# youdie006/CLAP2Diffusion

Hardware: AMD Instinct MI355X
Metric: 512x512 images/sec @ 50 DDIM steps, batch=8, 1/2/4/8 MI355X (higher is better)
Workload: dtype fp16; 1 GPU; c3: batch=8/GPU, 50 DDIM steps, 512x512, CFG 7.5, log-mel+HTSAT+projectors+CLIP+UNet+VAE, all-gather of images; global_batch=8, ddim_steps=50, resolution=512, parallelism=dp1

## Files before the change

clap2diffusion_amd/csrc/common.h:

```cpp
#pragma once
#include <hip/hip_runtime.h>
#include <stdint.h>
#include <stddef.h>
#include <type_traits>
#include <mutex>
#include "../../include/c2d.h"

typedef _Float16 f16;
typedef _Float16 f16x8 __attribute__((ext_vector_type(8)));
typedef _Float16 f16x4 __attribute__((ext_vector_type(4)));
typedef _Float16 f16x2 __attribute__((ext_vector_type(2)));
typedef float f32x4 __attribute__((ext_vector_type(4)));
typedef float f32x2 __attribute__((ext_vector_type(2)));
typedef float f32x16 __attribute__((ext_vector_type(16)));
typedef short s16x4 __attribute__((ext_vector_type(4)));
typedef uint32_t u32x4 __attribute__((ext_vector_type(4)));
typedef uint32_t u32x2 __attribute__((ext_vector_type(2)));

#define LDS_AS __attribute__((address_space(3)))



#ifdef C2D_ENABLE_ABLATION
#define C2D_ABL(x, bit) ((x) & (bit))
#else
#define C2D_ABL(x, bit) 0
#endif

namespace c2d {

template <int B, int E, class F>
__device__ __forceinline__ void static_for(F&& f) {
    if constexpr (B < E) {
        f(std::integral_constant<int, B>{});
        static_for<B + 1, E>(f);
    }
}

extern thread_local int g_last_hip_error;

#ifndef C2D_TUNE_GEMM_MODE
#define C2D_TUNE_GEMM_MODE 0
#endif
#ifndef C2D_TUNE_GEMM_KORDER
#define C2D_TUNE_GEMM_KORDER 1
#endif
#ifndef C2D_TUNE_GEMM_LDSEPI
#define C2D_TUNE_GEMM_LDSEPI 1
#endif
#ifndef C2D_TUNE_SPLITK_F16
#define C2D_TUNE_SPLITK_F16 0
#endif
#ifndef C2D_TUNE_TAIL_SPLIT
#define C2D_TUNE_TAIL_SPLIT 1
#endif
#ifndef C2D_TUNE_PANEL_REGB
#define C2D_TUNE_PANEL_REGB 0
#endif
#ifndef C2D_TUNE_PANEL_STAGGER
#define C2D_TUNE_PANEL_STAGGER 2
#endif
#ifndef C2D_TUNE_PANEL_CARRY
#define C2D_TUNE_PANEL_CARRY 1
#endif
#ifndef C2D_TUNE_PANEL_PRIO
#define C2D_TUNE_PANEL_PRIO 1
#endif
#ifndef C2D_TUNE_ATTN_NEGC
#define C2D_TUNE_ATTN_NEGC 1
#endif
#ifndef C2D_TUNE_ATTN_RES
#define C2D_TUNE_ATTN_RES 1
#endif
#ifndef C2D_TUNE_ATTN_W8
#define C2D_TUNE_ATTN_W8 1
#endif
#ifndef C2D_TUNE_ATTN_PP
#define C2D_TUNE_ATTN_PP 0
#endif
#ifndef C2D_TUNE_GN_BLOCKS
#define C2D_TUNE_GN_BLOCKS 512
#endif
#ifndef C2D_TUNE_GN_APPLY_BLOCKS
#define C2D_TUNE_GN_APPLY_BLOCKS 2048
#endif
#ifndef C2D_TUNE_GN_FUSED_HW
#define C2D_TUNE_GN_FUSED_HW 256
#endif
#ifndef C2D_TUNE_GN_FOLD
#define C2D_TUNE_GN_FOLD 1
#endif
#ifndef C2D_TUNE_GN_FOLD_CAP
#define C2D_TUNE_GN_FOLD_CAP 32
#endif
#ifndef C2D_TUNE_GN_FOLD_APPLY_BLOCKS
#define C2D_TUNE_GN_FOLD_APPLY_BLOCKS 1024
#endif
struct Tuning {
    int gemm_mode, gemm_korder, gemm_lds_epi, splitk_f16, tail_split, panel_regb, panel_stagger;
    int attn_negc, attn_res, attn_w8, attn_pp;
    int gn_blocks, gn_apply_blocks, gn_fused_hw, gn_fold, gn_fold_cap, gn_fold_apply_blocks;
};
constexpr Tuning kTuning = {
    C2D_TUNE_GEMM_MODE, C2D_TUNE_GEMM_KORDER, C2D_TUNE_GEMM_LDSEPI, C2D_TUNE_SPLITK_F16, C2D_TUNE_TAIL_SPLIT,
    C2D_TUNE_PANEL_REGB, C2D_TUNE_PANEL_STAGGER,
    C2D_TUNE_ATTN_NEGC, C2D_TUNE_ATTN_RES, C2D_TUNE_ATTN_W8, C2D_TUNE_ATTN_PP,
    C2D_TUNE_GN_BLOCKS < 64 ? 512 : C2D_TUNE_GN_BLOCKS, C2D_TUNE_GN_APPLY_BLOCKS < 64 ? 2048 : C2D_TUNE_GN_APPLY_BLOCKS,
    C2D_TUNE_GN_FUSED_HW, C2D_TUNE_GN_FOLD, C2D_TUNE_GN_FOLD_CAP < 1 ? 32 : C2D_TUNE_GN_FOLD_CAP,
    C2D_TUNE_GN_FOLD_APPLY_BLOCKS < 64 ? 1024 : C2D_TUNE_GN_FOLD_APPLY_BLOCKS,
};
constexpr const Tuning& tuning() { return kTuning; }
int ablation_gemm();
int ablation_attn();
int plan_override_tile();
int plan_override_split();
constexpr int kMaxDevices = 64;
int current_device();

template <auto K>
inline void ensure_lds(int bytes) {
    static std::once_flag once[kMaxDevices];
    std::call_once(once[current_device()], [bytes] {
        (void)hipFuncSetAttribute((const void*)K, hipFuncAttributeMaxDynamicSharedMemorySize, bytes);
    });
}

inline int check_launch() {
    hipError_t e = hipGetLastError();
    if (e != hipSuccess) {
        g_last_hip_error = (int)e;
        return C2D_E_HIP;
    }
    return C2D_OK;
}

inline bool aligned16(const void* p) { return ((uintptr_t)p & 15) == 0; }

__device__ __forceinline__ float silu_f(float x) { return x / (1.0f + __expf(-x)); }
__device__ __forceinline__ float sigmoid_lin(float x, float k) { return x / (1.0f + __expf(-k * x)); }
__device__ __forceinline__ float erf_as(float x) {
    const float z = fabsf(x);
    const float t = __builtin_amdgcn_rcpf(fmaf(0.3275911f, z, 1.0f));
    float p = fmaf(1.061405429f, t, -1.453152027f);
    p = fmaf(p, t, 1.421413741f);
    p = fmaf(p, t, -0.284496736f);
    p = fmaf(p, t, 0.254829592f);
    const float e = 1.0f - p * t * __expf(-z * z);
    return copysignf(e, x);
}
__device__ __forceinline__ float gelu_f(float x) { return 0.5f * x * (1.0f + erf_as(x * 0.70710678118654752f)); }

__device__ __forceinline__ float gelu_sig(float x) {
    const float xc = __builtin_amdgcn_fmed3f(x, -8.0f, 8.0f);
    const float x2 = xc * xc;
    const float z = xc * fmaf(fmaf(-0.0009763994f, x2, 0.10652431f), x2, 2.3013635f);
    return x * __builtin_amdgcn_rcpf(1.0f + __builtin_amdgcn_exp2f(-z));
}
__device__ __forceinline__ f32x2 geglu2(f32x2 h, f32x2 g) {
    const f32x2 xc = {__builtin_amdgcn_fmed3f(g.x, -8.0f, 8.0f), __builtin_amdgcn_fmed3f(g.y, -8.0f, 8.0f)};
    const f32x2 x2 = xc * xc;
    f32x2 q = __builtin_elementwise_fma(x2, (f32x2){0.0009763994f, 0.0009763994f},
                                        (f32x2){-0.10652431f, -0.10652431f});
    q = __builtin_elementwise_fma(q, x2, (f32x2){-2.3013635f, -2.3013635f});
    const f32x2 nz = xc * q;
    f32x2 e = {__builtin_amdgcn_exp2f(nz.x), __builtin_amdgcn_exp2f(nz.y)};
    e = e + (f32x2){1.0f, 1.0f};
    const f32x2 hg = h * g;
    return hg * (f32x2){__builtin_amdgcn_rcpf(e.x), __builtin_amdgcn_rcpf(e.y)};
}


__device__ __forceinline__ int xcd_remap(int bid, int nwg) {
    const int q = nwg >> 3, r = nwg & 7;
    const int xcd = bid & 7, local = bid >> 3;
    return (xcd < r ? xcd * (q + 1) : r * (q + 1) + (xcd - r) * q) + local;
}

__device__ __forceinline__ const char* uniform_ptr(const void* p) {
    const uint64_t v = (uint64_t)p;
    const uint32_t lo = __builtin_amdgcn_readfirstlane((uint32_t)v);
    const uint32_t hi = __builtin_amdgcn_readfirstlane((uint32_t)(v >> 32));
    return (const char*)(((uint64_t)hi << 32) | lo);
}

__device__ __forceinline__ __amdgpu_buffer_rsrc_t make_rsrc(const void* base, unsigned bytes) {
    return __builtin_amdgcn_make_buffer_rsrc(const_cast<void*>(base), 0, (int)bytes, 0x00020000);
}

__device__ __forceinline__ float wave_sum(float v) {
#pragma unroll
    for (int o = 32; o > 0; o >>= 1) v += __shfl_xor(v, o);
    return v;
}
__device__ __forceinline__ float wave_max(float v) {
#pragma unroll
    for (int o = 32; o > 0; o >>= 1) v = fmaxf(v, __shfl_xor(v, o));
    return v;
}

}
```

clap2diffusion_amd/csrc/epilogue.h:

```cpp
#pragma once

namespace c2d {

template <int W, bool GG, int ROWS, int COLS, int RES, int TEMB, int NT = 64, int RG = 0, bool WB = false>
struct EpiPass {
    typedef _Float16 hv __attribute__((ext_vector_type(W)));
    static constexpr int CPR = GG ? COLS / (2 * W) : COLS / W;
    static constexpr int CPT = 16 / W;
    static constexpr int NCH = ROWS * CPR;
    static constexpr int NIT = (NCH + NT - 1) / NT;
    static_assert(COLS % (GG ? 32 : 8) == 0, "epilogue image width");
    hv r[RES ? NIT : 1], t[TEMB ? NIT : 1];
    __device__ __forceinline__ static bool has_res(const IgemmParams& p) { return RES > 0 || (RES < 0 && p.resid); }
    __device__ __forceinline__ static bool has_temb(const IgemmParams& p) { return TEMB > 0 || (TEMB < 0 && p.temb); }

    __device__ __forceinline__ static void geo(const IgemmParams& p, int m0, int jp0, int lane, int it, int& row,
                                               int& sc, int& m, int& j, bool& ok) {
        int c = lane + NT * it;
        ok = c < NCH;
        c = ok ? c : NCH - 1;
        row = c / CPR;
        const int cc = c - row * CPR;
        if constexpr (GG) {
            const int t = cc / CPT, q = cc - t * CPT;
            sc = t * 32 + q * W;
            j = ((jp0 + t * 32) >> 1) + q * W;
        } else {
            sc = cc * W;
            j = jp0 + sc;
        }
        m = m0 + (RG ? (row >> 5) * RG + (row & 31) : row);
        ok = ok && m < p.M && j < (GG ? (p.cout >> 1) : p.cout);
        if (!ok) { m = m0 < p.M ? m0 : 0; j = 0; }
    }

    __device__ __forceinline__ void prefetch(const IgemmParams& p, int m0, int jp0, int lane) {
        if constexpr (RES != 0 || TEMB != 0) {
            const int hw = p.oh * p.ow;
            const int n_all = (RG == 0 && (hw % ROWS) == 0) ? m0 / hw : -1;
#pragma unroll
            for (int it = 0; it < NIT; ++it) {
                int row, sc, m, j;
                bool ok;
                geo(p, m0, jp0, lane, it, row, sc, m, j, ok);
                if (TEMB != 0 && has_temb(p))
                    t[it] = *reinterpret_cast<const hv*>(p.temb + (size_t)(ok ? (n_all >= 0 ? n_all : m / hw) : 0) *
                                                                      p.temb_ld + j);
                if (RES != 0 && has_res(p)) r[it] = *reinterpret_cast<const hv*>(p.resid + (size_t)m * p.resid_ld + j);
            }
        }
    }

    __device__ __forceinline__ static void body(const IgemmParams& p, const float* img, int pitchf, int row, int sc,
                                                int m, int j, bool ok, const hv& rr, const hv& tt) {
        const float* src = img + row * pitchf + sc;
        float v[W];
#pragma unroll
        for (int q = 0; q < W; q += 4) {
            const float4 x = *reinterpret_cast<const float4*>(src + q);
            v[q] = x.x; v[q + 1] = x.y; v[q + 2] = x.z; v[q + 3] = x.w;
        }
        if constexpr (GG) {
#pragma unroll
            for (int q = 0; q < W; q += 4) {
                const float4 y = *reinterpret_cast<const float4*>(src + 16 + q);
                v[q] *= gelu_sig(y.x); v[q + 1] *= gelu_sig(y.y); v[q + 2] *= gelu_sig(y.z); v[q + 3] *= gelu_sig(y.w);
            }
        } else if (p.act == C2D_ACT_GELU) {
#pragma unroll
            for (int q = 0; q < W; ++q) v[q] = gelu_f(v[q]);
        } else if (p.act == C2D_ACT_RELU) {
#pragma unroll
            for (int q = 0; q < W; ++q) v[q] = fmaxf(v[q], 0.f);
        } else if (p.act == C2D_ACT_SILU) {
#pragma unroll
            for (int q = 0; q < W; ++q) v[q] = silu_f(v[q]);
        } else if (p.act == C2D_ACT_QUICK_GELU) {
#pragma unroll
            for (int q = 0; q < W; ++q) v[q] = sigmoid_lin(v[q], 1.702f);
        }
        if (TEMB != 0 && has_temb(p)) {
#pragma unroll
            for (int q = 0; q < W; ++q) v[q] += (float)tt[q];
        }
        if (RES != 0 && has_res(p)) {
#pragma unroll
            for (int q = 0; q < W; ++q) v[q] += (float)rr[q];
        }
        hv o;
#pragma unroll
        for (int q = 0; q < W; ++q) o[q] = (f16)v[q];
        if (ok) *reinterpret_cast<hv*>(p.out + (size_t)m * p.out_ld + j) = o;
        if constexpr (WB) {
            float* dst = const_cast<float*>(src);
#pragma unroll
            for (int q = 0; q < W; q += 4)
                *reinterpret_cast<float4*>(dst + q) = make_float4((float)o[q], (float)o[q + 1], (float)o[q + 2], (float)o[q + 3]);
        }
    }

    __device__ __forceinline__ void finish(const IgemmParams& p, const float* img, int pitchf, int m0, int jp0,
                                           int lane) const {
#pragma unroll
        for (int it = 0; it < NIT; ++it) {
            int row, sc, m, j;
            bool ok;
            geo(p, m0, jp0, lane, it, row, sc, m, j, ok);
            body(p, img, pitchf, row, sc, m, j, ok, r[RES ? it : 0], t[TEMB ? it : 0]);
        }
    }

    __device__ __forceinline__ static void compact(const IgemmParams& p, const float* img, int pitchf, int m0,
                                                   int jp0, int lane) {
        const int hw = p.oh * p.ow;
        const int n_all = (RG == 0 && (hw % ROWS) == 0) ? m0 / hw : -1;
#pragma unroll 2
        for (int it = 0; it < NIT; ++it) {
            int row, sc, m, j;
            bool ok;
            geo(p, m0, jp0, lane, it, row, sc, m, j, ok);
            hv rr, tt;
            if (TEMB != 0 && has_temb(p))
                tt = *reinterpret_cast<const hv*>(p.temb + (size_t)(ok ? (n_all >= 0 ? n_all : m / hw) : 0) * p.temb_ld + j);
            if (RES != 0 && has_res(p)) rr = *reinterpret_cast<const hv*>(p.resid + (size_t)m * p.resid_ld + j);
            body(p, img, pitchf, row, sc, m, j, ok, rr, tt);
        }
    }
};

template <bool COMPACT, int NT, int RG, int W, bool GG, int ROWS, int COLS, int RES, int TEMB, class WriteImg>
__device__ __forceinline__ void epi_pass_t(const IgemmParams& p, const float* img, int pitchf, int m0, int jp0,
                                           int lane, WriteImg&& write_img) {
    typedef EpiPass<W, GG, ROWS, COLS, RES, TEMB, NT, RG> EP;
    auto sync = [&]() __attribute__((always_inline)) {
        if constexpr (NT == 64) {
            __builtin_amdgcn_s_waitcnt(15 | (7 << 4) | (0 << 8) | (3 << 14));
            __builtin_amdgcn_wave_barrier();
        } else {
            __builtin_amdgcn_s_waitcnt(15 | (7 << 4) | (0 << 8) | (3 << 14));
            asm volatile("" ::: "memory");
            __builtin_amdgcn_s_barrier();
            asm volatile("" ::: "memory");
        }
    };
    if constexpr (COMPACT) {
        write_img();
        sync();
        EP::compact(p, img, pitchf, m0, jp0, lane);
    } else {
        EP ep;
        ep.prefetch(p, m0, jp0, lane);
        write_img();
        sync();
        ep.finish(p, img, pitchf, m0, jp0, lane);
    }
    sync();
}

template <int NT, int RG, int ROWS, int COLS, class WriteImg, class After>
__device__ __forceinline__ void epi_pass_wb(const IgemmParams& p, const float* img, int pitchf, int m0, int jp0,
                                            int lane, WriteImg&& write_img, After&& after) {
    typedef EpiPass<8, false, ROWS, COLS, -1, -1, NT, RG, true> EP;
    auto sync = [&]() __attribute__((always_inline)) {
        __builtin_amdgcn_s_waitcnt(15 | (7 << 4) | (0 << 8) | (3 << 14));
        asm volatile("" ::: "memory");
        __builtin_amdgcn_s_barrier();
        asm volatile("" ::: "memory");
    };
    write_img();
    sync();
    EP::compact(p, img, pitchf, m0, jp0, lane);
    sync();
    after();
    sync();
}

template <int NPASS, int ROWS, int BN, int BM, int RG, class WriteImg>
__device__ __forceinline__ void epi_gn_moments(const IgemmParams& p, float* img, int pitchb, int m0, int n0, int tid,
                                               WriteImg&& write_img) {
    float sh = 0.f, s1 = 0.f, s2 = 0.f;
    static_for<0, NPASS>([&](auto pass) __attribute__((always_inline)) {
        constexpr int b0 = 2 * decltype(pass)::value;
        epi_pass_wb<512, RG, ROWS, BN>(p, img, pitchb, m0 + b0 * 16, n0, tid,
                                       [&]() __attribute__((always_inline)) { write_img(pass); },
                                       [&]() __attribute__((always_inline)) {
            if (tid < BN) {
                if constexpr (b0 == 0) sh = img[tid];
#pragma unroll 8
                for (int r = 0; r < ROWS; ++r) {
                    const float d = img[r * pitchb + tid] - sh;
                    s1 += d;
                    s2 = fmaf(d, d, s2);
                }
            }
        });
    });
    float2* chm = reinterpret_cast<float2*>(img);
    if (tid < BN) chm[tid] = make_float2(sh + s1 * (1.0f / BM), s2 - s1 * s1 * (1.0f / BM));
    __syncthreads();
    const int cpg = p.gn_cpg, ng = BN / cpg;
    if (tid < ng) {
        float mg = 0.f;
        for (int i = 0; i < cpg; ++i) mg += chm[tid * cpg + i].x;
        mg /= (float)cpg;
        float q = 0.f;
        for (int i = 0; i < cpg; ++i) {
            const float2 e = chm[tid * cpg + i];
            const float d = e.x - mg;
            q += e.y + (float)BM * d * d;
        }
        const int hw = p.oh * p.ow, nimg = m0 / hw, tpi = hw / BM, groups = p.cout / cpg;
        const size_t slot = ((size_t)nimg * tpi + (m0 - nimg * hw) / BM) * groups + n0 / cpg + tid;
        reinterpret_cast<float2*>(p.gn_mom)[slot] = make_float2(mg, q);
    }
}

template <int ROWS, int COLS, bool COMPACT, int NT = 64, int RG = 0, class WriteImg>
__device__ __forceinline__ void epi_pass(const IgemmParams& p, const float* img, int pitchf, int m0, int jp0,
                                         int lane, WriteImg&& w) {
    const bool gg = p.act == C2D_ACT_GEGLU;
    const int out_cols = gg ? (p.cout >> 1) : p.cout;
    const uintptr_t al = (uintptr_t)p.out | (uintptr_t)p.resid | (uintptr_t)p.temb;
    const bool wide = ((out_cols | p.out_ld | (p.resid ? p.resid_ld : 0) | (p.temb ? p.temb_ld : 0)) & 7) == 0 &&
                      (al & 15) == 0;
    if constexpr (COMPACT) {
        if constexpr (COLS % 32 == 0) {
            if (gg) {
                if (wide) epi_pass_t<true, NT, RG, 8, true, ROWS, COLS, -1, 0>(p, img, pitchf, m0, jp0, lane, w);
                else epi_pass_t<true, NT, RG, 4, true, ROWS, COLS, -1, 0>(p, img, pitchf, m0, jp0, lane, w);
                return;
            }
        }
        if (wide) epi_pass_t<true, NT, RG, 8, false, ROWS, COLS, -1, -1>(p, img, pitchf, m0, jp0, lane, w);
        else epi_pass_t<true, NT, RG, 4, false, ROWS, COLS, -1, -1>(p, img, pitchf, m0, jp0, lane, w);
        return;
    }
    if constexpr (COLS % 32 == 0) {
        if (gg) {
            if (wide && !p.resid) epi_pass_t<COMPACT, NT, RG, 8, true, ROWS, COLS, 0, 0>(p, img, pitchf, m0, jp0, lane, w);
            else epi_pass_t<COMPACT, NT, RG, 4, true, ROWS, COLS, -1, 0>(p, img, pitchf, m0, jp0, lane, w);
            return;
        }
    }
    if (!wide) epi_pass_t<COMPACT, NT, RG, 4, false, ROWS, COLS, -1, -1>(p, img, pitchf, m0, jp0, lane, w);
    else if (p.resid) {
        if (p.temb) epi_pass_t<COMPACT, NT, RG, 8, false, ROWS, COLS, 1, 1>(p, img, pitchf, m0, jp0, lane, w);
        else epi_pass_t<COMPACT, NT, RG, 8, false, ROWS, COLS, 1, 0>(p, img, pitchf, m0, jp0, lane, w);
    } else {
        if (p.temb) epi_pass_t<COMPACT, NT, RG, 8, false, ROWS, COLS, 0, 1>(p, img, pitchf, m0, jp0, lane, w);
        else epi_pass_t<COMPACT, NT, RG, 8, false, ROWS, COLS, 0, 0>(p, img, pitchf, m0, jp0, lane, w);
    }
}

__device__ __forceinline__ f32x4 bias4(const IgemmParams& p, int j) {
    if (!p.bias || j >= p.cout) return (f32x4){0.f, 0.f, 0.f, 0.f};
    return *reinterpret_cast<const f32x4*>(p.bias + j);
}

template <int W, bool GG, int ROWS, int COLS>
__device__ __forceinline__ void epi_rows_plain_t(const IgemmParams& p, const float* img, int pitchf, int m0, int jp0,
                                           int lane) {
    typedef _Float16 hv __attribute__((ext_vector_type(W)));
    constexpr int CPR = GG ? COLS / (2 * W) : COLS / W;
    constexpr int CPT = 16 / W;
    static_assert(COLS % (GG ? 32 : 8) == 0, "epilogue image width");
    const int hw = p.oh * p.ow;
    const int out_cols = GG ? (p.cout >> 1) : p.cout;
    const int n_all = (hw % ROWS) == 0 ? m0 / hw : -1;
#pragma unroll 2
    for (int c = lane; c < ROWS * CPR; c += 64) {
        const int row = c / CPR, cc = c - row * CPR;
        const int m = m0 + row;
        int sc, jp, j;
        if constexpr (GG) {
            const int t = cc / CPT, q = cc - t * CPT;
            sc = t * 32 + q * W;
            jp = jp0 + sc;
            j = ((jp0 + t * 32) >> 1) + q * W;
        } else {
            sc = cc * W;
            jp = jp0 + sc;
            j = jp;
        }
        if (m >= p.M || j >= out_cols) continue;
        const float* src = img + row * pitchf + sc;
        float v[W];
#pragma unroll
        for (int r = 0; r < W; r += 4) {
            const float4 x = *reinterpret_cast<const float4*>(src + r);
            v[r] = x.x; v[r + 1] = x.y; v[r + 2] = x.z; v[r + 3] = x.w;
        }
        if (p.bias) {
#pragma unroll
            for (int r = 0; r < W; r += 4) {
                const float4 bb = *reinterpret_cast<const float4*>(p.bias + jp + r);
                v[r] += bb.x; v[r + 1] += bb.y; v[r + 2] += bb.z; v[r + 3] += bb.w;
            }
        }
        if constexpr (GG) {
            float g[W];
#pragma unroll
            for (int r = 0; r < W; r += 4) {
                const float4 x = *reinterpret_cast<const float4*>(src + 16 + r);
                g[r] = x.x; g[r + 1] = x.y; g[r + 2] = x.z; g[r + 3] = x.w;
                if (p.bias) {
                    const float4 bb = *reinterpret_cast<const float4*>(p.bias + jp + 16 + r);
                    g[r] += bb.x; g[r + 1] += bb.y; g[r + 2] += bb.z; g[r + 3] += bb.w;
                }
            }
#pragma unroll
            for (int r = 0; r < W; ++r) v[r] *= gelu_sig(g[r]);
        } else if (p.act == C2D_ACT_GELU) {
#pragma unroll
            for (int r = 0; r < W; ++r) v[r] = gelu_f(v[r]);
        } else if (p.act == C2D_ACT_RELU) {
#pragma unroll
            for (int r = 0; r < W; ++r) v[r] = fmaxf(v[r], 0.f);
        } else if (p.act == C2D_ACT_SILU) {
#pragma unroll
            for (int r = 0; r < W; ++r) v[r] = silu_f(v[r]);
        } else if (p.act == C2D_ACT_QUICK_GELU) {
#pragma unroll
            for (int r = 0; r < W; ++r) v[r] = sigmoid_lin(v[r], 1.702f);
        }
        if (p.temb) {
            const hv tt = *reinterpret_cast<const hv*>(p.temb + (size_t)(n_all >= 0 ? n_all : m / hw) * p.temb_ld + j);
#pragma unroll
            for (int r = 0; r < W; ++r) v[r] += (float)tt[r];
        }
        if (p.resid) {
            const hv rr = *reinterpret_cast<const hv*>(p.resid + (size_t)m * p.resid_ld + j);
#pragma unroll
            for (int r = 0; r < W; ++r) v[r] += (float)rr[r];
        }
        hv o;
#pragma unroll
        for (int r = 0; r < W; ++r) o[r] = (f16)v[r];
        *reinterpret_cast<hv*>(p.out + (size_t)m * p.out_ld + j) = o;
    }
}

template <int ROWS, int COLS>
__device__ __forceinline__ void epi_rows_plain(const IgemmParams& p, const float* img, int pitchf, int m0, int jp0,
                                         int lane) {
    const bool gg = p.act == C2D_ACT_GEGLU;
    const int out_cols = gg ? (p.cout >> 1) : p.cout;
    const uintptr_t al = (uintptr_t)p.out | (uintptr_t)p.resid | (uintptr_t)p.temb;
    const bool wide = ((out_cols | p.out_ld | (p.resid ? p.resid_ld : 0) | (p.temb ? p.temb_ld : 0)) & 7) == 0 &&
                      (al & 15) == 0;
    if constexpr (COLS % 32 == 0) {
        if (gg) {
            if (wide) epi_rows_plain_t<8, true, ROWS, COLS>(p, img, pitchf, m0, jp0, lane);
            else epi_rows_plain_t<4, true, ROWS, COLS>(p, img, pitchf, m0, jp0, lane);
            return;
        }
    }
    if (wide) epi_rows_plain_t<8, false, ROWS, COLS>(p, img, pitchf, m0, jp0, lane);
    else epi_rows_plain_t<4, false, ROWS, COLS>(p, img, pitchf, m0, jp0, lane);
}

}
```

clap2diffusion_amd/csrc/igemm.hip:

```cpp
#include "common.h"
#include <stdlib.h>
#include <type_traits>

#ifndef C2D_PP16_DEFAULT
#define C2D_PP16_DEFAULT 1
#endif

#ifndef C2D_IGEMM_PART
#define C2D_IGEMM_PART -1
#endif
#define C2D_PART(k) (C2D_IGEMM_PART < 0 || C2D_IGEMM_PART == (k))

namespace c2d {

enum AMode { AM_1X1 = 0, AM_3X3_FAST = 1, AM_3X3_GEN = 2 };

struct IgemmParams {
    const f16* src0; const f16* src1; int c0, c1, cin;
    int n, h, w, oh, ow, stride, up, pad;
    int vh, vw;
    const f16* wt; int cout, kpad, ktot;
    int pro, pro_silu;
    const float* pro_a; const float* pro_b; const float* gamma; const float* beta;
    const float* bias; int act;
    const f16* temb; int temb_ld;
    const f16* resid; int resid_ld;
    f16* out; int out_ld;
    int M;
    int gx, gy;
    int ksplit;
    int nkt;
    float* ws;
    int slab16;
    int abl;
    int lds_epi;
    int cmajor;
    float pro_eps;
    float* gn_mom;
    int gn_cpg;
};

__device__ __forceinline__ void store_partial(const IgemmParams& p, int slice, int m, int j, const f32x4& v) {
    const size_t off = ((size_t)slice * p.M + m) * p.cout + j;
    if (p.slab16) {
        const f16x4 h = {(f16)v[0], (f16)v[1], (f16)v[2], (f16)v[3]};
        *reinterpret_cast<f16x4*>(reinterpret_cast<f16*>(p.ws) + off) = h;
    } else {
        *reinterpret_cast<f32x4*>(p.ws + off) = v;
    }
}

}
#include "epilogue.h"
namespace c2d {

__device__ __forceinline__ int lds_off(int row, int c) { return row * 128 + ((c ^ ((row >> 1) & 7)) << 4); }

template <int BM>
struct RowInfo {
    int n[BM / 32], iy[BM / 32], ix[BM / 32];
    bool ok[BM / 32];
};

__device__ __forceinline__ f16x8 zero8() {
    f16x8 z;
#pragma unroll
    for (int i = 0; i < 8; ++i) z[i] = (f16)0.f;
    return z;
}

template <int AMODE>
__device__ __forceinline__ f16x8 load_a_chunk(const IgemmParams& p, int n, int iy0, int ix0, bool rok,
                                              int k, int tap_fast, int cbase_fast, int cc, int& cout_c,
                                              bool& valid) {
    int c, ky, kx;
    if (AMODE == AM_1X1) {
        c = k; ky = 0; kx = 0;
        valid = rok && (c < p.cin);
    } else if (AMODE == AM_3X3_FAST) {
        c = cbase_fast + cc * 8;
        ky = tap_fast / 3; kx = tap_fast - ky * 3;
        valid = rok;
    } else {
        int tap = k / p.cin;
        c = k - tap * p.cin;
        ky = tap / 3; kx = tap - ky * 3;
        valid = rok && (tap < 9);
    }
    int iy = iy0 + ky, ix = ix0 + kx;
    valid = valid && iy >= 0 && iy < p.vh && ix >= 0 && ix < p.vw;
    cout_c = c;
    if (!valid) return zero8();
    if (p.up) { iy >>= 1; ix >>= 1; }
    size_t pix = ((size_t)n * p.h + iy) * p.w + ix;
    const f16* ptr = (c < p.c0) ? (p.src0 + pix * p.c0 + c) : (p.src1 + pix * p.c1 + (c - p.c0));
    return *reinterpret_cast<const f16x8*>(ptr);
}

__device__ __forceinline__ f16x8 apply_pro(const IgemmParams& p, f16x8 v, int n, int m, int c) {
    if (p.pro == C2D_PRO_GN) {
        const float4* sc = reinterpret_cast<const float4*>(p.pro_a + (size_t)n * p.cin + c);
        const float4* sh = reinterpret_cast<const float4*>(p.pro_b + (size_t)n * p.cin + c);
        float4 s0 = sc[0], s1 = sc[1], h0 = sh[0], h1 = sh[1];
        float s[8] = {s0.x, s0.y, s0.z, s0.w, s1.x, s1.y, s1.z, s1.w};
        float hh[8] = {h0.x, h0.y, h0.z, h0.w, h1.x, h1.y, h1.z, h1.w};
#pragma unroll
        for (int i = 0; i < 8; ++i) {
            float y = (float)v[i] * s[i] + hh[i];
            if (p.pro_silu) y = silu_f(y);
            v[i] = (f16)y;
        }
    } else if (p.pro == C2D_PRO_LN) {
        float2 st = *reinterpret_cast<const float2*>(p.pro_a + (size_t)m * 2);
        const float4* g = reinterpret_cast<const float4*>(p.gamma + c);
        const float4* b = reinterpret_cast<const float4*>(p.beta + c);
        float4 g0 = g[0], g1 = g[1], b0 = b[0], b1 = b[1];
        float gg[8] = {g0.x, g0.y, g0.z, g0.w, g1.x, g1.y, g1.z, g1.w};
        float bb[8] = {b0.x, b0.y, b0.z, b0.w, b1.x, b1.y, b1.z, b1.w};
#pragma unroll
        for (int i = 0; i < 8; ++i) v[i] = (f16)(((float)v[i] - st.x) * st.y * gg[i] + bb[i]);
    } else if (p.pro == C2D_PRO_SILU) {
#pragma unroll
        for (int i = 0; i < 8; ++i) v[i] = (f16)silu_f((float)v[i]);
    }
    return v;
}

template <int TM, int TN>
__device__ __forceinline__ void epilogue_tiles(const IgemmParams& p, f32x4 (&acc)[TN][TM], int mrow0, int ncol0,
                                               int lane) {
    const int hw = p.oh * p.ow;
    const int lr = lane & 15, lc = 4 * (lane >> 4);
    int mrow[TM], nimg[TM];
    bool mok[TM];
#pragma unroll
    for (int b = 0; b < TM; ++b) {
        const int m = mrow0 + b * 16 + lr;
        mok[b] = m < p.M;
        mrow[b] = mok[b] ? m : p.M - 1;
        nimg[b] = mrow[b] / hw;
    }
    if (p.act != C2D_ACT_GEGLU) {
        int col[TN];
        bool cok[TN];
        float4 bv[TN];
#pragma unroll
        for (int a = 0; a < TN; ++a) {
            const int j = ncol0 + a * 16 + lc;
            cok[a] = j < p.cout;
            col[a] = cok[a] ? j : 0;
            bv[a] = p.bias ? *reinterpret_cast<const float4*>(p.bias + col[a]) : make_float4(0.f, 0.f, 0.f, 0.f);
        }
        f16x4 rv[TM][TN], tv[TM][TN];
        if (p.resid) {
#pragma unroll
            for (int b = 0; b < TM; ++b)
#pragma unroll
                for (int a = 0; a < TN; ++a)
                    rv[b][a] = *reinterpret_cast<const f16x4*>(p.resid + (size_t)mrow[b] * p.resid_ld + col[a]);
        }
        if (p.temb) {
#pragma unroll
            for (int b = 0; b < TM; ++b)
#pragma unroll
                for (int a = 0; a < TN; ++a)
                    tv[b][a] = *reinterpret_cast<const f16x4*>(p.temb + (size_t)nimg[b] * p.temb_ld + col[a]);
        }
#pragma unroll
        for (int b = 0; b < TM; ++b) {
#pragma unroll
            for (int a = 0; a < TN; ++a) {
                float v[4] = {acc[a][b][0] + bv[a].x, acc[a][b][1] + bv[a].y, acc[a][b][2] + bv[a].z,
                              acc[a][b][3] + bv[a].w};
#pragma unroll
                for (int r = 0; r < 4; ++r) {
                    if (p.act == C2D_ACT_GELU) v[r] = gelu_f(v[r]);
                    else if (p.act == C2D_ACT_RELU) v[r] = fmaxf(v[r], 0.f);
                    else if (p.act == C2D_ACT_SILU) v[r] = silu_f(v[r]);
                    else if (p.act == C2D_ACT_QUICK_GELU) v[r] = sigmoid_lin(v[r], 1.702f);
                    if (p.temb) v[r] += (float)tv[b][a][r];
                    if (p.resid) v[r] += (float)rv[b][a][r];
                }
                f16x4 o;
#pragma unroll
                for (int r = 0; r < 4; ++r) o[r] = (f16)v[r];
                if (mok[b] && cok[a]) *reinterpret_cast<f16x4*>(p.out + (size_t)mrow[b] * p.out_ld + col[a]) = o;
            }
        }
    } else {
        constexpr int TP = TN / 2;
        int jo[TP], jh[TP];
        bool cok[TP];
        float4 bh[TP], bg[TP];
#pragma unroll
        for (int q = 0; q < TP; ++q) {
            const int jp = ncol0 + 2 * q * 16;
            cok[q] = jp < p.cout;
            const int jpc = cok[q] ? jp : 0;
            jo[q] = (jpc >> 1) + lc;
            jh[q] = jpc + lc;
            bh[q] = p.bias ? *reinterpret_cast<const float4*>(p.bias + jh[q]) : make_float4(0.f, 0.f, 0.f, 0.f);
            bg[q] = p.bias ? *reinterpret_cast<const float4*>(p.bias + jh[q] + 16) : make_float4(0.f, 0.f, 0.f, 0.f);
        }
        f16x4 rv[TM][TP];
        if (p.resid) {
#pragma unroll
            for (int b = 0; b < TM; ++b)
#pragma unroll
                for (int q = 0; q < TP; ++q)
                    rv[b][q] = *reinterpret_cast<const f16x4*>(p.resid + (size_t)mrow[b] * p.resid_ld + jo[q]);
        }
#pragma unroll
        for (int b = 0; b < TM; ++b) {
#pragma unroll
            for (int q = 0; q < TP; ++q) {
                const f32x4 h4 = acc[2 * q][b], g4 = acc[2 * q + 1][b];
                const float hb[4] = {bh[q].x, bh[q].y, bh[q].z, bh[q].w}, gb[4] = {bg[q].x, bg[q].y, bg[q].z, bg[q].w};
                f16x4 o;
#pragma unroll
                for (int r = 0; r < 4; ++r) {
                    float v = (h4[r] + hb[r]) * gelu_sig(g4[r] + gb[r]);
                    if (p.resid) v += (float)rv[b][q][r];
                    o[r] = (f16)v;
                }
                if (mok[b] && cok[q]) *reinterpret_cast<f16x4*>(p.out + (size_t)mrow[b] * p.out_ld + jo[q]) = o;
            }
        }
    }
}

template <int BM, int BN>
__device__ __forceinline__ void epilogue(const IgemmParams& p, f32x4 (&acc)[BN / 32][BM / 32], int m0, int n0, int wm,
                                         int wn, int lane) {
    epilogue_tiles<BM / 32, BN / 32>(p, acc, m0 + wm * (BM / 2), n0 + wn * (BN / 2), lane);
}

__device__ __forceinline__ void epilogue_w64(const IgemmParams& p, f32x4 (&acc)[4][4], int mw0, int nw0, int lane) {
    epilogue_tiles<4, 4>(p, acc, mw0, nw0, lane);
}

template <int BM, int BN, int AMODE>
__global__ void __launch_bounds__(256) igemm_kernel(IgemmParams p) {
    constexpr int TM = BM / 32;
    constexpr int TN = BN / 32;
    constexpr int ACH = BM / 32;
    constexpr int BCH = BN / 32;
    constexpr int A_BYTES = BM * 128, B_BYTES = BN * 128;
    extern __shared__ __attribute__((aligned(16))) char smem[];

    const int tid = threadIdx.x, lane = tid & 63, wave = tid >> 6;
    const int wm = wave >> 1, wn = wave & 1;
    const int tile = xcd_remap(blockIdx.x, p.gx * p.gy);
    const int mt = tile / p.gx, nt = tile - mt * p.gx;
    const int m0 = mt * BM, n0 = nt * BN;

    const int cc = tid & 7;
    const int hw = p.oh * p.ow;
    int a_n[ACH], a_iy[ACH], a_ix[ACH], a_m[ACH];
    bool a_ok[ACH];
#pragma unroll
    for (int i = 0; i < ACH; ++i) {
        int m = m0 + (tid >> 3) + 32 * i;
        a_m[i] = m;
        a_ok[i] = m < p.M;
        int mm = a_ok[i] ? m : 0;
        int nn = mm / hw, r = mm - nn * hw;
        int oy = r / p.ow, ox = r - oy * p.ow;
        a_n[i] = nn;
        a_iy[i] = oy * p.stride - p.pad;
        a_ix[i] = ox * p.stride - p.pad;
    }
    const f16* b_ptr[BCH];
    bool b_ok[BCH];
#pragma unroll
    for (int i = 0; i < BCH; ++i) {
        int j = n0 + (tid >> 3) + 32 * i;
        b_ok[i] = j < p.cout;
        b_ptr[i] = p.wt + (size_t)(b_ok[i] ? j : 0) * p.kpad + cc * 8;
    }

    f32x4 acc[TN][TM];
#pragma unroll
    for (int a = 0; a < TN; ++a)
#pragma unroll
        for (int b = 0; b < TM; ++b) acc[a][b] = (f32x4){0.f, 0.f, 0.f, 0.f};

    f16x8 ra[ACH], rb[BCH];
    int rc[ACH];
    bool rv[ACH];
    const int nk = p.kpad / 64;

    auto gload = [&](int kt) {
        const int k0 = kt * 64;
        int tap = 0, cbase = 0;
        if (AMODE == AM_3X3_FAST) { tap = k0 / p.cin; cbase = k0 - tap * p.cin; }
#pragma unroll
        for (int i = 0; i < ACH; ++i)
            ra[i] = load_a_chunk<AMODE>(p, a_n[i], a_iy[i], a_ix[i], a_ok[i], k0 + cc * 8, tap, cbase, cc, rc[i], rv[i]);
#pragma unroll
        for (int i = 0; i < BCH; ++i)
            rb[i] = b_ok[i] ? *reinterpret_cast<const f16x8*>(b_ptr[i] + k0) : zero8();
    };
    auto swrite = [&](int buf) {
        char* As = smem + buf * (A_BYTES + B_BYTES);
        char* Bs = As + A_BYTES;
#pragma unroll
        for (int i = 0; i < ACH; ++i) {
            f16x8 v = ra[i];
            if (p.pro != C2D_PRO_NONE && rv[i]) v = apply_pro(p, v, a_n[i], a_m[i], rc[i]);
            int row = (tid >> 3) + 32 * i;
            *reinterpret_cast<f16x8*>(As + lds_off(row, cc)) = v;
        }
#pragma unroll
        for (int i = 0; i < BCH; ++i) {
            int row = (tid >> 3) + 32 * i;
            *reinterpret_cast<f16x8*>(Bs + lds_off(row, cc)) = rb[i];
        }
    };

    gload(0);
    swrite(0);
    __syncthreads();

    for (int kt = 0; kt < nk; ++kt) {
        const int buf = kt & 1;
        if (kt + 1 < nk) gload(kt + 1);
        const char* As = smem + buf * (A_BYTES + B_BYTES);
        const char* Bs = As + A_BYTES;
#pragma unroll
        for (int kk = 0; kk < 2; ++kk) {
            const int ch = kk * 4 + (lane >> 4);
            f16x8 fa[TM], fb[TN];
#pragma unroll
            for (int t = 0; t < TM; ++t) {
                int row = wm * (BM / 2) + t * 16 + (lane & 15);
                fa[t] = *reinterpret_cast<const f16x8*>(As + lds_off(row, ch));
            }
#pragma unroll
            for (int t = 0; t < TN; ++t) {
                int row = wn * (BN / 2) + t * 16 + (lane & 15);
                fb[t] = *reinterpret_cast<const f16x8*>(Bs + lds_off(row, ch));
            }
#pragma unroll
            for (int a = 0; a < TN; ++a)
#pragma unroll
                for (int b = 0; b < TM; ++b)
                    acc[a][b] = __builtin_amdgcn_mfma_f32_16x16x32_f16(fb[a], fa[b], acc[a][b], 0, 0, 0);
        }
        if (kt + 1 < nk) swrite(buf ^ 1);
        __syncthreads();
    }

    epilogue<BM, BN>(p, acc, m0, n0, wm, wn, lane);
}


typedef __attribute__((address_space(3))) void* lptr_t;
constexpr unsigned kOOB = 0x80000000u;

__device__ __forceinline__ void wait_vmcnt_le(int n) {
#define C2D_WAITVM(N) __builtin_amdgcn_s_waitcnt(((N) & 15) | (7 << 4) | (15 << 8) | (((N) >> 4) << 14))
    switch (n) {
        case 4: C2D_WAITVM(4); break;
        case 6: C2D_WAITVM(6); break;
        case 8: C2D_WAITVM(8); break;
        case 12: C2D_WAITVM(12); break;
        case 16: C2D_WAITVM(16); break;
        default: C2D_WAITVM(0); break;
    }
#undef C2D_WAITVM
}


__device__ __forceinline__ void dma_piece(__amdgpu_buffer_rsrc_t r, char* lds, unsigned off) {
    __builtin_amdgcn_raw_ptr_buffer_load_lds(r, (lptr_t)lds, 16, off, 0, 0, 0);
}

template <int TM, int TN>
__device__ __forceinline__ void epilogue_chunked(const IgemmParams& p, f32x4 (&acc)[TN][TM], int mrow0, int ncol0,
                                                 int lane) {
    constexpr int MC = TM < 4 ? TM : 4;
#pragma unroll
    for (int b0 = 0; b0 < TM; b0 += MC) {
        f32x4 sub[TN][MC];
#pragma unroll
        for (int a = 0; a < TN; ++a)
#pragma unroll
            for (int b = 0; b < MC; ++b) sub[a][b] = acc[a][b0 + b];
        epilogue_tiles<MC, TN>(p, sub, mrow0 + b0 * 16, ncol0, lane);
    }
}

template <int WM, int WN, int TM, int TN, int STAGES, int KS, int KG = 1>
__global__ void __launch_bounds__(64 * WM * WN * KG) igemm_dma_kernel(IgemmParams p) {
    constexpr int NW = WM * WN;
    constexpr int BM = WM * TM * 16, BN = WN * TN * 16;
    constexpr int AI = BM / (8 * NW), BI = BN / (8 * NW);
    constexpr int PER = AI + BI;
    constexpr int A_BYTES = BM * 128, B_BYTES = BN * 128, STAGE = A_BYTES + B_BYTES;
    static_assert(AI * 8 * NW == BM && BI * 8 * NW == BN, "tile / wave mismatch");
    extern __shared__ __attribute__((aligned(16))) char smem_all[];

    const int tid = threadIdx.x, lane = tid & 63;
    const int wave_all = __builtin_amdgcn_readfirstlane(tid >> 6);
    const int kg = wave_all / NW, wave = wave_all - kg * NW;
    char* const smem = smem_all + (KG > 1 ? kg * STAGES * STAGE : 0);
    const int wm = wave / WN, wn = wave - (wave / WN) * WN;
    const int bid = xcd_remap(blockIdx.x, p.gx * p.gy * p.ksplit);
    const int tile = bid / p.ksplit, slice = bid - tile * p.ksplit;
    const int mt = tile / p.gx, nt = tile - mt * p.gx;
    const int m0 = mt * BM, n0 = nt * BN;
    const int lrow = lane >> 3, slot = lane & 7;
    const int hw = p.oh * p.ow;
    const bool two = p.c1 > 0;
    const int pshift = KS == 3 ? p.w + 1 : 0;

    unsigned a_off0[AI], a_off1[AI], a_mask[AI];
    int a_ch[AI];
#pragma unroll
    for (int i = 0; i < AI; ++i) {
        const int row = (wave * AI + i) * 8 + lrow;
        const int m = m0 + row;
        const int mm = m < p.M ? m : 0;
        const int nn = mm / hw, r = mm - nn * hw;
        const int oy = r / p.ow, ox = r - oy * p.ow;
        const int iy0 = oy * p.stride - p.pad, ix0 = ox * p.stride - p.pad;
        unsigned mask = 0;
        if (m < p.M) {
#pragma unroll
            for (int ky = 0; ky < KS; ++ky)
#pragma unroll
                for (int kx = 0; kx < KS; ++kx)
                    if (iy0 + ky >= 0 && iy0 + ky < p.h && ix0 + kx >= 0 && ix0 + kx < p.w) mask |= 1u << (ky * KS + kx);
        }
        const int pix0 = (nn * p.h + iy0) * p.w + ix0 + pshift;
        a_ch[i] = (slot ^ ((row >> 1) & 7)) * 8;
        a_off0[i] = (unsigned)(2 * (pix0 * p.c0 + a_ch[i]));
        a_off1[i] = (unsigned)(2 * (pix0 * p.c1 + a_ch[i]));
        a_mask[i] = mask;
    }
    unsigned b_off[BI];
#pragma unroll
    for (int i = 0; i < BI; ++i) {
        const int row = (wave * BI + i) * 8 + lrow;
        const int j = n0 + row;
        b_off[i] = (j < p.cout) ? (unsigned)(2 * (j * p.kpad + (slot ^ ((row >> 1) & 7)) * 8)) : kOOB;
    }
    const size_t npix = (size_t)p.n * p.h * p.w;
    const unsigned bytes0 = (unsigned)(npix * p.c0 * 2), bytes1 = (unsigned)(npix * p.c1 * 2);
    const unsigned wbytes = (unsigned)((size_t)p.cout * p.kpad * 2);
    const bool ctail = (p.cin & 63) != 0;

    const int nk_all = p.kpad / 64;
    const int kb0 = slice * p.nkt, ke0 = min(nk_all, kb0 + p.nkt);
    const int kper = (ke0 - kb0 + KG - 1) / KG;
    const int kb = min(ke0, kb0 + kg * kper), ke = min(ke0, kb + kper);
    const char* u_src0 = uniform_ptr(p.src0);
    const char* u_src1 = uniform_ptr(p.src1);
    const char* u_wt = uniform_ptr(p.wt);
    int tap = 0, cbase = kb * 64;
    if (KS == 3) {
        if (p.cmajor) { tap = kb % 9; cbase = (kb / 9) * 64; }
        else { tap = cbase / p.cin; cbase -= tap * p.cin; }
    }
    auto issue = [&](int kt, int buf) {
        (void)kt;
        const int k0 = tap * p.cin + cbase;
        const int ky = tap / 3, kx = tap - (tap / 3) * 3;
        const bool use1 = two && cbase >= p.c0;
        const int cs = use1 ? p.c1 : p.c0;
        const unsigned sterm = 2u * (unsigned)((KS == 3 ? (ky * p.w + kx) * cs : 0) + (use1 ? cbase - p.c0 : cbase));
        const char* sb = use1 ? u_src1 : u_src0;
        const unsigned bias = 2u * (unsigned)(pshift * cs);
        const unsigned sbytes = use1 ? bytes1 : bytes0;
        const __amdgpu_buffer_rsrc_t ra = make_rsrc(sb + sterm - bias, sbytes + bias - sterm);
        const __amdgpu_buffer_rsrc_t rb = make_rsrc(u_wt + 2 * k0, wbytes - 2 * k0);
        const int lim = p.cin - cbase;
        char* base = smem + buf * STAGE;
#pragma unroll
        for (int i = 0; i < AI; ++i) {
            unsigned ok = (a_mask[i] >> tap) & 1u;
            if (ctail) ok &= (unsigned)(a_ch[i] < lim);
            const unsigned off = (use1 ? a_off1[i] : a_off0[i]) | ((ok - 1u) & kOOB);
            dma_piece(ra, base + (wave * AI + i) * 1024, off);
        }
#pragma unroll
        for (int i = 0; i < BI; ++i)
            dma_piece(rb, base + A_BYTES + (wave * BI + i) * 1024, b_off[i]);
        if (KS == 3 && p.cmajor) {
            if (++tap == 9) { tap = 0; cbase += 64; }
        } else {
            cbase += 64;
            if (KS == 3 && cbase >= p.cin) { cbase = 0; ++tap; }
        }
    };

    int fa0[2], fb0[2];
#pragma unroll
    for (int kk = 0; kk < 2; ++kk) {
        const int l = lds_off(lane & 15, kk * 4 + (lane >> 4));
        fa0[kk] = wm * TM * 2048 + l;
        fb0[kk] = A_BYTES + wn * TN * 2048 + l;
    }

    f32x4 acc[TN][TM];
#pragma unroll
    for (int a = 0; a < TN; ++a)
#pragma unroll
        for (int b = 0; b < TM; ++b) acc[a][b] = (f32x4){0.f, 0.f, 0.f, 0.f};

#pragma unroll
    for (int s0 = 0; s0 < STAGES - 1; ++s0)
        if (kb + s0 < ke) issue(kb + s0, s0);
    int rd = 0, wr = STAGES - 1;
    const int kend = KG > 1 ? kb + kper : ke;
    for (int kt = kb; kt < kend; ++kt) {
        if (kt + STAGES - 2 < ke) wait_vmcnt_le(PER * (STAGES - 2));
        else wait_vmcnt_le(0);
        asm volatile("" ::: "memory");
        __builtin_amdgcn_s_barrier();
        asm volatile("" ::: "memory");
        if (kt + STAGES - 1 < ke && !(C2D_ABL(p.abl, 1))) issue(kt + STAGES - 1, wr);
        const char* S = smem + rd * STAGE;
        if (KG > 1 && kt >= ke) continue;
#pragma unroll
        for (int kk = 0; kk < 2; ++kk) {
            f16x8 fa[TM], fb[TN];
#pragma unroll
            for (int t = 0; t < TN; ++t) fb[t] = *reinterpret_cast<const f16x8*>(S + fb0[kk] + t * 2048);
#pragma unroll
            for (int t = 0; t < TM; ++t) fa[t] = *reinterpret_cast<const f16x8*>(S + fa0[kk] + t * 2048);
            if (C2D_ABL(p.abl, 2)) {
#pragma unroll
                for (int t = 0; t < TN; ++t) asm volatile("" :: "v"(fb[t]));
#pragma unroll
                for (int t = 0; t < TM; ++t) asm volatile("" :: "v"(fa[t]));
                continue;
            }
            __builtin_amdgcn_s_setprio(1);
#pragma unroll
            for (int b = 0; b < TM; ++b)
#pragma unroll
                for (int a = 0; a < TN; ++a)
                    acc[a][b] = __builtin_amdgcn_mfma_f32_16x16x32_f16(fb[a], fa[b], acc[a][b], 0, 0, 0);
            __builtin_amdgcn_s_setprio(0);
        }
        rd = (rd + 1 == STAGES) ? 0 : rd + 1;
        wr = (wr + 1 == STAGES) ? 0 : wr + 1;
    }
    if constexpr (KG > 1) {
        constexpr int EPI = NW * 16 * (TM < 2 ? TM : 2) * (TN * 16 + 4) * 4;
        constexpr int RED = (EPI + 1023) / 1024 * 1024;
        f32x4* red = reinterpret_cast<f32x4*>(smem_all + RED);
        __syncthreads();
        if (kg > 0) {
#pragma unroll
            for (int a = 0; a < TN; ++a)
#pragma unroll
                for (int b = 0; b < TM; ++b)
                    red[((((kg - 1) * NW + wave) * TN + a) * TM + b) * 64 + lane] = acc[a][b];
        }
        __syncthreads();
        if (kg > 0) return;
#pragma unroll
        for (int g = 1; g < KG; ++g)
#pragma unroll
            for (int a = 0; a < TN; ++a)
#pragma unroll
                for (int b = 0; b < TM; ++b) acc[a][b] += red[((((g - 1) * NW + wave) * TN + a) * TM + b) * 64 + lane];
    }
    if (p.ksplit > 1) {
        const int mw0 = m0 + wm * TM * 16, nw0 = n0 + wn * TN * 16;
#pragma unroll
        for (int b = 0; b < TM; ++b) {
            const int m = mw0 + b * 16 + (lane & 15);
#pragma unroll
            for (int a = 0; a < TN; ++a) {
                const int j = nw0 + a * 16 + 4 * (lane >> 4);
                if (m < p.M && j < p.cout) store_partial(p, slice, m, j, acc[a][b]);
            }
        }
        return;
    }
    __syncthreads();
    {
        constexpr int PITCHF = TN * 16 + 4;
        constexpr int RB = TM < 2 ? TM : 2;
        float* img = reinterpret_cast<float*>(smem) + wave * 16 * RB * PITCHF;
        const int mw0 = m0 + wm * TM * 16, nw0 = n0 + wn * TN * 16;
        static_for<0, TM / RB>([&](auto pass) __attribute__((always_inline)) {
            constexpr int b0 = RB * decltype(pass)::value;
            epi_pass<RB * 16, TN * 16, false>(p, img, PITCHF, mw0 + b0 * 16, nw0, lane, [&]() __attribute__((always_inline)) {
                f32x4 bv[TN];
#pragma unroll
                for (int a = 0; a < TN; ++a) bv[a] = bias4(p, nw0 + a * 16 + 4 * (lane >> 4));
#pragma unroll
                for (int bb = 0; bb < RB; ++bb)
#pragma unroll
                    for (int a = 0; a < TN; ++a)
                        *reinterpret_cast<f32x4*>(img + (bb * 16 + (lane & 15)) * PITCHF + a * 16 + 4 * (lane >> 4)) =
                            acc[a][b0 + bb] + bv[a];
            });
        });
    }
}

#if C2D_PART(0)
template <bool S16>
__device__ __forceinline__ f32x4 slab_quad(const float* ws, size_t off) {
    if constexpr (S16) {
        const f16x4 h = *reinterpret_cast<const f16x4*>(reinterpret_cast<const f16*>(ws) + off);
        return (f32x4){(float)h[0], (float)h[1], (float)h[2], (float)h[3]};
    } else {
        return *reinterpret_cast<const f32x4*>(ws + off);
    }
}

template <int KS, bool S16>
__global__ void __launch_bounds__(256) splitk_reduce_kernel(IgemmParams p) {
    const int cq = p.cout >> 2;
    const size_t i = (size_t)blockIdx.x * blockDim.x + threadIdx.x;
    if (i >= (size_t)p.M * cq) return;
    const int hw = p.oh * p.ow;
    const size_t slab = (size_t)p.M * p.cout;
    const int m = (int)(i / cq);
    const int j = (int)(i - (size_t)m * cq) * 4;
    const size_t src = (size_t)m * p.cout + j;
    float4 bv = {0.f, 0.f, 0.f, 0.f};
    f16x4 tv = {0, 0, 0, 0}, rv = {0, 0, 0, 0};
    if (p.bias) bv = *reinterpret_cast<const float4*>(p.bias + j);
    if (p.temb) tv = *reinterpret_cast<const f16x4*>(p.temb + (size_t)(m / hw) * p.temb_ld + j);
    if (p.resid) rv = *reinterpret_cast<const f16x4*>(p.resid + (size_t)m * p.resid_ld + j);
    f32x4 acc;
    if constexpr (KS > 0) {
        f32x4 v[KS];
#pragma unroll
        for (int sl = 0; sl < KS; ++sl) v[sl] = slab_quad<S16>(p.ws, src + sl * slab);
        acc = v[0];
#pragma unroll
        for (int sl = 1; sl < KS; ++sl) acc += v[sl];
    } else {
        acc = slab_quad<S16>(p.ws, src);
        int sl = 1;
        for (; sl + 4 <= p.ksplit; sl += 4) {
            const f32x4 a = slab_quad<S16>(p.ws, src + sl * slab);
            const f32x4 b = slab_quad<S16>(p.ws, src + (sl + 1) * slab);
            const f32x4 c = slab_quad<S16>(p.ws, src + (sl + 2) * slab);
            const f32x4 d = slab_quad<S16>(p.ws, src + (sl + 3) * slab);
            acc += a; acc += b; acc += c; acc += d;
        }
        for (; sl < p.ksplit; ++sl) acc += slab_quad<S16>(p.ws, src + sl * slab);
    }
    float v[4] = {acc[0] + bv.x, acc[1] + bv.y, acc[2] + bv.z, acc[3] + bv.w};
    f16x4 o;
#pragma unroll
    for (int r = 0; r < 4; ++r) {
        if (p.act == C2D_ACT_GELU) v[r] = gelu_f(v[r]);
        else if (p.act == C2D_ACT_RELU) v[r] = fmaxf(v[r], 0.f);
        else if (p.act == C2D_ACT_SILU) v[r] = silu_f(v[r]);
        else if (p.act == C2D_ACT_QUICK_GELU) v[r] = sigmoid_lin(v[r], 1.702f);
        if (p.temb) v[r] += (float)tv[r];
        if (p.resid) v[r] += (float)rv[r];
        o[r] = (f16)v[r];
    }
    *reinterpret_cast<f16x4*>(p.out + (size_t)m * p.out_ld + j) = o;
}

constexpr int kGnRb = 16;
template <int KS, bool S16>
__global__ void __launch_bounds__(640) splitk_reduce_gn_kernel(IgemmParams p) {
    __shared__ float2 cm[8][320];
    const int t = threadIdx.x, q = t % 80, rs = t / 80;
    const int m0 = blockIdx.x * kGnRb, j = blockIdx.y * 320 + 4 * q;
    const int hw = p.oh * p.ow;
    const size_t slab = (size_t)p.M * p.cout;
    float4 bv = {0.f, 0.f, 0.f, 0.f};
    f16x4 tv = {0, 0, 0, 0}, rv[2] = {{0, 0, 0, 0}, {0, 0, 0, 0}};
    if (p.bias) bv = *reinterpret_cast<const float4*>(p.bias + j);
    if (p.temb) tv = *reinterpret_cast<const f16x4*>(p.temb + (size_t)(m0 / hw) * p.temb_ld + j);
    f32x4 v[2][KS];
#pragma unroll
    for (int i = 0; i < 2; ++i) {
        const int m = m0 + rs + 8 * i;
        if (p.resid) rv[i] = *reinterpret_cast<const f16x4*>(p.resid + (size_t)m * p.resid_ld + j);
#pragma unroll
        for (int sl = 0; sl < KS; ++sl) v[i][sl] = slab_quad<S16>(p.ws, (size_t)m * p.cout + j + sl * slab);
    }
    float y[2][4];
    const float b4[4] = {bv.x, bv.y, bv.z, bv.w};
#pragma unroll
    for (int i = 0; i < 2; ++i) {
        f32x4 acc = v[i][0];
#pragma unroll
        for (int sl = 1; sl < KS; ++sl) acc += v[i][sl];
        f16x4 o;
#pragma unroll
        for (int r = 0; r < 4; ++r) {
            float x = acc[r] + b4[r];
            if (p.temb) x += (float)tv[r];
            if (p.resid) x += (float)rv[i][r];
            o[r] = (f16)x;
            y[i][r] = (float)o[r];
        }
        *reinterpret_cast<f16x4*>(p.out + (size_t)(m0 + rs + 8 * i) * p.out_ld + j) = o;
    }
#pragma unroll
    for (int r = 0; r < 4; ++r) {
        const float d = y[0][r] - y[1][r];
        cm[rs][4 * q + r] = make_float2(0.5f * (y[0][r] + y[1][r]), 0.5f * d * d);
    }
    __syncthreads();
    float2 col = {0.f, 0.f};
    if (t < 320) {
        float mu = 0.f;
#pragma unroll
        for (int k = 0; k < 8; ++k) mu += cm[k][t].x;
        mu *= 0.125f;
        float m2 = 0.f;
#pragma unroll
        for (int k = 0; k < 8; ++k) {
            const float d = cm[k][t].x - mu;
            m2 += cm[k][t].y + 2.0f * d * d;
        }
        col = make_float2(mu, m2);
    }
    __syncthreads();
    if (t < 320) cm[0][t] = col;
    __syncthreads();
    const int cpg = p.gn_cpg, ng = 320 / cpg;
    if (t < ng) {
        float mg = 0.f;
        for (int i = 0; i < cpg; ++i) mg += cm[0][t * cpg + i].x;
        mg /= (float)cpg;
        float m2 = 0.f;
        for (int i = 0; i < cpg; ++i) {
            const float d = cm[0][t * cpg + i].x - mg;
            m2 += cm[0][t * cpg + i].y + (float)kGnRb * d * d;
        }
        const int nimg = m0 / hw, groups = p.cout / cpg;
        const size_t slot = ((size_t)nimg * (hw / kGnRb) + (m0 - nimg * hw) / kGnRb) * groups + blockIdx.y * ng + t;
        reinterpret_cast<float2*>(p.gn_mom)[slot] = make_float2(mg, m2);
    }
}

void run_splitk_reduce(const IgemmParams& p, hipStream_t s) {
    if (p.gn_mom) {
        const dim3 grid((unsigned)(p.M / kGnRb), (unsigned)(p.cout / 320)), blk(640);
#define C2D_SKG(KS)                                                                                    \
    if (p.slab16) hipLaunchKernelGGL((splitk_reduce_gn_kernel<KS, true>), grid, blk, 0, s, p);        \
    else hipLaunchKernelGGL((splitk_reduce_gn_kernel<KS, false>), grid, blk, 0, s, p)
        switch (p.ksplit) {
            case 2: C2D_SKG(2); break;
            case 3: C2D_SKG(3); break;
            case 4: C2D_SKG(4); break;
            case 5: C2D_SKG(5); break;
            case 6: C2D_SKG(6); break;
            case 8: C2D_SKG(8); break;
            case 10: C2D_SKG(10); break;
            case 12: C2D_SKG(12); break;
            case 15: C2D_SKG(15); break;
            default: C2D_SKG(16); break;
        }
#undef C2D_SKG
        return;
    }
    const size_t total = (size_t)p.M * (p.cout >> 2);
    const dim3 grid((unsigned)((total + 255) / 256)), blk(256);
#define C2D_SKR(KS)                                                                   \
    if (p.slab16) hipLaunchKernelGGL((splitk_reduce_kernel<KS, true>), grid, blk, 0, s, p); \
    else hipLaunchKernelGGL((splitk_reduce_kernel<KS, false>), grid, blk, 0, s, p)
    switch (p.ksplit) {
        case 2: C2D_SKR(2); break;
        case 3: C2D_SKR(3); break;
        case 4: C2D_SKR(4); break;
        case 6: C2D_SKR(6); break;
        case 8: C2D_SKR(8); break;
        case 12: C2D_SKR(12); break;
        case 16: C2D_SKR(16); break;
        default: C2D_SKR(0); break;
    }
#undef C2D_SKR
}
#else
void run_splitk_reduce(const IgemmParams& p, hipStream_t s);
#endif

}
#include "igemm_m32.h"
#include "igemm_pp16.h"
#include "igemm_pps.h"
#include "igemm_pp16r.h"
#include "igemm_panel.h"
namespace c2d {

template <int WM, int WN, int TM, int TN, int STAGES, int KS, int KG = 1>
static void launch_dma(const IgemmParams& p, hipStream_t s) {
    constexpr int ring = KG * STAGES * (WM * TM + WN * TN) * 16 * 128;
    constexpr int epi0 = WM * WN * 16 * (TM < 2 ? TM : 2) * (TN * 16 + 4) * 4;
    constexpr int epi = KG > 1 ? (epi0 + 1023) / 1024 * 1024 + (KG - 1) * WM * WN * TM * TN * 1024 : epi0;
    constexpr int smem = ring > epi ? ring : epi;
    static_assert(smem <= 160 * 1024, "LDS ring / epilogue image too large");
    auto k = igemm_dma_kernel<WM, WN, TM, TN, STAGES, KS, KG>;
    ensure_lds<igemm_dma_kernel<WM, WN, TM, TN, STAGES, KS, KG>>(smem);
    hipLaunchKernelGGL(k, dim3(p.gx * p.gy * p.ksplit), dim3(64 * WM * WN * KG), smem, s, p);
    if (p.ksplit > 1) run_splitk_reduce(p, s);
}

template <int BM, int BN, int AMODE>
static void launch(const IgemmParams& p, hipStream_t s) {
    const int smem = 2 * (BM + BN) * 128;
    dim3 grid(p.gx * p.gy);
    hipLaunchKernelGGL((igemm_kernel<BM, BN, AMODE>), grid, dim3(256), smem, s, p);
}

}

using namespace c2d;

static int gemm_mode() { return tuning().gemm_mode; }

static int gemm_tile() { return plan_override_tile(); }

template <int WM, int WN, int TM, int TN, int ST, int KG = 1>
static void run_dma(IgemmParams& p, int ksize, int cout, hipStream_t s) {
    constexpr int BM = WM * TM * 16, BN = WN * TN * 16;
    p.gx = (cout + BN - 1) / BN;
    p.gy = (p.M + BM - 1) / BM;
    if (ksize == 1) launch_dma<WM, WN, TM, TN, ST, 1, KG>(p, s);
    else launch_dma<WM, WN, TM, TN, ST, 3, KG>(p, s);
}

#define C2D_TILE_FN(ID) void run_tile_##ID(IgemmParams& p, int ksize, int cout, hipStream_t s)
namespace c2d {
C2D_TILE_FN(25); C2D_TILE_FN(40); C2D_TILE_FN(41); C2D_TILE_FN(28); C2D_TILE_FN(29);
C2D_TILE_FN(7); C2D_TILE_FN(1); C2D_TILE_FN(2); C2D_TILE_FN(3); C2D_TILE_FN(50); C2D_TILE_FN(8); C2D_TILE_FN(9);
C2D_TILE_FN(42); C2D_TILE_FN(43); C2D_TILE_FN(44); C2D_TILE_FN(70); C2D_TILE_FN(80); C2D_TILE_FN(81);
#if C2D_PART(1)
C2D_TILE_FN(40) { run_pp16<5>(p, ksize, cout, s); }
C2D_TILE_FN(41) { run_pp16<4>(p, ksize, cout, s); }
C2D_TILE_FN(50) { (void)ksize; (void)cout; run_pps(p, s); }
C2D_TILE_FN(42) { (void)ksize; (void)cout; run_pp16r<5>(p, 42, s); }
C2D_TILE_FN(43) { (void)ksize; (void)cout; run_pp16r<5>(p, 43, s); }
C2D_TILE_FN(44) { (void)ksize; (void)cout; run_pp16r<5>(p, 44, s); }
#endif
#if C2D_PART(2)
C2D_TILE_FN(25) { run_m32<4, 2, 2, 5, 64, 2, 3, 0, true>(p, ksize, cout, s); }
C2D_TILE_FN(28) { run_m32<4, 2, 2, 4, 64, 2, 3>(p, ksize, cout, s); }
C2D_TILE_FN(29) { run_m32<4, 2, 2, 2, 64, 3, 3>(p, ksize, cout, s); }
#endif
#if C2D_PART(3)
C2D_TILE_FN(7) { run_dma<2, 4, 4, 5, 2>(p, ksize, cout, s); }
C2D_TILE_FN(1) { run_dma<4, 2, 4, 4, 3>(p, ksize, cout, s); }
C2D_TILE_FN(2) { run_dma<2, 2, 4, 4, 3>(p, ksize, cout, s); }
C2D_TILE_FN(3) { run_dma<2, 2, 2, 2, 3>(p, ksize, cout, s); }
C2D_TILE_FN(8) { run_dma<2, 2, 4, 5, 2>(p, ksize, cout, s); }
C2D_TILE_FN(9) { run_dma<2, 2, 2, 5, 2>(p, ksize, cout, s); }
C2D_TILE_FN(80) { run_dma<2, 2, 4, 5, 2, 2>(p, ksize, cout, s); }
C2D_TILE_FN(81) { run_dma<2, 2, 2, 5, 2, 2>(p, ksize, cout, s); }
#endif
#if C2D_PART(4)
C2D_TILE_FN(70) { (void)ksize; (void)cout; run_panel(p, s); }
#endif
}
#undef C2D_TILE_FN

#if C2D_PART(0)
struct DmaTile { int id, bm, bn, occ; float rate; bool geglu; };
static const DmaTile kDmaTiles[] = {
    {25, 256, 320, 1, 0.0f, true},
    {40, 256, 320, 1, 0.0f, false},
    {41, 256, 256, 1, 0.0f, true},
    {28, 256, 256, 1, 0.0f, true},
    {29, 256, 128, 1, 0.0f, true},
    {7, 128, 320, 1, 3.1f, false},
    {1, 256, 128, 1, 2.9f, true},
    {2, 128, 128, 1, 2.2f, true},
    {3, 64, 64, 3, 1.9f, true},
    {8, 128, 160, 2, 0.0f, false},
    {9, 64, 160, 2, 0.0f, false},
    {80, 128, 160, 1, 0.0f, false},
    {81, 64, 160, 1, 0.0f, false},
    {42, 256, 320, 1, 0.0f, false},
    {43, 128, 320, 1, 0.0f, false},
    {44, 128, 320, 1, 0.0f, false},
};
struct DmaPlan { int id, split, nkt; };

static DmaPlan plan_dma(long M, int cout, int nk, bool geglu, int force_id, int force_split) {
    DmaPlan best = {3, 1, nk};
    double best_t = 1e300;
    const int splits[] = {1, 2, 3, 4, 6, 8, 12, 16};
    for (const DmaTile& t : kDmaTiles) {
        if (geglu && !t.geglu) continue;
        if (force_id && t.id != force_id) continue;
        if (!force_id && t.rate <= 0.f) continue;
        const long tiles = ((M + t.bm - 1) / t.bm) * ((cout + t.bn - 1) / t.bn);
        for (int sp : splits) {
            if (force_split && sp != force_split) continue;
            if (!force_split && sp > 8) continue;
            if (sp > 1 && (geglu || nk < 8 * sp || tiles >= 256)) continue;
            const int nkt = (nk + sp - 1) / sp;
            const int eff = (nk + nkt - 1) / nkt;
            const long blocks = tiles * eff;
            const long slots = 256L * t.occ;
            const double blk_us = 2.0 * t.bm * t.bn * 64.0 * (nkt + 3) * t.occ / ((t.rate > 0.f ? t.rate : 3.0f) * 1e6);
            double est = (double)((blocks + slots - 1) / slots) * blk_us;
            if (eff > 1) est += (double)M * cout * 4.0 * (eff + 1) / 4e6 + 2.0;
            if (est < best_t) { best_t = est; best = {t.id, eff, nkt}; }
        }
    }
    return best;
}

static int gemm_abl() { return ablation_gemm(); }

static int gemm_korder() { return tuning().gemm_korder; }

static int gemm_lds_epi() { return tuning().gemm_lds_epi; }

static bool epi_direct_ok(const c2d_conv_desc* d) {
    const int out_cols = d->act == C2D_ACT_GEGLU ? d->cout / 2 : d->cout;
    const uintptr_t a8 = (uintptr_t)d->out | (uintptr_t)d->resid | (uintptr_t)d->temb;
    return (out_cols % 4) == 0 && (d->out_ld % 4) == 0 && (!d->resid || (d->resid_ld % 4) == 0) &&
           (!d->temb || (d->temb_ld % 4) == 0) && (a8 & 7) == 0 && ((uintptr_t)d->bias & 15) == 0;
}

static int gemm_split() { return plan_override_split(); }

static bool pps_eligible(const c2d_conv_desc* d) {
    const long M = (long)d->n * d->oh * d->ow;
    return d->ksize == 1 && !d->resid && !d->temb && (d->act == C2D_ACT_NONE || d->act == C2D_ACT_GEGLU) &&
           pps_nk_ok(d->kpad / 64) && (d->out_ld % 4) == 0 && ((uintptr_t)d->out & 7) == 0 &&
           ((uintptr_t)d->bias & 15) == 0 && (size_t)M * d->out_ld * 2 < (1u << 31);
}

struct PlanHint { int ksize; long M; int kpad, cout; bool geglu; int id, split; };
static const PlanHint kPlanHints[] = {
    {1, 8192, 1280, 320, false, 9, 1},
    {1, 2048, 640, 1920, false, 9, 1},
    {1, 512, 1280, 1280, false, 3, 1},
    {1, 2048, 640, 5120, true, 50, 1},
    {3, 8192, 2880, 320, false, 7, 4},
    {3, 8192, 5760, 320, false, 40, 6},
    {3, 8192, 8640, 320, false, 40, 8},
    {3, 2048, 5760, 640, false, 7, 8},
    {3, 2048, 17280, 640, false, 40, 16},
    {3, 512, 11520, 1280, false, 7, 12},
    {3, 512, 17280, 1280, false, 41, 16},
    {3, 512, 23040, 1280, false, 41, 16},
    {3, 128, 11520, 1280, false, 81, 12},
    {3, 128, 23040, 1280, false, 81, 12},
    {1, 2048, 3200, 640, false, 81, 2},
    {1, 128, 6400, 1280, false, 3, 12},
    {1, 73728, 320, 320, false, 7, 1},
    {1, 73728, 1280, 320, false, 7, 1},
    {1, 18432, 640, 640, false, 41, 1},
    {1, 18432, 2560, 640, false, 41, 1},
    {1, 4608, 5120, 1280, false, 40, 3},
    {1, 4608, 1280, 10240, true, 41, 1},
    {1, 1152, 1280, 1280, false, 3, 1},
    {3, 18432, 5760, 640, false, 41, 1},
    {3, 1152, 11520, 1280, false, 41, 8},
    {3, 1152, 23040, 1280, false, 41, 8},
    {1, 1152, 6400, 1280, false, 80, 3},
    {1, 73728, 1600, 320, false, 7, 1},
    {1, 18432, 3200, 640, false, 41, 1},
#ifndef C2D_NO_PANEL_HINTS
    {1, 65536, 320, 2560, true, 70, 1},
    {1, 16384, 640, 5120, true, 70, 1},
    {1, 65536, 320, 960, false, 70, 1},
    {1, 73728, 320, 2560, true, 70, 1},
    {1, 8192, 320, 2560, true, 70, 1},
    {1, 8192, 320, 960, false, 70, 1},
#endif
    {1, 4096, 1280, 1280, false, 80, 1},
    {1, 1024, 1280, 1280, false, 3, 1},
    {3, 1024, 11520, 1280, false, 41, 12},
    {3, 1024, 23040, 1280, false, 41, 12},
    {1, 4096, 6400, 1280, false, 80, 1},
    {1, 2097152, 256, 128, false, 1, 1},
    {1, 524288, 512, 256, false, 1, 1},
};

static bool plan_hint(int ksize, long M, int kpad, int cout, bool geglu, DmaPlan& pl) {
    for (const PlanHint& h : kPlanHints)
        if (h.ksize == ksize && h.M == M && h.kpad == kpad && h.cout == cout && h.geglu == geglu) {
            const int nk = kpad / 64;
            const int nkt = (nk + h.split - 1) / h.split;
            pl = {h.id, (nk + nkt - 1) / nkt, nkt};
            return true;
        }
    return false;
}

struct RrHint { long M; int kpad, cout, id, split; };
static const RrHint kRrHints[] = {
    {8192, 5760, 320, 42, 5},
    {8192, 8640, 320, 42, 8},
    {2048, 2880, 640, 43, 5},
    {2048, 5760, 640, 43, 5},
    {2048, 8640, 640, 43, 8},
    {2048, 11520, 640, 43, 5},
    {2048, 17280, 640, 43, 8},
    {512, 5760, 1280, 44, 10},
    {512, 11520, 1280, 44, 10},
    {512, 17280, 1280, 44, 15},
    {512, 23040, 1280, 44, 10},
};

static bool rr_compatible(int id, int rr_id) { return id == rr_id; }

static bool rr_hint(long M, int kpad, int cout, int rr_id, int& id, int& split) {
    for (const RrHint& h : kRrHints)
        if (h.M == M && h.kpad == kpad && h.cout == cout && rr_compatible(h.id, rr_id)) {
            id = h.id;
            split = h.split;
            return true;
        }
    return false;
}

static DmaPlan rr_plan(int id, int nk, int split) {
    const int ncb = nk / 9;
    const int sp = split < 1 ? 1 : (split > ncb ? ncb : split);
    const int cbs = (ncb + sp - 1) / sp;
    return {id, (ncb + cbs - 1) / cbs, 9 * cbs};
}

static DmaPlan plan_for(long M, int cout, int kpad, int act, bool pps_ok, int ksize, int rr_id = 0,
                        bool panel_ok = false) {
    const bool geglu = act == C2D_ACT_GEGLU;
    const int nk = kpad / 64;
    int id = gemm_tile();
    if (id == 70) {
        if (panel_ok && gemm_split() <= 1) return {70, 1, nk};
        id = 0;
    }
    if (id == 42 || id == 43 || id == 44) {
        if (rr_id && rr_compatible(id, rr_id)) return rr_plan(id, nk, gemm_split());
        id = 0;
    }
    if (!id && rr_id && !gemm_split()) {
        int hid = 0, sp = 0;
        if (rr_hint(M, kpad, cout, rr_id, hid, sp)) return rr_plan(hid, nk, sp);
    }
    if (!id && rr_id && !gemm_split() && cout % 320 == 0) {
        const long tiles = (M / (rr_id == 42 ? 256 : 128)) * (cout / 320);
        const int ncb = nk / 9;
        if (tiles >= 192 && (rr_id != 43 || ncb < 30)) return rr_plan(rr_id, nk, 1);
        if (rr_id == 44 && tiles >= 96 && ncb >= 4 && ncb <= 10) return rr_plan(rr_id, nk, 2);
    }
    if (!id && !gemm_split()) {
        DmaPlan pl;
        if (plan_hint(ksize, M, kpad, cout, geglu, pl) && (pl.id != 50 || pps_ok) && (pl.id != 70 || panel_ok)) return pl;
    }
    if (id == 7 && geglu) id = 0;
    if (id == 50) {
        if (pps_ok) return {50, 1, nk};
        id = 0;
    }
    if (!id && pps_ok && geglu && (nk == 5 || nk == 10) && ((M + 191) / 192) * ((cout + 255) / 256) >= 512)
        return {50, 1, nk};
    if (id) {
        DmaPlan pl = plan_dma(M, cout, nk, geglu, id, gemm_split());
        if (pl.id) return pl;
    }
    if (cout <= 64 && !geglu) {
        DmaPlan pl = plan_dma(M, cout, nk, geglu, 29, 0);
        if (pl.id == 29) return pl;
    }
    if (!geglu && cout % 320 != 0) {
        const long mt = (M + 255) / 256;
        if (C2D_PP16_DEFAULT && cout % 256 == 0 && mt * (cout / 256) >= 192) return {41, 1, nk};
        if (cout % 256 != 0 && cout % 128 == 0 && mt * (cout / 128) >= 192) return {29, 1, nk};
    }
    const int t256x320 = (geglu || !C2D_PP16_DEFAULT) ? 25 : 40;
    const long t24 = ((M + 255) / 256) * ((cout + 319) / 320);
    if (t24 >= 192) {
        if (!geglu && C2D_PP16_DEFAULT) {
            const long mt = (M + 255) / 256;
            const long r40 = (t24 + 255) / 256, r41 = (mt * ((cout + 255) / 256) + 255) / 256;
            if (r41 * 256 < r40 * 320) return {41, 1, nk};
        }
        return {t256x320, 1, nk};
    }
    if (nk >= 90 && t24 >= 64) {
        DmaPlan pl = plan_dma(M, cout, nk, geglu, 25, 0);
        if (pl.id == 25) pl.id = t256x320;
        return pl;
    }
    const long t7 = geglu ? ((M + 255) / 256) * ((cout + 127) / 128) : ((M + 127) / 128) * ((cout + 319) / 320);
    if (t7 >= 256) return {geglu ? 1 : 7, 1, nk};
    return plan_dma(M, cout, nk, geglu, 0, 0);
}

static void dispatch_dma(IgemmParams& p, const DmaPlan& pl, int ksize, int cout, hipStream_t s) {
    p.ksplit = pl.split;
    p.nkt = pl.nkt;
    switch (pl.id) {
        case 42: return run_tile_42(p, ksize, cout, s);
        case 43: return run_tile_43(p, ksize, cout, s);
        case 44: return run_tile_44(p, ksize, cout, s);
        case 25: return run_tile_25(p, ksize, cout, s);
        case 40: return run_tile_40(p, ksize, cout, s);
        case 41: return run_tile_41(p, ksize, cout, s);
        case 28: return run_tile_28(p, ksize, cout, s);
        case 29: return run_tile_29(p, ksize, cout, s);
        case 50: return run_tile_50(p, ksize, cout, s);
        case 7: return run_tile_7(p, ksize, cout, s);
        case 1: return run_tile_1(p, ksize, cout, s);
        case 2: return run_tile_2(p, ksize, cout, s);
        case 8: return run_tile_8(p, ksize, cout, s);
        case 9: return run_tile_9(p, ksize, cout, s);
        case 80: return run_tile_80(p, ksize, cout, s);
        case 81: return run_tile_81(p, ksize, cout, s);
        case 70: return run_tile_70(p, ksize, cout, s);
        default: return run_tile_3(p, ksize, cout, s);
    }
}

static bool dma_eligible(const c2d_conv_desc* d) {
    const int cin = d->c0 + d->c1;
    const int amode = (d->ksize == 1) ? AM_1X1 : ((cin % 64) == 0 ? AM_3X3_FAST : AM_3X3_GEN);
    const int pd = d->src_pad ? 2 : 0;
    const size_t src_bytes = (size_t)d->n * (d->h + pd) * (d->w + pd) * (size_t)(d->c0 > d->c1 ? d->c0 : d->c1) * 2;
    return (d->pro == C2D_PRO_NONE || d->pro == C2D_PRO_LNFOLD) && amode != AM_3X3_GEN && !d->up && gemm_mode() != 2 &&
           (d->c1 == 0 || (d->c0 & 63) == 0) && src_bytes < (1u << 31) &&
           (size_t)d->cout * d->kpad * 2 < (1u << 31);
}

static bool panel_eligible(const c2d_conv_desc* d) {
    return d->ksize == 1 && d->c1 == 0 && (d->c0 == 320 || d->c0 == 640) && d->kpad == d->c0 && (d->cout & 31) == 0 &&
           (d->pro == C2D_PRO_NONE || (d->pro == C2D_PRO_LNFOLD && !d->resid)) &&
           !d->temb && (d->act == C2D_ACT_NONE || (d->act == C2D_ACT_GEGLU && !d->resid)) &&
           epi_direct_ok(d) && dma_eligible(d) && (size_t)d->n * d->oh * d->ow * d->out_ld * 2 < (1u << 31);
}

static int rr_eligible(const c2d_conv_desc* d) {
    if (!(d->src_pad && d->pro == C2D_PRO_NONE && d->oh == d->h && d->ow == d->w && d->kpad == 9 * d->c0)) return 0;
    return pp16r_tile_for(d->ksize, d->stride, 0, d->c1, d->c0, d->ow, d->oh, d->w + 2);
}

static int tail_images(const c2d_conv_desc* d, const DmaPlan& pl) {
    if (pl.split != 1 || d->n < 2 || d->pro != C2D_PRO_NONE || d->kpad / 64 < 16) return 0;
    if (plan_override_tile() || plan_override_split() || !tuning().tail_split) return 0;
    const DmaTile* t = nullptr;
    for (const DmaTile& x : kDmaTiles)
        if (x.id == pl.id) t = &x;
    if (!t) return 0;
    const long hw = (long)d->oh * d->ow, slots = 256L * t->occ;
    const long gx = (d->cout + t->bn - 1) / t->bn;
    const long tiles = (d->n * hw + t->bm - 1) / t->bm * gx;
    const long full = tiles / slots * slots, rem = tiles - full;
    if (full == 0 || rem == 0 || rem > slots / 4) return 0;
    int n1 = d->n - 1;
    while (n1 > 0 && (n1 * hw + t->bm - 1) / t->bm * gx > full) --n1;
    return n1;
}

static c2d_conv_desc tail_desc(const c2d_conv_desc* d, int n1) {
    c2d_conv_desc t = *d;
    const size_t in_pix = (size_t)n1 * (d->src_pad ? (size_t)(d->h + 2) * (d->w + 2) : (size_t)d->h * d->w);
    const size_t out_rows = (size_t)n1 * d->oh * d->ow;
    t.n = d->n - n1;
    t.src0 = static_cast<const f16*>(d->src0) + in_pix * d->c0;
    if (d->src1) t.src1 = static_cast<const f16*>(d->src1) + in_pix * d->c1;
    if (d->temb) t.temb = static_cast<const f16*>(d->temb) + (size_t)n1 * d->temb_ld;
    if (d->resid) t.resid = static_cast<const f16*>(d->resid) + out_rows * d->resid_ld;
    t.out = static_cast<f16*>(d->out) + out_rows * d->out_ld;
    return t;
}

static size_t tail_ws_bytes(const c2d_conv_desc* d, int n1) {
    const c2d_conv_desc t = tail_desc(d, n1);
    const long Mt = (long)t.n * t.oh * t.ow;
    const DmaPlan tp = plan_for(Mt, t.cout, t.kpad, t.act, pps_eligible(&t), t.ksize, rr_eligible(&t), panel_eligible(&t));
    return tp.split > 1 ? (size_t)tp.split * Mt * t.cout * sizeof(float) : 0;
}

extern "C" size_t c2d_conv2d_igemm_workspace_size(const c2d_conv_desc* d) {
    if (!d || d->ksize < 1 || d->oh <= 0 || d->ow <= 0 || d->n <= 0 || d->cout <= 0 || d->kpad < 64) return 0;
    if (!dma_eligible(d)) return 0;
    if (d->pro == C2D_PRO_LNFOLD) return 0;
    const long M = (long)d->n * d->oh * d->ow;
    const DmaPlan pl = plan_for(M, d->cout, d->kpad, d->act, pps_eligible(d), d->ksize, rr_eligible(d), panel_eligible(d));
    if (const int n1 = tail_images(d, pl)) return tail_ws_bytes(d, n1);
    return pl.split > 1 ? (size_t)pl.split * M * d->cout * sizeof(float) : 0;
}

static bool gn_split_ok(int ks) {
    return ks == 2 || ks == 3 || ks == 4 || ks == 5 || ks == 6 || ks == 8 || ks == 10 || ks == 12 || ks == 15 || ks == 16;
}

static int gn_rows_for(const c2d_conv_desc* d) {
    if (!d || d->gn_groups <= 0 || d->cout % d->gn_groups) return 0;
    const int cpg = d->cout / d->gn_groups;
    if (320 % cpg || d->cout % 320 || d->act != C2D_ACT_NONE) return 0;
    if ((d->out_ld & 7) || (d->resid && (d->resid_ld & 7)) || (d->temb && (d->temb_ld & 7)) || d->out_ld < d->cout) return 0;
    if (((uintptr_t)d->out | (uintptr_t)d->resid | (uintptr_t)d->temb) & 15) return 0;
    if (d->ksize < 1 || d->oh <= 0 || d->ow <= 0 || d->n <= 0 || d->kpad < 64 || !dma_eligible(d)) return 0;
    const long M = (long)d->n * d->oh * d->ow;
    DmaPlan pl = plan_for(M, d->cout, d->kpad, d->act, pps_eligible(d), d->ksize, rr_eligible(d), panel_eligible(d));
    if (pl.id == 50 || pl.id == 70) return 0;
    bool split = false;
    if (pl.split > 1) {
        const size_t need = (size_t)pl.split * M * d->cout * sizeof(float);
        split = d->ws && d->ws_bytes >= need && aligned16(d->ws);
    }
    if (d->n >= 2 && tail_images(d, pl)) return 0;
    if (split) {
        if (pl.id == 42 || pl.id == 43 || pl.id == 44) {
            const int ncb = d->c0 / 64, cbs = (pl.nkt + 8) / 9 < 1 ? 1 : ((pl.nkt + 8) / 9 > ncb ? ncb : (pl.nkt + 8) / 9);
            pl.split = (ncb + cbs - 1) / cbs;
        }
        return gn_split_ok(pl.split) && ((long)d->oh * d->ow) % kGnRb == 0 ? kGnRb : 0;
    }
    if (!(d->resid || d->temb)) return 0;
    if (pl.id == 40) return ((long)d->oh * d->ow) % 256 == 0 ? 256 : 0;
    if (pl.id != 42 && pl.id != 43 && pl.id != 44) return 0;
    return pl.id == 42 ? 256 : 128;
}

extern "C" int c2d_conv2d_gn_rows(const c2d_conv_desc* d) { return gn_rows_for(d); }

extern "C" int c2d_conv2d_igemm_plan(const c2d_conv_desc* d, int* tile_id, int* ksplit) {
    if (!d || !tile_id || !ksplit) return C2D_E_ARG;
    if (d->ksize < 1 || d->oh <= 0 || d->ow <= 0 || d->n <= 0 || d->cout <= 0 || d->kpad < 64) return C2D_E_SHAPE;
    if (d->pro == C2D_PRO_LNFOLD) {
        if (!panel_eligible(d)) return C2D_E_SHAPE;
        *tile_id = 70;
        *ksplit = 1;
        return C2D_OK;
    }
    if (!dma_eligible(d)) {
        *tile_id = 0;
        *ksplit = 1;
        return C2D_OK;
    }
    const long M = (long)d->n * d->oh * d->ow;
    DmaPlan pl = plan_for(M, d->cout, d->kpad, d->act, pps_eligible(d), d->ksize, rr_eligible(d), panel_eligible(d));
    if (pl.split > 1) {
        const size_t need = (size_t)pl.split * M * d->cout * sizeof(float);
        if (!(d->ws && d->ws_bytes >= need && aligned16(d->ws))) pl.split = 1;
    }
    *tile_id = pl.id;
    *ksplit = pl.split;
    return C2D_OK;
}

static int conv_run(const c2d_conv_desc* d, hipStream_t s, const DmaPlan* fixed);

extern "C" int c2d_conv2d_igemm(const c2d_conv_desc* d, void* stream) {
    if (!d || !d->src0 || !d->weight || !d->out) return C2D_E_ARG;
    hipStream_t s = (hipStream_t)stream;
    if (d->gn_mom && gn_rows_for(d) == 0) return C2D_E_SHAPE;
    if (d->gn_mom && ((uintptr_t)d->gn_mom & 7)) return C2D_E_ALIGN;
    if (d->n >= 2 && d->ksize >= 1 && d->oh > 0 && d->ow > 0 && d->cout > 0 && d->kpad >= 64 && dma_eligible(d)) {
        const long M = (long)d->n * d->oh * d->ow;
        const DmaPlan pl = plan_for(M, d->cout, d->kpad, d->act, pps_eligible(d), d->ksize, rr_eligible(d), panel_eligible(d));
        if (const int n1 = tail_images(d, pl)) {
            c2d_conv_desc head = *d;
            head.n = n1;
            const int rc = conv_run(&head, s, &pl);
            if (rc != C2D_OK) return rc;
            const c2d_conv_desc tail = tail_desc(d, n1);
            return conv_run(&tail, s, nullptr);
        }
    }
    return conv_run(d, s, nullptr);
}

static int conv_run(const c2d_conv_desc* d, hipStream_t s, const DmaPlan* fixed) {
    if (!d || !d->src0 || !d->weight || !d->out) return C2D_E_ARG;
    if (d->ksize != 1 && d->ksize != 3) return C2D_E_SHAPE;
    if (d->c1 > 0 && !d->src1) return C2D_E_ARG;
    const int cin = d->c0 + d->c1;
    if ((d->c0 & 7) || (d->c1 & 7) || cin <= 0) return C2D_E_SHAPE;
    if (d->kpad & 63) return C2D_E_SHAPE;
    const int ktot = d->ksize * d->ksize * cin;
    if (d->kpad < ktot) return C2D_E_SHAPE;
    if ((d->cout & 3) || d->cout <= 0) return C2D_E_SHAPE;
    if (d->act == C2D_ACT_GEGLU && (d->cout & 31)) return C2D_E_SHAPE;
    if (d->act == C2D_ACT_GEGLU && d->temb) return C2D_E_ARG;
    if (d->act != C2D_ACT_NONE && d->act != C2D_ACT_GEGLU && d->temb) return C2D_E_ARG;
    if ((d->out_ld & 3) || (d->resid && (d->resid_ld & 3)) || (d->temb && (d->temb_ld & 3))) return C2D_E_ALIGN;
    if (!aligned16(d->src0) || (d->src1 && !aligned16(d->src1)) || !aligned16(d->weight)) return C2D_E_ALIGN;
    if (((uintptr_t)d->out & 7) || (d->resid && ((uintptr_t)d->resid & 7)) || (d->temb && ((uintptr_t)d->temb & 7)))
        return C2D_E_ALIGN;
    if (d->bias && ((uintptr_t)d->bias & 15)) return C2D_E_ALIGN;
    if (d->pro == C2D_PRO_GN && (!d->pro_a || !d->pro_b || (cin & 3))) return C2D_E_ARG;
    if (d->pro == C2D_PRO_LN && (!d->pro_a || !d->gamma || !d->beta)) return C2D_E_ARG;
    if (d->pro < 0 || d->pro > 4 || d->act < 0 || d->act > 5) return C2D_E_ARG;
    if (d->pro == C2D_PRO_LNFOLD && !(d->pro_eps > 0.f)) return C2D_E_ARG;
    if (d->pro == C2D_PRO_LNFOLD && !panel_eligible(d)) return C2D_E_SHAPE;
    if (d->stride != 1 && d->stride != 2) return C2D_E_SHAPE;
    if (d->ksize == 1 && (d->stride != 1 || d->up || d->oh != d->h || d->ow != d->w)) return C2D_E_SHAPE;
    if (d->up && d->stride != 1) return C2D_E_SHAPE;
    if (d->src_pad && (d->ksize != 3 || d->stride != 1 || d->up || d->c1 || d->oh != d->h || d->ow != d->w))
        return C2D_E_SHAPE;
    if (d->src_pad && d->pro != C2D_PRO_NONE) return C2D_E_ARG;

    IgemmParams p;
    p.src0 = (const f16*)d->src0; p.src1 = (const f16*)d->src1;
    p.c0 = d->c0; p.c1 = d->c1; p.cin = cin;
    p.n = d->n; p.h = d->h; p.w = d->w; p.oh = d->oh; p.ow = d->ow;
    p.stride = d->stride; p.up = d->up; p.pad = (d->ksize == 3) ? 1 : 0;
    p.vh = d->up ? 2 * d->h : d->h; p.vw = d->up ? 2 * d->w : d->w;
    if (d->src_pad) {
        p.h = d->h + 2; p.w = d->w + 2; p.vh = p.h; p.vw = p.w; p.pad = 0;
    } else if (d->ksize == 3) {
        int eh = (p.vh + 2 - 3) / d->stride + 1, ew = (p.vw + 2 - 3) / d->stride + 1;
        if (eh != d->oh || ew != d->ow) return C2D_E_SHAPE;
    }
    p.wt = (const f16*)d->weight; p.cout = d->cout; p.kpad = d->kpad; p.ktot = ktot;
    p.pro = d->pro; p.pro_silu = d->pro_silu;
    p.pro_a = d->pro_a; p.pro_b = d->pro_b; p.gamma = d->gamma; p.beta = d->beta;
    p.bias = d->bias; p.act = d->act;
    p.pro_eps = d->pro == C2D_PRO_LNFOLD ? d->pro_eps : 0.f;
    p.temb = (const f16*)d->temb; p.temb_ld = d->temb_ld;
    p.resid = (const f16*)d->resid; p.resid_ld = d->resid_ld;
    p.out = (f16*)d->out; p.out_ld = d->out_ld;
    p.M = d->n * d->oh * d->ow;
    p.gn_mom = (float*)d->gn_mom;
    p.gn_cpg = d->gn_mom ? d->cout / d->gn_groups : 0;
    if (p.M <= 0) return C2D_OK;

    const int amode = (d->ksize == 1) ? AM_1X1 : ((cin % 64) == 0 ? AM_3X3_FAST : AM_3X3_GEN);
    const bool dma = dma_eligible(d);
    p.ksplit = 1;
    p.nkt = d->kpad / 64;
    p.ws = nullptr;
    p.slab16 = tuning().splitk_f16;
    p.abl = gemm_abl();
    p.lds_epi = (gemm_lds_epi() || !epi_direct_ok(d)) ? 1 : 0;
    p.cmajor = gemm_korder();
    const long t128 = (long)((p.M + 127) / 128) * ((d->cout + 127) / 128);
    if (dma) {
        DmaPlan pl = fixed ? *fixed : plan_for(p.M, d->cout, d->kpad, d->act, pps_eligible(d), d->ksize, rr_eligible(d), panel_eligible(d));
        if (d->pro == C2D_PRO_LNFOLD) pl = {70, 1, d->kpad / 64};
        if (pl.split > 1) {
            const size_t need = (size_t)pl.split * p.M * d->cout * sizeof(float);
            if (d->ws && d->ws_bytes >= need && aligned16(d->ws)) {
                p.ws = (float*)d->ws;
            } else {
                pl.split = 1;
                pl.nkt = d->kpad / 64;
            }
        }
        dispatch_dma(p, pl, d->ksize, d->cout, s);
    } else if (t128 < 512) {
        p.gx = (d->cout + 63) / 64; p.gy = (p.M + 63) / 64;
        if (amode == AM_1X1) launch<64, 64, AM_1X1>(p, s);
        else if (amode == AM_3X3_FAST) launch<64, 64, AM_3X3_FAST>(p, s);
        else launch<64, 64, AM_3X3_GEN>(p, s);
    } else {
        p.gx = (d->cout + 127) / 128; p.gy = (p.M + 127) / 128;
        if (amode == AM_1X1) launch<128, 128, AM_1X1>(p, s);
        else if (amode == AM_3X3_FAST) launch<128, 128, AM_3X3_FAST>(p, s);
        else launch<128, 128, AM_3X3_GEN>(p, s);
    }
    return check_launch();
}

#endif
```

clap2diffusion_amd/csrc/igemm_m32.h:

```cpp
#pragma once

namespace c2d {

template <int BK, int SW = 0>
__device__ __forceinline__ int sw_of(int row) {
    if (BK == 64) return (row >> 1) & 7;
    if (SW == 1) return (0x78 >> (2 * ((row >> 2) & 3))) & 3;
    return (row >> 2) & 3;
}
template <int BK, int SW = 0>
__device__ __forceinline__ int lds_sw(int row, int c) {
    return row * (2 * BK) + ((c ^ sw_of<BK, SW>(row)) << 4);
}

template <int BM, int BN, int BK, int NW, int KS, int SW = 0, bool PRE = false>
struct M32Loader {
    static constexpr int RB = 2 * BK, RPP = 1024 / RB, CPR = BK / 8;
    static constexpr int NA = BM / RPP, NB = BN / RPP;
    static constexpr int SA = NA / NW;
    static constexpr int SB = (NB + NW - 1) / NW;
    static_assert(NA % NW == 0, "A pieces must split evenly over the waves");
    int a_pix[PRE ? 1 : SA];
    unsigned a_off0[PRE ? SA : 1], a_off1[PRE ? SA : 1];
    unsigned a_mask[SA];
    unsigned b_off[SB];
    unsigned bytes0, bytes1, wbytes;
    const char *u_src0, *u_src1, *u_wt;
    int pshift, tap, cbase, lrow, lchunk, cin_;
    bool two, ctail, cbase_major;

    static constexpr int PMIN = SA + NB / NW, PMAX = SA + SB;
    __device__ __forceinline__ static int pieces(int wave) {
        return SA + (NB / NW) + (((NB % NW) != 0 && wave < (NB % NW)) ? 1 : 0);
    }
    __device__ __forceinline__ int row_of(int wave, int i) const { return (wave + i * NW) * RPP + lrow; }
    __device__ __forceinline__ int chunk_of(int row) const { return (lchunk ^ sw_of<BK, SW>(row)) * 8; }

    __device__ __forceinline__ void init(const IgemmParams& p, int m0, int n0, int wave, int lane, int kb) {
        lrow = lane / CPR;
        lchunk = lane % CPR;
        const int hw = p.oh * p.ow;
        two = p.c1 > 0;
        pshift = KS == 3 ? p.w + 1 : 0;
#pragma unroll
        for (int i = 0; i < SA; ++i) {
            const int m = m0 + row_of(wave, i);
            const int mm = m < p.M ? m : 0;
            const int nn = mm / hw, r = mm - nn * hw;
            const int oy = r / p.ow, ox = r - oy * p.ow;
            const int iy0 = oy * p.stride - p.pad, ix0 = ox * p.stride - p.pad;
            unsigned mask = 0;
            if (m < p.M) {
#pragma unroll
                for (int ky = 0; ky < KS; ++ky)
#pragma unroll
                    for (int kx = 0; kx < KS; ++kx)
                        if (iy0 + ky >= 0 && iy0 + ky < p.h && ix0 + kx >= 0 && ix0 + kx < p.w)
                            mask |= 1u << (ky * KS + kx);
            }
            const int pix = (nn * p.h + iy0) * p.w + ix0 + pshift;
            if constexpr (PRE) {
                const int ch = chunk_of(row_of(wave, i));
                a_off0[i] = (unsigned)(2 * (pix * p.c0 + ch));
                a_off1[i] = (unsigned)(2 * (pix * p.c1 + ch));
            } else {
                a_pix[i] = pix;
            }
            a_mask[i] = mask;
        }
#pragma unroll
        for (int i = 0; i < SB; ++i) {
            const int row = row_of(wave, i);
            const int j = n0 + row;
            b_off[i] = (row < BN && j < p.cout) ? (unsigned)(2 * (j * p.kpad + chunk_of(row))) : kOOB;
        }
        const size_t npix = (size_t)p.n * p.h * p.w;
        bytes0 = (unsigned)(npix * p.c0 * 2);
        bytes1 = (unsigned)(npix * p.c1 * 2);
        wbytes = (unsigned)((size_t)p.cout * p.kpad * 2);
        ctail = (p.cin % BK) != 0;
        cin_ = p.cin;
        cbase_major = p.cmajor != 0;
        u_src0 = uniform_ptr(p.src0);
        u_src1 = uniform_ptr(p.src1);
        u_wt = uniform_ptr(p.wt);
        cbase = kb * BK;
        tap = 0;
        if (KS == 3) {
            if (p.cmajor) { tap = kb % 9; cbase = (kb / 9) * BK; }
            else { tap = cbase / p.cin; cbase -= tap * p.cin; }
        }
    }

    struct Stage {
        __amdgpu_buffer_rsrc_t ra, rb;
        int cs, lim, tap;
        bool use1;
    };
    __device__ __forceinline__ Stage prep(const IgemmParams& p) const { return prep_at(p, tap, cbase); }
    __device__ __forceinline__ Stage prep_at(const IgemmParams& p, int tap, int cbase) const {
        Stage st;
        const int k0 = tap * p.cin + cbase;
        const int ky = tap / 3, kx = tap - (tap / 3) * 3;
        const bool use1 = two && cbase >= p.c0;
        st.cs = use1 ? p.c1 : p.c0;
        const unsigned sterm = 2u * (unsigned)((KS == 3 ? (ky * p.w + kx) * st.cs : 0) + (use1 ? cbase - p.c0 : cbase));
        const char* sb = use1 ? u_src1 : u_src0;
        const unsigned bias = 2u * (unsigned)(pshift * st.cs);
        const unsigned sbytes = use1 ? bytes1 : bytes0;
        st.ra = make_rsrc(sb + sterm - bias, sbytes + bias - sterm);
        st.rb = make_rsrc(u_wt + 2 * k0, wbytes - 2 * k0);
        st.lim = p.cin - cbase;
        st.tap = tap;
        st.use1 = use1;
        return st;
    }
    __device__ __forceinline__ void piece(const Stage& st, char* lds, int wave, int i) const {
        if (i < SA) {
            const int ch = chunk_of(row_of(wave, i));
            unsigned ok = (a_mask[i] >> st.tap) & 1u;
            if (ctail) ok &= (unsigned)(ch < st.lim);
            unsigned off;
            if constexpr (PRE) off = (st.use1 ? a_off1[i] : a_off0[i]) | ((ok - 1u) & kOOB);
            else off = (unsigned)(2 * (a_pix[i] * st.cs + ch)) | ((ok - 1u) & kOOB);
            dma_piece(st.ra, lds + (wave + i * NW) * 1024, off);
        } else {
            const int j = i - SA;
            if (j == SB - 1 && (NB % NW) != 0 && wave >= (NB % NW)) return;
            dma_piece(st.rb, lds + BM * RB + (wave + j * NW) * 1024, b_off[j]);
        }
    }
    __device__ __forceinline__ void advance() {
        if (KS == 3 && cbase_major) {
            if (++tap == 9) { tap = 0; cbase += BK; }
        } else {
            cbase += BK;
            if (KS == 3 && cbase >= cin_) { cbase = 0; ++tap; }
        }
    }

    __device__ __forceinline__ void issue(const IgemmParams& p, int kt, char* lds, int wave) {
        (void)kt;
        const Stage st = prep(p);
#pragma unroll
        for (int i = 0; i < PMAX; ++i) piece(st, lds, wave, i);
        advance();
    }
};

template <int N>
__device__ __forceinline__ void wait_vm_c() {
    static_assert(N >= 0 && N < 64, "vmcnt range");
    __builtin_amdgcn_s_waitcnt((N & 15) | (7 << 4) | (15 << 8) | ((N >> 4) << 14));
}

__device__ __forceinline__ void wait_vm(int n) {
#define C2D_WVM(N) case N: __builtin_amdgcn_s_waitcnt(((N) & 15) | (7 << 4) | (15 << 8) | (((N) >> 4) << 14)); break;
    switch (n) {
        C2D_WVM(1) C2D_WVM(2) C2D_WVM(3) C2D_WVM(4) C2D_WVM(5) C2D_WVM(6) C2D_WVM(7) C2D_WVM(8) C2D_WVM(9)
        C2D_WVM(10) C2D_WVM(11) C2D_WVM(12) C2D_WVM(13) C2D_WVM(14) C2D_WVM(15) C2D_WVM(16) C2D_WVM(18)
        C2D_WVM(20) C2D_WVM(21) C2D_WVM(24) C2D_WVM(27) C2D_WVM(28) C2D_WVM(30) C2D_WVM(32) C2D_WVM(36)
        C2D_WVM(40) C2D_WVM(42) C2D_WVM(45) C2D_WVM(48) C2D_WVM(54) C2D_WVM(56) C2D_WVM(60)
        default: __builtin_amdgcn_s_waitcnt((7 << 4) | (15 << 8)); break;
    }
#undef C2D_WVM
}

template <int TM, int TN>
__device__ __forceinline__ void epilogue32_lds(const IgemmParams& p, const f32x16 (&acc)[TN][TM], int mw0, int nw0,
                                               int lane, int wave, char* lds) {
    constexpr int G = TN < 3 ? TN : 3;
    constexpr int PITCHF = G * 32 + 4;
    float* img = reinterpret_cast<float*>(lds) + wave * 32 * PITCHF;
    const int lr = lane & 31, lh = lane >> 5;
    if (!p.resid && !p.temb) {
#pragma unroll
        for (int b = 0; b < TM; ++b) {
#pragma unroll
            for (int a0 = 0; a0 < TN; a0 += G) {
#pragma unroll
                for (int a = a0; a < a0 + G && a < TN; ++a)
#pragma unroll
                    for (int g = 0; g < 4; ++g) {
                        const f32x4 v = {acc[a][b][4 * g], acc[a][b][4 * g + 1], acc[a][b][4 * g + 2], acc[a][b][4 * g + 3]};
                        *reinterpret_cast<f32x4*>(img + lr * PITCHF + (a - a0) * 32 + g * 8 + lh * 4) = v;
                    }
                __builtin_amdgcn_s_waitcnt(15 | (7 << 4) | (0 << 8) | (3 << 14));
                __builtin_amdgcn_wave_barrier();
                const int nt = (a0 + G <= TN) ? G : TN - a0;
                if (nt == 3) epi_rows_plain<32, 96>(p, img, PITCHF, mw0 + b * 32, nw0 + a0 * 32, lane);
                else if (nt == 2) epi_rows_plain<32, 64>(p, img, PITCHF, mw0 + b * 32, nw0 + a0 * 32, lane);
                else epi_rows_plain<32, 32>(p, img, PITCHF, mw0 + b * 32, nw0 + a0 * 32, lane);
                __builtin_amdgcn_s_waitcnt(15 | (7 << 4) | (0 << 8) | (3 << 14));
                __builtin_amdgcn_wave_barrier();
            }
        }
        return;
    }
    static_for<0, TM * ((TN + G - 1) / G)>([&](auto pass) __attribute__((always_inline)) {
        constexpr int b = decltype(pass)::value / ((TN + G - 1) / G);
        constexpr int a0 = (decltype(pass)::value % ((TN + G - 1) / G)) * G;
        constexpr int nt = (a0 + G <= TN) ? G : TN - a0;
        auto write_img = [&]() __attribute__((always_inline)) {
#pragma unroll
            for (int a = a0; a < a0 + nt; ++a)
#pragma unroll
                for (int g = 0; g < 4; ++g) {
                    const f32x4 bv = bias4(p, nw0 + a * 32 + g * 8 + lh * 4);
                    const f32x4 v = {acc[a][b][4 * g], acc[a][b][4 * g + 1], acc[a][b][4 * g + 2], acc[a][b][4 * g + 3]};
                    *reinterpret_cast<f32x4*>(img + lr * PITCHF + (a - a0) * 32 + g * 8 + lh * 4) = v + bv;
                }
        };
        epi_pass<32, nt * 32, true>(p, img, PITCHF, mw0 + b * 32, nw0 + a0 * 32, lane, write_img);
    });
}

template <int TM, int TN, int ACT>
__device__ __forceinline__ void epilogue32_direct(const IgemmParams& p, const f32x16 (&acc)[TN][TM], int mw0,
                                                  int nw0, int lane) {
    typedef _Float16 h4 __attribute__((ext_vector_type(4)));
    constexpr bool GG = ACT == C2D_ACT_GEGLU;
    const int lh = lane >> 5;
    const int hw = p.oh * p.ow;
    const int out_cols = GG ? (p.cout >> 1) : p.cout;
#pragma unroll
    for (int b = 0; b < TM; ++b) {
        const int m = mw0 + b * 32 + (lane & 31);
        if (m >= p.M) continue;
        const f16* trow = p.temb ? p.temb + (size_t)(m / hw) * p.temb_ld : nullptr;
        const f16* rrow = p.resid ? p.resid + (size_t)m * p.resid_ld : nullptr;
        f16* orow = p.out + (size_t)m * p.out_ld;
#pragma unroll
        for (int a = 0; a < TN; ++a) {
            const int jb = nw0 + a * 32;
#pragma unroll
            for (int g = 0; g < (GG ? 2 : 4); ++g) {
                const int jp = jb + g * 8 + 4 * lh;
                const int j = GG ? (jb >> 1) + g * 8 + 4 * lh : jp;
                if (j >= out_cols) continue;
                float v[4] = {acc[a][b][4 * g], acc[a][b][4 * g + 1], acc[a][b][4 * g + 2], acc[a][b][4 * g + 3]};
                if (p.bias) {
                    const float4 bb = *reinterpret_cast<const float4*>(p.bias + jp);
                    v[0] += bb.x; v[1] += bb.y; v[2] += bb.z; v[3] += bb.w;
                }
                if constexpr (GG) {
                    float gt[4] = {acc[a][b][4 * g + 8], acc[a][b][4 * g + 9], acc[a][b][4 * g + 10], acc[a][b][4 * g + 11]};
                    if (p.bias) {
                        const float4 bb = *reinterpret_cast<const float4*>(p.bias + jp + 16);
                        gt[0] += bb.x; gt[1] += bb.y; gt[2] += bb.z; gt[3] += bb.w;
                    }
#pragma unroll
                    for (int r = 0; r < 4; ++r) v[r] *= gelu_sig(gt[r]);
                }
                if (trow) {
                    const h4 t = *reinterpret_cast<const h4*>(trow + j);
#pragma unroll
                    for (int r = 0; r < 4; ++r) v[r] += (float)t[r];
                }
                if (rrow) {
                    const h4 t = *reinterpret_cast<const h4*>(rrow + j);
#pragma unroll
                    for (int r = 0; r < 4; ++r) v[r] += (float)t[r];
                }
                h4 o;
#pragma unroll
                for (int r = 0; r < 4; ++r) o[r] = (f16)v[r];
                *reinterpret_cast<h4*>(orow + j) = o;
            }
        }
    }
}

template <int WM, int WN, int TM, int TN, int BK, int STAGES, int KS, int DB, int WPE = 0, int EACT = -1>
__global__ void __launch_bounds__(64 * WM * WN) __attribute__((amdgpu_waves_per_eu(WPE > 0 ? WPE : 1)))
igemm_m32_kernel(IgemmParams p) {
    constexpr int NW = WM * WN;
    constexpr int BM = WM * TM * 32, BN = WN * TN * 32;
    constexpr int RB = 2 * BK, STAGE = (BM + BN) * RB, NS = BK / 16;
    typedef M32Loader<BM, BN, BK, NW, KS> Loader;
    extern __shared__ __attribute__((aligned(16))) char smem[];

    const int tid = threadIdx.x, lane = tid & 63;
    const int wave = __builtin_amdgcn_readfirstlane(tid >> 6);
    const int wm = wave / WN, wn = wave - (wave / WN) * WN;
    const int bid = xcd_remap(blockIdx.x, p.gx * p.gy * p.ksplit);
    const int tile = bid / p.ksplit, slice = bid - tile * p.ksplit;
    const int mt = tile / p.gx, nt = tile - mt * p.gx;
    const int m0 = mt * BM, n0 = nt * BN;
    const int nk_all = p.kpad / BK;
    const int kb = slice * p.nkt, ke = min(nk_all, kb + p.nkt);
// ... 199 lines not shown
```

clap2diffusion_amd/csrc/igemm_pp16.h:

```cpp
#pragma once

#ifndef C2D_PP16_PH
#define C2D_PP16_PH 0
#endif
#ifndef C2D_PP16_LGKM_ALL
#define C2D_PP16_LGKM_ALL 1
#endif

namespace c2d {

template <int TN, int KS, int PH>
__global__ void __launch_bounds__(512) igemm_pp16_kernel(IgemmParams p) {
    constexpr int BK = 64, NW = 8, TMW = 8;
    constexpr int BM = 2 * TMW * 16, BN = 4 * TN * 16;
    constexpr int RB = 2 * BK, STAGE = (BM + BN) * RB;
    typedef M32Loader<BM, BN, BK, NW, KS> Loader;
    constexpr int P = Loader::PMAX;
    static_assert(Loader::PMIN == P, "every wave deals the same pieces");
    constexpr int RT = PH == 4 ? 4 : 8;
    static_assert(PH == 2 || PH == 4, "pp16 phases per K step");
    constexpr int PPH = (P + PH - 2) / (PH - 1);
    extern __shared__ __attribute__((aligned(16))) char smem[];

    const int tid = threadIdx.x, lane = tid & 63;
    const int wave = __builtin_amdgcn_readfirstlane(tid >> 6);
    const int wr = wave >> 2, wc = wave & 3;
    const int bid = xcd_remap(blockIdx.x, p.gx * p.gy * p.ksplit);
    const int tile = bid / p.ksplit, slice = bid - tile * p.ksplit;
    const int mt = tile / p.gx, nt = tile - mt * p.gx;
    const int m0 = mt * BM, n0 = nt * BN;
    const int nk_all = p.kpad / BK;
    const int kb = slice * p.nkt, ke = min(nk_all, kb + p.nkt);

    Loader ld;
    ld.init(p, m0, n0, wave, lane, kb);
    const int fo0 = lds_sw<BK>(lane & 15, lane >> 4), fo1 = lds_sw<BK>(lane & 15, 4 + (lane >> 4));
    const int a_base = wr * TMW * 16 * RB, b_base = BM * RB + wc * TN * 16 * RB;

    f32x4 acc[TN][TMW];
#pragma unroll
    for (int a = 0; a < TN; ++a)
#pragma unroll
        for (int b = 0; b < TMW; ++b) acc[a][b] = (f32x4){0.f, 0.f, 0.f, 0.f};

#define C2D_BAR() do { asm volatile("" ::: "memory"); __builtin_amdgcn_s_barrier(); asm volatile("" ::: "memory"); } while (0)
    if (kb < ke) ld.issue(p, kb, smem + (kb & 1) * STAGE, wave);
    wait_vm_c<0>();
    C2D_BAR();
    if (wr) C2D_BAR();

    f16x8 fa[RT], fb[TN];
    for (int kt = kb; kt < ke; ++kt) {
        const char* S = smem + (kt & 1) * STAGE;
        char* Wn = smem + ((kt + 1) & 1) * STAGE;
        const bool nxt = kt + 1 < ke;
        typename Loader::Stage st = ld.prep(p);
#pragma unroll
        for (int q = 0; q < PH; ++q) {
            const int ks = PH == 4 ? q >> 1 : q, rh = PH == 4 ? q & 1 : 0;
            const int fo = ks ? fo1 : fo0;
            if (rh == 0) {
#pragma unroll
                for (int t = 0; t < TN; ++t) fb[t] = *reinterpret_cast<const f16x8*>(S + b_base + t * 16 * RB + fo);
            }
#pragma unroll
            for (int t = 0; t < RT; ++t)
                fa[t] = *reinterpret_cast<const f16x8*>(S + a_base + (rh * 4 + t) * 16 * RB + fo);
            if (q < PH - 1 && nxt && !C2D_ABL(p.abl, 1)) {
#pragma unroll
                for (int i = 0; i < PPH; ++i)
                    if (q * PPH + i < P) ld.piece(st, Wn, wave, q * PPH + i);
            }
            if (q == PH - 1 && nxt) wait_vm_c<0>();
            if (q == PH - 1 || C2D_PP16_LGKM_ALL)
                __builtin_amdgcn_s_waitcnt(15 | (7 << 4) | (0 << 8) | (3 << 14));
            C2D_BAR();
            if (C2D_ABL(p.abl, 2)) {
#pragma unroll
                for (int t = 0; t < RT; ++t) asm volatile("" :: "v"(fa[t]));
#pragma unroll
                for (int t = 0; t < TN; ++t) asm volatile("" :: "v"(fb[t]));
            } else {
                __builtin_amdgcn_s_setprio(1);
#pragma unroll
                for (int b = 0; b < RT; ++b)
#pragma unroll
                    for (int a = 0; a < TN; ++a)
                        acc[a][rh * 4 + b] = __builtin_amdgcn_mfma_f32_16x16x32_f16(fb[a], fa[b], acc[a][rh * 4 + b], 0, 0, 0);
                __builtin_amdgcn_s_setprio(0);
            }
            C2D_BAR();
        }
        if (nxt) ld.advance();
    }
    if (!wr) C2D_BAR();
#undef C2D_BAR

    const int mw0 = m0 + wr * TMW * 16, nw0 = n0 + wc * TN * 16;
    if (C2D_ABL(p.abl, 4)) {
#pragma unroll
        for (int a = 0; a < TN; ++a)
#pragma unroll
            for (int b = 0; b < TMW; ++b) asm volatile("" :: "v"(acc[a][b]));
        return;
    }
    if (p.ksplit > 1) {
#pragma unroll
        for (int b = 0; b < TMW; ++b) {
            const int m = mw0 + b * 16 + (lane & 15);
#pragma unroll
            for (int a = 0; a < TN; ++a) {
                const int j = nw0 + a * 16 + 4 * (lane >> 4);
                if (m < p.M && j < p.cout) store_partial(p, slice, m, j, acc[a][b]);
            }
        }
        return;
    }
    __syncthreads();
    if (!p.resid && !p.temb) {
        constexpr int PITCHF = TN * 16 + 4;
        float* img = reinterpret_cast<float*>(smem) + wave * 32 * PITCHF;
#pragma unroll
        for (int b0 = 0; b0 < TMW; b0 += 2) {
#pragma unroll
            for (int bb = 0; bb < 2; ++bb)
#pragma unroll
                for (int a = 0; a < TN; ++a)
                    *reinterpret_cast<f32x4*>(img + (bb * 16 + (lane & 15)) * PITCHF + a * 16 + 4 * (lane >> 4)) =
                        acc[a][b0 + bb];
            __builtin_amdgcn_s_waitcnt(15 | (7 << 4) | (0 << 8) | (3 << 14));
            __builtin_amdgcn_wave_barrier();
            epi_rows_plain<32, TN * 16>(p, img, PITCHF, mw0 + b0 * 16, nw0, lane);
            __builtin_amdgcn_s_waitcnt(15 | (7 << 4) | (0 << 8) | (3 << 14));
            __builtin_amdgcn_wave_barrier();
        }
    } else if (TN == 5 && p.gn_mom) {
        constexpr int BN = 4 * TN * 16, PITCHB = BN + 4;
        float* img = reinterpret_cast<float*>(smem);
        const int wr0 = wr * 32, wc0 = wc * TN * 16;
        epi_gn_moments<TMW / 2, 64, BN, BM, TMW * 16>(p, img, PITCHB, m0, n0, tid, [&](auto pass) __attribute__((always_inline)) {
            constexpr int b0 = 2 * decltype(pass)::value;
            f32x4 bv[TN];
#pragma unroll
            for (int a = 0; a < TN; ++a) bv[a] = bias4(p, nw0 + a * 16 + 4 * (lane >> 4));
#pragma unroll
            for (int bb = 0; bb < 2; ++bb)
#pragma unroll
                for (int a = 0; a < TN; ++a)
                    *reinterpret_cast<f32x4*>(img + (wr0 + bb * 16 + (lane & 15)) * PITCHB + wc0 + a * 16 +
                                              4 * (lane >> 4)) = acc[a][b0 + bb] + bv[a];
        });
    } else {
        constexpr int BN = 4 * TN * 16, PITCHB = BN + 4;
        float* img = reinterpret_cast<float*>(smem);
        const int wr0 = wr * 32, wc0 = wc * TN * 16;
        static_for<0, TMW / 2>([&](auto pass) __attribute__((always_inline)) {
            constexpr int b0 = 2 * decltype(pass)::value;
            epi_pass<64, BN, true, 512, TMW * 16>(p, img, PITCHB, m0 + b0 * 16, n0, tid, [&]() __attribute__((always_inline)) {
                f32x4 bv[TN];
#pragma unroll
                for (int a = 0; a < TN; ++a) bv[a] = bias4(p, nw0 + a * 16 + 4 * (lane >> 4));
#pragma unroll
                for (int bb = 0; bb < 2; ++bb)
#pragma unroll
                    for (int a = 0; a < TN; ++a)
                        *reinterpret_cast<f32x4*>(img + (wr0 + bb * 16 + (lane & 15)) * PITCHB + wc0 + a * 16 +
                                                  4 * (lane >> 4)) = acc[a][b0 + bb] + bv[a];
            });
        });
    }
}

template <int TN, int KS>
static void launch_pp16(const IgemmParams& p, hipStream_t s) {
    constexpr int PH = C2D_PP16_PH ? C2D_PP16_PH : ((KS == 1 || TN == 4) ? 2 : 4);
    constexpr int ring = 2 * (256 + 4 * TN * 16) * 128;
    constexpr int epi_wg = 64 * (4 * TN * 16 + 4) * 4, epi_wv = 8 * 32 * (TN * 16 + 4) * 4;
    constexpr int epi = epi_wg > epi_wv ? epi_wg : epi_wv;
    constexpr int smem = ring > epi ? ring : epi;
    static_assert(smem <= 160 * 1024, "LDS ring / epilogue image too large");
    auto k = igemm_pp16_kernel<TN, KS, PH>;
    ensure_lds<igemm_pp16_kernel<TN, KS, PH>>(smem);
    hipLaunchKernelGGL(k, dim3(p.gx * p.gy * p.ksplit), dim3(512), smem, s, p);
    if (p.ksplit > 1) run_splitk_reduce(p, s);
}

template <int TN>
static void run_pp16(IgemmParams& p, int ksize, int cout, hipStream_t s) {
    constexpr int BM = 256, BN = 4 * TN * 16;
    p.gx = (cout + BN - 1) / BN;
    p.gy = (p.M + BM - 1) / BM;
    if (ksize == 1) launch_pp16<TN, 1>(p, s);
    else launch_pp16<TN, 3>(p, s);
}

}
```

clap2diffusion_amd/layers.py:

```python
from __future__ import annotations

import torch
import torch.nn as nn

from . import ops


class HLinear(nn.Module):
    def __init__(self, in_features: int, out_features: int, bias: bool = True):
        super().__init__()
        self.in_features, self.out_features = in_features, out_features
        self.kpad = ops.kpad_of(in_features)
        self.register_buffer("weight", torch.zeros(out_features, self.kpad, dtype=torch.float16))
        self.register_buffer("bias", torch.zeros(out_features, dtype=torch.float32) if bias else None)

    @torch.no_grad()
    def load(self, w: torch.Tensor, b: torch.Tensor | None = None) -> None:
        wp, kp = ops.pack_linear_weight(w.float())
        assert kp == self.kpad and wp.shape[0] == self.out_features
        self.weight.copy_(wp)
        if self.bias is not None:
            self.bias.copy_(b.float() if b is not None else torch.zeros_like(self.bias))

    def forward(self, x: torch.Tensor, **kw) -> torch.Tensor:
        shp = x.shape
        x2 = x.reshape(-1, shp[-1])
        if not x2.is_contiguous():
            x2 = x2.contiguous()
        out = ops.conv(x2, self.weight, self.kpad, self.out_features, ksize=1, bias=self.bias, **kw)
        return out.view(*shp[:-1], out.shape[-1])


class HConv2d(nn.Module):

    def __init__(self, cin: int, cout: int, ksize: int, stride: int = 1, cin_pad: int | None = None):
        super().__init__()
        self.cin, self.cout, self.ksize, self.stride = cin, cout, ksize, stride
        self.cin_pad = cin_pad or cin
        self.kpad = ops.kpad_of(ksize * ksize * self.cin_pad)
        self.register_buffer("weight", torch.zeros(cout, self.kpad, dtype=torch.float16))
        self.register_buffer("bias", torch.zeros(cout, dtype=torch.float32))

    @torch.no_grad()
    def load(self, w: torch.Tensor, b: torch.Tensor | None) -> None:
        wp, kp = ops.pack_conv_weight(w.float(), cin_pad=self.cin_pad if self.cin_pad != self.cin else None)
        assert kp == self.kpad, (kp, self.kpad)
        self.weight.copy_(wp)
        if b is not None:
            self.bias.copy_(b.float())

    def forward(self, x: torch.Tensor, **kw) -> torch.Tensor:
        return ops.conv(x, self.weight, self.kpad, self.cout, ksize=self.ksize, stride=self.stride, bias=self.bias, **kw)


class HGroupNorm(nn.Module):

    def __init__(self, num_groups: int, num_channels: int, eps: float):
        super().__init__()
        self.num_groups, self.num_channels, self.eps = num_groups, num_channels, eps
        self.register_buffer("weight", torch.ones(num_channels))
        self.register_buffer("bias", torch.zeros(num_channels))

    @torch.no_grad()
    def load(self, w, b):
        self.weight.copy_(w.float())
        self.bias.copy_(b.float())

    def stats(self, x: torch.Tensor, x2: torch.Tensor | None = None):
        return ops.group_norm_stats(x, self.num_groups, self.eps, self.weight, self.bias, x2=x2)

    def apply(self, x: torch.Tensor, x2: torch.Tensor | None = None, silu: bool = False,
              pad: bool = False, mom=None) -> torch.Tensor:
        return ops.group_norm(x, self.num_groups, self.eps, self.weight, self.bias, silu, x2=x2, pad=pad, mom=mom)


class HLayerNorm(nn.Module):
    def __init__(self, c: int, eps: float = 1e-5):
        super().__init__()
        self.c, self.eps = c, eps
        self.register_buffer("weight", torch.ones(c))
        self.register_buffer("bias", torch.zeros(c))

    @torch.no_grad()
    def load(self, w, b):
        self.weight.copy_(w.float())
        self.bias.copy_(b.float())

    def forward(self, x: torch.Tensor) -> torch.Tensor:
        shp = x.shape
        return ops.layer_norm(x.reshape(-1, shp[-1]), self.weight, self.bias, self.eps).view(shp)

    def prologue(self, x2d: torch.Tensor):
        return ops.layer_norm_stats(x2d, self.eps), self.weight, self.bias


def load_tree(module: nn.Module, sd: dict, prefix: str = "") -> list[str]:
    used = []
    for name, m in module.named_modules():
        if isinstance(m, (HLinear, HConv2d, HGroupNorm, HLayerNorm)):
            key = (prefix + name) if name else prefix.rstrip(".")
            wk, bk = key + ".weight", key + ".bias"
            if wk not in sd:
                raise KeyError(f"missing weight {wk}")
            m.load(sd[wk], sd.get(bk))
            used.append(wk)
            if bk in sd:
                used.append(bk)
    return used
```

clap2diffusion_amd/ops.py:

```python
from __future__ import annotations

import ctypes
import functools
import math

import torch

from . import torch_ops
from ._lib import C2D_ACT

C2D = torch.ops.c2d

F16 = torch.float16


def _require(t: torch.Tensor, name: str) -> None:
    if not t.is_cuda:
        raise RuntimeError(f"{name} must be a device tensor (HIP path only, no CPU fallback)")


def kpad_of(k: int) -> int:
    return (k + 63) // 64 * 64


def pack_conv_weight(w: torch.Tensor, cin_pad: int | None = None) -> tuple[torch.Tensor, int]:
    cout, cin, kh, kw = w.shape
    if cin_pad and cin_pad > cin:
        w = torch.nn.functional.pad(w, (0, 0, 0, 0, 0, cin_pad - cin))
        cin = cin_pad
    k = kh * kw * cin
    wp = w.permute(0, 2, 3, 1).reshape(cout, k)
    kp = kpad_of(k)
    if kp > k:
        wp = torch.nn.functional.pad(wp, (0, kp - k))
    return wp.to(F16).contiguous(), kp


def pack_weights_device(w: torch.Tensor, cin_pad: int | None = None) -> tuple[torch.Tensor, int]:
    _require(w, "w")
    w = w.float().contiguous()
    cout, cin = w.shape[:2]
    ks = w.shape[2] if w.dim() == 4 else 1
    cp = max(cin_pad or cin, cin)
    kp = kpad_of(ks * ks * cp)
    out = torch.empty(cout, kp, device=w.device, dtype=F16)
    C2D.pack_weights(w, cout, cin, ks, cp, kp, out)
    return out, kp


def pack_linear_weight(w: torch.Tensor) -> tuple[torch.Tensor, int]:
    out_f, in_f = w.shape
    kp = kpad_of(in_f)
    wp = torch.nn.functional.pad(w, (0, kp - in_f)) if kp > in_f else w
    return wp.to(F16).contiguous(), kp


def geglu_interleave(w: torch.Tensor, b: torch.Tensor | None):
    two_i = w.shape[0]
    inner = two_i // 2
    assert inner % 16 == 0
    idx = torch.arange(two_i).view(2, inner // 16, 16).permute(1, 0, 2).reshape(-1)
    wi = w[idx]
    bi = b[idx] if b is not None else None
    return wi, bi


def conv(x: torch.Tensor, weight: torch.Tensor, kpad: int, cout: int, *, ksize: int, bias=None, stride: int = 1,
         up: bool = False, x2: torch.Tensor | None = None, gn=None, gn_silu: bool = False, ln=None,
         silu_in: bool = False, act: str | None = None, temb: torch.Tensor | None = None,
         resid: torch.Tensor | None = None, out: torch.Tensor | None = None, padded: bool = False,
         ln_fold=None, gn_moments: int = 0):
    _require(x, "x")
    if x.dim() == 2:
        h, w = 1, x.shape[0]
    else:
        _, h, w, _ = x.shape
        if padded:
            assert ksize == 3 and stride == 1 and not up and x2 is None, "padded source: 3x3, stride 1, one source"
            assert gn is None and ln is None and not silu_in, "padded source: no GN / LN / SiLU prologue"
            h, w = h - 2, w - 2
    assert x.is_contiguous() and x.dtype == F16
    if x2 is not None:
        assert x2.is_contiguous() and x2.dtype == F16 and x2.shape[:-1] == x.shape[:-1]
    if ksize == 3:
        vh, vw = (2 * h, 2 * w) if up else (h, w)
        oh, ow = (vh + 2 - 3) // stride + 1, (vw + 2 - 3) // stride + 1
    else:
        oh, ow = h, w
    out_cols = cout // 2 if act == "geglu" else cout
    if out is None:
        shape = (x.shape[0], out_cols) if x.dim() == 2 else (x.shape[0], oh, ow, out_cols)
        out = torch.empty(shape, device=x.device, dtype=F16)
    assert out.stride(-1) == 1
    if resid is not None:
        assert resid.stride(-1) == 1
    gs, gh = gn if gn is not None else (None, None)
    ls, lg, lb = ln if ln is not None else (None, None, None)
    mom, rows = None, 0
    if gn_moments and x.dim() == 4 and act is None and not up and out.is_contiguous():
        rows = gn_moment_rows(out.shape[0], oh, ow, x.shape[-1], cout, ksize, stride, bool(padded), resid is not None,
                              temb is not None, gn_moments, x2.shape[-1] if x2 is not None else 0)
        if rows:
            mom = torch.empty((out.shape[0], oh * ow // rows, gn_moments, 2), device=x.device, dtype=torch.float32)
    C2D.conv2d_igemm(x, weight, kpad, cout, ksize, stride, up, x2, gs, gh, gn_silu, ls, lg, lb, silu_in, bias,
                     C2D_ACT[act], temb, resid, out, bool(padded), float(ln_fold or 0.0), mom, int(gn_moments))
    if gn_moments:
        return out, (GnMoments(out, mom, rows, gn_moments) if mom is not None else None)
    return out


class GnMoments:

    def __init__(self, of: torch.Tensor, mom: torch.Tensor, rows: int, groups: int):
        self.of, self.mom, self.rows, self.groups = of, mom, rows, groups

    def matches(self, x: torch.Tensor, groups: int) -> bool:
        return (x is self.of and groups == self.groups and x.dim() == 4 and
                tuple(self.mom.shape[:1]) == tuple(x.shape[:1]))


@functools.lru_cache(maxsize=None)
def gn_moment_rows(n: int, oh: int, ow: int, cin: int, cout: int, ksize: int, stride: int, padded: bool, resid: bool,
                   temb: bool, groups: int, c1: int = 0) -> int:
    import ctypes
    from ._lib import ConvDesc, lib
    d = ConvDesc()
    h, w = (oh, ow) if padded or ksize == 1 or stride == 1 else (oh * stride, ow * stride)
    d.c0, d.n, d.h, d.w, d.oh, d.ow, d.ksize, d.stride, d.src_pad = cin, n, h, w, oh, ow, ksize, stride, int(padded)
    d.c1 = c1
    if c1:
        d.src1 = 256
    d.cout, d.kpad, d.out_ld = cout, kpad_of(ksize * ksize * (cin + c1)), cout
    d.out = 256
    if resid:
        d.resid, d.resid_ld = 256, cout
    if temb:
        d.temb, d.temb_ld = 256, cout
    d.ws, d.ws_bytes = 256, 1 << 40
    d.gn_groups = groups
    return int(lib().c2d_conv2d_gn_rows(ctypes.byref(d)))


@torch.no_grad()
def fold_layernorm(weight: torch.Tensor, bias: torch.Tensor | None, gamma: torch.Tensor, beta: torch.Tensor,
                   in_features: int):
    w = weight[:, :in_features].float()
    wp = torch.zeros_like(weight)
    wp[:, :in_features] = (w * gamma.float().view(1, -1)).to(F16)
    b = w @ beta.float()
    if bias is not None:
        b = b + bias.float()
    return wp.contiguous(), b.contiguous()


@functools.lru_cache(maxsize=None)
def panel_gemm(m: int, k: int, cout: int, geglu: bool, lnfold: bool = False) -> bool:
    import ctypes
    from ._lib import C2D_PRO_LNFOLD, ConvDesc, lib
    d = ConvDesc()
    d.c0, d.n, d.h, d.w, d.oh, d.ow, d.ksize, d.stride = k, 1, 1, m, 1, m, 1, 1
    d.cout, d.kpad, d.act = cout, kpad_of(k), C2D_ACT["geglu" if geglu else None]
    d.out_ld = cout // 2 if geglu else cout
    if lnfold:
        d.pro, d.pro_eps = C2D_PRO_LNFOLD, 1e-5
    tid, ks = ctypes.c_int(), ctypes.c_int()
    rc = lib().c2d_conv2d_igemm_plan(ctypes.byref(d), ctypes.byref(tid), ctypes.byref(ks))
    return rc == 0 and tid.value == 70


ROWRING_TILES = (42, 43, 44)


@functools.lru_cache(maxsize=None)
def rowring_conv(n: int, h: int, w: int, cin: int, cout: int) -> bool:
    import ctypes
    from ._lib import ConvDesc, check, lib
    d = ConvDesc()
    d.c0, d.n, d.h, d.w, d.oh, d.ow, d.ksize, d.stride = cin, n, h, w, h, w, 3, 1
    d.cout, d.kpad, d.src_pad = cout, kpad_of(9 * cin), 1
    d.out_ld = cout
    tid, ks = ctypes.c_int(), ctypes.c_int()
    check(lib().c2d_conv2d_igemm_plan(ctypes.byref(d), ctypes.byref(tid), ctypes.byref(ks)), "c2d_conv2d_igemm_plan")
    return tid.value in ROWRING_TILES


def conv_workspace_bytes(n: int, h: int, w: int, c0: int, c1: int, cout: int, ksize: int) -> int:
    import ctypes
    from ._lib import ConvDesc, lib
    d = ConvDesc()
    d.c0, d.c1, d.n, d.h, d.w, d.oh, d.ow, d.ksize, d.stride = c0, c1, n, h, w, h, w, ksize, 1
    d.cout, d.kpad, d.out_ld = cout, kpad_of(ksize * ksize * (c0 + c1)), cout
    return int(lib().c2d_conv2d_igemm_workspace_size(ctypes.byref(d)))


class record_conv_plans:

    def __enter__(self):
        self.plans = []
        torch_ops._plan_probe = self.plans
        return self.plans

    def __exit__(self, *exc):
        torch_ops._plan_probe = None
        return False


class force_plan:

    def __init__(self, tile: int, split: int = 0):
        self.tile, self.split = int(tile), int(split)

    def __enter__(self):
        import ctypes
        from ._lib import check, lib
        t, sp = ctypes.c_int(0), ctypes.c_int(0)
        check(lib().c2d_get_plan_override(ctypes.byref(t), ctypes.byref(sp)), "c2d_get_plan_override")
        self.prev = (t.value, sp.value)
        check(lib().c2d_set_plan_override(self.tile, self.split), "c2d_set_plan_override")
        rowring_conv.cache_clear()
        gn_moment_rows.cache_clear()
        return self

    def __exit__(self, *exc):
        from ._lib import lib
        lib().c2d_set_plan_override(*self.prev)
        rowring_conv.cache_clear()
        gn_moment_rows.cache_clear()
        return False


def plan_override_from_env() -> None:
    import os
    from ._lib import check, lib
    t, sp = int(os.environ.get("C2D_GEMM_TILE", "0") or 0), int(os.environ.get("C2D_GEMM_SPLIT", "0") or 0)
    if t or sp:
        check(lib().c2d_set_plan_override(t, sp), "c2d_set_plan_override")


def group_norm_stats(x: torch.Tensor, groups: int, eps: float, gamma: torch.Tensor, beta: torch.Tensor,
                     x2: torch.Tensor | None = None):
    _require(x, "x")
    c = x.shape[-1] + (x2.shape[-1] if x2 is not None else 0)
    scale = torch.empty((x.shape[0], c), device=x.device, dtype=torch.float32)
    shift = torch.empty_like(scale)
    C2D.groupnorm_stats(x, x2, groups, float(eps), gamma, beta, scale, shift)
    return scale, shift


def group_norm_apply(x: torch.Tensor, gn, silu: bool, x2: torch.Tensor | None = None,
                     out: torch.Tensor | None = None) -> torch.Tensor:
    _require(x, "x")
    c = x.shape[-1] + (x2.shape[-1] if x2 is not None else 0)
    if out is None:
        out = torch.empty((*x.shape[:-1], c), device=x.device, dtype=F16)
    C2D.groupnorm_apply(x, x2, gn[0], gn[1], bool(silu), out)
    return out


# ... 149 lines not shown
```

clap2diffusion_amd/torch_ops.py:

```python
import ctypes
from typing import Optional

import torch
from torch import Tensor
from torch.library import custom_op

from ._lib import C2D_PRO_GN, C2D_PRO_LN, C2D_PRO_LNFOLD, C2D_PRO_NONE, C2D_PRO_SILU, ConvDesc, check, lib, ptr, stream_ptr

_CU = "cuda"


def _conv_desc(x, weight, kpad, cout, ksize, stride, up, x2, gn_scale, gn_shift, gn_silu, ln_stats, ln_gamma,
               ln_beta, silu_in, bias, act, temb, resid, out, src_pad=False, lnf_eps=0.0, gn_mom=None,
               gn_groups=0) -> ConvDesc:
    if x.dim() == 2:
        n, h, w = 1, 1, x.shape[0]
        c0 = x.shape[1]
    else:
        n, h, w, c0 = x.shape
        if src_pad:
            h, w = h - 2, w - 2
    c1 = x2.shape[-1] if x2 is not None else 0
    if ksize == 3:
        vh, vw = (2 * h, 2 * w) if up else (h, w)
        oh, ow = (vh + 2 - 3) // stride + 1, (vw + 2 - 3) // stride + 1
    else:
        oh, ow = h, w
    d = ConvDesc()
    d.src0 = ptr(x); d.src1 = ptr(x2); d.c0 = c0; d.c1 = c1
    d.n, d.h, d.w, d.oh, d.ow = n, h, w, oh, ow
    d.ksize, d.stride, d.up = ksize, stride, int(up)
    d.weight = ptr(weight); d.cout = cout; d.kpad = kpad
    if lnf_eps > 0.0:
        d.pro = C2D_PRO_LNFOLD; d.pro_eps = lnf_eps
    elif gn_scale is not None:
        d.pro = C2D_PRO_GN; d.pro_silu = int(gn_silu); d.pro_a = ptr(gn_scale); d.pro_b = ptr(gn_shift)
    elif ln_stats is not None:
        d.pro = C2D_PRO_LN; d.pro_a = ptr(ln_stats); d.gamma = ptr(ln_gamma); d.beta = ptr(ln_beta)
    elif silu_in:
        d.pro = C2D_PRO_SILU
    else:
        d.pro = C2D_PRO_NONE
    d.bias = ptr(bias)
    d.act = act
    if temb is not None:
        d.temb = ptr(temb); d.temb_ld = temb.stride(0)
    if resid is not None:
        d.resid = ptr(resid); d.resid_ld = resid.stride(-2) if resid.dim() == 2 else resid.shape[-1]
    d.out = ptr(out)
    d.out_ld = out.stride(-2) if out.dim() == 2 else out.shape[-1]
    d.src_pad = int(src_pad)
    if gn_mom is not None:
        d.gn_mom = ptr(gn_mom); d.gn_groups = gn_groups
    return d


_plan_probe: Optional[list] = None


@custom_op("c2d::conv2d_igemm", mutates_args=("out",), device_types=_CU)
def conv2d_igemm(x: Tensor, weight: Tensor, kpad: int, cout: int, ksize: int, stride: int, up: bool,
                 x2: Optional[Tensor], gn_scale: Optional[Tensor], gn_shift: Optional[Tensor], gn_silu: bool,
                 ln_stats: Optional[Tensor], ln_gamma: Optional[Tensor], ln_beta: Optional[Tensor], silu_in: bool,
                 bias: Optional[Tensor], act: int, temb: Optional[Tensor], resid: Optional[Tensor],
                 out: Tensor, src_pad: bool = False, lnf_eps: float = 0.0, gn_mom: Optional[Tensor] = None,
                 gn_groups: int = 0) -> None:
    d = _conv_desc(x, weight, kpad, cout, ksize, stride, up, x2, gn_scale, gn_shift, gn_silu, ln_stats, ln_gamma,
                   ln_beta, silu_in, bias, act, temb, resid, out, src_pad, lnf_eps, gn_mom, gn_groups)
    wsb = lib().c2d_conv2d_igemm_workspace_size(ctypes.byref(d))
    if wsb:
        ws = torch.empty(wsb // 4, device=x.device, dtype=torch.float32)
        d.ws = ptr(ws); d.ws_bytes = wsb
    if _plan_probe is not None:
        tid, ks = ctypes.c_int(), ctypes.c_int()
        check(lib().c2d_conv2d_igemm_plan(ctypes.byref(d), ctypes.byref(tid), ctypes.byref(ks)), "c2d_conv2d_igemm_plan")
        _plan_probe.append((tid.value, ks.value))
    check(lib().c2d_conv2d_igemm(ctypes.byref(d), stream_ptr()), "c2d_conv2d_igemm")


@conv2d_igemm.register_fake
def _(x, weight, kpad, cout, ksize, stride, up, x2, gn_scale, gn_shift, gn_silu, ln_stats, ln_gamma, ln_beta,
      silu_in, bias, act, temb, resid, out, src_pad=False, lnf_eps=0.0, gn_mom=None, gn_groups=0):
    return None


@custom_op("c2d::pack_weights", mutates_args=("out",), device_types=_CU)
def pack_weights(w: Tensor, cout: int, cin: int, ksize: int, cin_pad: int, kpad: int, out: Tensor) -> None:
    check(lib().c2d_pack_weights(ptr(w), cout, cin, ksize, cin_pad, kpad, ptr(out), stream_ptr()), "c2d_pack_weights")


@custom_op("c2d::groupnorm_stats", mutates_args=("scale", "shift"), device_types=_CU)
def groupnorm_stats(x: Tensor, x2: Optional[Tensor], groups: int, eps: float, gamma: Tensor, beta: Tensor,
                    scale: Tensor, shift: Tensor) -> None:
    n, c0 = x.shape[0], x.shape[-1]
    c1 = x2.shape[-1] if x2 is not None else 0
    hw = x.numel() // (n * c0)
    ws = torch.empty(lib().c2d_groupnorm_workspace_size(n, c0 + c1, hw) // 4, device=x.device, dtype=torch.float32)
    check(lib().c2d_groupnorm_stats(ptr(x), ptr(x2), c0, c1, n, hw, groups, eps, ptr(gamma), ptr(beta), ptr(scale),
                                    ptr(shift), ptr(ws), stream_ptr()), "c2d_groupnorm_stats")


@custom_op("c2d::groupnorm_apply", mutates_args=("out",), device_types=_CU)
def groupnorm_apply(x: Tensor, x2: Optional[Tensor], scale: Tensor, shift: Tensor, silu: bool, out: Tensor) -> None:
    n, c0 = x.shape[0], x.shape[-1]
    c1 = x2.shape[-1] if x2 is not None else 0
    hw = x.numel() // (n * c0)
    check(lib().c2d_groupnorm_apply(ptr(x), ptr(x2), c0, c1, n, hw, ptr(scale), ptr(shift), int(silu), ptr(out),
                                    stream_ptr()), "c2d_groupnorm_apply")


@custom_op("c2d::groupnorm", mutates_args=("out",), device_types=_CU)
def groupnorm(x: Tensor, x2: Optional[Tensor], groups: int, eps: float, gamma: Tensor, beta: Tensor, silu: bool,
              out: Tensor) -> None:
    n, c0 = x.shape[0], x.shape[-1]
    c1 = x2.shape[-1] if x2 is not None else 0
    hw = x.numel() // (n * c0)
    wsb = lib().c2d_groupnorm_run_workspace_size(n, c0 + c1, hw, groups)
    ws = torch.empty((wsb + 15) // 16 * 4, device=x.device, dtype=torch.float32) if wsb else None
    check(lib().c2d_groupnorm(ptr(x), ptr(x2), c0, c1, n, hw, groups, eps, ptr(gamma), ptr(beta), int(silu), ptr(out),
                              ptr(ws), wsb, stream_ptr()), "c2d_groupnorm")


@custom_op("c2d::groupnorm_pad", mutates_args=("out",), device_types=_CU)
def groupnorm_pad(x: Tensor, x2: Optional[Tensor], groups: int, eps: float, gamma: Tensor, beta: Tensor, silu: bool,
                  out: Tensor) -> None:
    n, h, w, c0 = x.shape
    c1 = x2.shape[-1] if x2 is not None else 0
    wsb = lib().c2d_groupnorm_pad_workspace_size(n, c0 + c1, h, w)
    ws = torch.empty((wsb + 15) // 16 * 4, device=x.device, dtype=torch.float32)
    check(lib().c2d_groupnorm_pad(ptr(x), ptr(x2), c0, c1, n, h, w, groups, eps, ptr(gamma), ptr(beta), int(silu),
                                  ptr(out), ptr(ws), wsb, stream_ptr()), "c2d_groupnorm_pad")


@custom_op("c2d::groupnorm_moments", mutates_args=("out",), device_types=_CU)
def groupnorm_moments(x: Tensor, groups: int, eps: float, gamma: Tensor, beta: Tensor, silu: bool, mom: Tensor,
                      rows: int, pad: bool, out: Tensor) -> None:
    n, h, w, c = x.shape
    check(lib().c2d_groupnorm_moments(ptr(x), c, n, h * w, groups, eps, ptr(gamma), ptr(beta), int(silu), ptr(mom),
                                      rows, w + 2 if pad else 0, ptr(out), stream_ptr()), "c2d_groupnorm_moments")


@custom_op("c2d::layernorm_stats", mutates_args=("stats",), device_types=_CU)
def layernorm_stats(x: Tensor, eps: float, stats: Tensor) -> None:
    m, c = x.shape
    check(lib().c2d_layernorm_stats(ptr(x), m, c, x.stride(0), eps, ptr(stats), stream_ptr()), "c2d_layernorm_stats")


@custom_op("c2d::layernorm", mutates_args=("out",), device_types=_CU)
def layernorm(x: Tensor, gamma: Tensor, beta: Tensor, eps: float, out: Tensor) -> None:
    m, c = x.shape
    check(lib().c2d_layernorm(ptr(x), m, c, x.stride(0), eps, ptr(gamma), ptr(beta), ptr(out), out.stride(0),
                              stream_ptr()), "c2d_layernorm")


@custom_op("c2d::attention_fwd", mutates_args=("out",), device_types=_CU)
def attention_fwd(q: Tensor, k: Tensor, v: Tensor, batch: int, heads: int, lq: int, lk: int, d: int, scale: float,
                  key_bias: Optional[Tensor], bias_ld_batch: int, bias_ld_head: int, out: Tensor,
                  bias_ld_query: int = 0) -> None:
    if key_bias is None:
        check(lib().c2d_attention_fwd(ptr(q), q.stride(0), ptr(k), k.stride(0), ptr(v), v.stride(0), ptr(out),
                                      out.stride(0), batch, heads, lq, lk, d, scale, 1, stream_ptr()), "c2d_attention_fwd")
    else:
        check(lib().c2d_attention_fwd_mask(ptr(q), q.stride(0), ptr(k), k.stride(0), ptr(v), v.stride(0), ptr(out),
                                           out.stride(0), batch, heads, lq, lk, d, scale, 1, ptr(key_bias),
                                           bias_ld_batch, bias_ld_head, bias_ld_query, stream_ptr()),
              "c2d_attention_fwd_mask")


@custom_op("c2d::attention_small", mutates_args=("out",), device_types=_CU)
def attention_small(q: Tensor, k: Tensor, v: Tensor, batch: int, heads: int, l: int, d: int, scale: float,
                    causal: bool, out: Tensor) -> None:
    check(lib().c2d_attention_small(ptr(q), q.stride(0), ptr(k), k.stride(0), ptr(v), v.stride(0), ptr(out),
                                    out.stride(0), batch, heads, l, d, scale, int(causal), stream_ptr()),
          "c2d_attention_small")


@custom_op("c2d::window_attention", mutates_args=("out",), device_types=_CU)
def window_attention(qkv: Tensor, row_map: Tensor, n_windows: int, heads: int, d: int, bias: Tensor,
                     mask: Optional[Tensor], out: Tensor) -> None:
    n_mask = mask.shape[0] if mask is not None else 0
    check(lib().c2d_window_attention(ptr(qkv), qkv.stride(0), ptr(row_map), n_windows, heads, d, ptr(bias), ptr(mask),
                                     n_mask, ptr(out), out.stride(0), stream_ptr()), "c2d_window_attention")


@custom_op("c2d::htsat_mel_patches", mutates_args=("out",), device_types=_CU)
def htsat_mel_patches(mel: Tensor, bn_scale: Tensor, bn_shift: Tensor, out: Tensor) -> None:
    b, t, _ = mel.shape
    check(lib().c2d_htsat_mel_patches(ptr(mel), b, t, ptr(bn_scale), ptr(bn_shift), ptr(out), stream_ptr()),
          "c2d_htsat_mel_patches")


@custom_op("c2d::patch_merge_gather", mutates_args=("out",), device_types=_CU)
def patch_merge_gather(x: Tensor, b: int, h: int, w: int, c: int, out: Tensor) -> None:
    check(lib().c2d_patch_merge_gather(ptr(x), b, h, w, c, ptr(out), stream_ptr()), "c2d_patch_merge_gather")


@custom_op("c2d::row_mean", mutates_args=("out",), device_types=_CU)
def row_mean(x: Tensor, b: int, rows: int, out: Tensor) -> None:
    check(lib().c2d_row_mean(ptr(x), b, rows, x.shape[1], x.stride(0), ptr(out), stream_ptr()), "c2d_row_mean")


@custom_op("c2d::softmax_rows", mutates_args=("out",), device_types=_CU)
def softmax_rows(x: Tensor, out: Tensor) -> None:
    check(lib().c2d_softmax_rows(ptr(x), x.shape[0], x.shape[1], x.stride(0), ptr(out), out.stride(0), stream_ptr()),
          "c2d_softmax_rows")


@custom_op("c2d::l2_normalize", mutates_args=("x",), device_types=_CU)
def l2_normalize(x: Tensor) -> None:
    m, c = x.shape
    check(lib().c2d_l2_normalize(ptr(x), m, c, stream_ptr()), "c2d_l2_normalize")


@custom_op("c2d::clap_log_mel", mutates_args=("out",), device_types=_CU)
def clap_log_mel(wave: Tensor, offsets: Tensor, lengths: Tensor, max_len: int, n_fft: int, hop: int, window: Tensor,
                 filters: Tensor, filter_range: Tensor, n_mels: int, out: Tensor) -> None:
    check(lib().c2d_clap_log_mel(ptr(wave), ptr(offsets), ptr(lengths), offsets.numel(), max_len, n_fft, hop,
                                 ptr(window), ptr(filters), ptr(filter_range), n_mels, ptr(out), stream_ptr()),
          "c2d_clap_log_mel")


@custom_op("c2d::timestep_embedding", mutates_args=("out",), device_types=_CU)
def timestep_embedding(t_table: Tensor, step_index: Optional[Tensor], n: int, dim: int, out: Tensor) -> None:
    check(lib().c2d_timestep_embedding(ptr(t_table), ptr(step_index), n, dim, ptr(out), stream_ptr()),
          "c2d_timestep_embedding")


@custom_op("c2d::cfg_ddim_step", mutates_args=("x", "step_index"), device_types=_CU)
def cfg_ddim_step(eps: Tensor, x: Tensor, guidance: float, coef: Tensor, step_index: Tensor, advance: bool) -> None:
    b, c, hgt, wid = x.shape
    check(lib().c2d_cfg_ddim_step(ptr(eps), ptr(x), b, c, hgt * wid, guidance, ptr(coef), ptr(step_index), int(advance),
                                  stream_ptr()), "c2d_cfg_ddim_step")


@custom_op("c2d::latent_to_nhwc", mutates_args=("out",), device_types=_CU)
# ... 28 lines not shown
```

clap2diffusion_amd/unet.py:

```python
from __future__ import annotations

import os

import torch
import torch.nn as nn

from . import ops
from .layers import HConv2d, HGroupNorm, HLayerNorm, HLinear
from .processor import AttnProcessor, AudioAttnProcessor
from .weights import SD15_UNET

FOLD_FF_OUT = os.environ.get("C2D_FOLD_FF_OUT", "1") != "0"
FOLD_LN = os.environ.get("C2D_LN_FOLD", "1") != "0"
FOLD_LN640 = os.environ.get("C2D_LN_FOLD640", "1") != "0"
GN_MOMENTS = os.environ.get("C2D_GN_MOMENTS", "1") != "0"
GN_GROUPS = 32
CFG_PREFIX_MIN = int(os.environ.get("C2D_CFG_PREFIX_MIN", "1"))


class Attention(nn.Module):

    def __init__(self, query_dim: int, cross_attention_dim: int | None = None, heads: int = 8,
                 dim_head: int | None = None, out_bias: bool = True):
        super().__init__()
        dim_head = dim_head or query_dim // heads
        inner = heads * dim_head
        ctx = cross_attention_dim or query_dim
        self.heads, self.dim_head = heads, dim_head
        self.scale = dim_head ** -0.5
        self.is_cross_attention = cross_attention_dim is not None
        self.to_q = HLinear(query_dim, inner, bias=False)
        self.to_k = HLinear(ctx, inner, bias=False)
        self.to_v = HLinear(ctx, inner, bias=False)
        self.to_out = nn.ModuleList([HLinear(inner, query_dim, bias=out_bias), nn.Dropout(0.0)])
        self.spatial_norm = None
        self.norm_cross = None
        self.residual_connection = False
        self.rescale_output_factor = 1.0
        self.upcast_attention = False
        self.upcast_softmax = False
        self.kpad_q = self.to_q.kpad
        self.kpad_kv = self.to_k.kpad
        self.register_buffer("w_qkv", None if self.is_cross_attention else
                             torch.zeros(3 * inner, self.kpad_q, dtype=torch.float16), persistent=False)
        self.register_buffer("w_kv", torch.zeros(2 * inner, self.kpad_kv, dtype=torch.float16), persistent=False)
        self.processor = AttnProcessor()

    @torch.no_grad()
    def finalize(self):
        self.w_kv.copy_(torch.cat([self.to_k.weight, self.to_v.weight], 0))
        if self.w_qkv is not None:
            self.w_qkv.copy_(torch.cat([self.to_q.weight, self.to_k.weight, self.to_v.weight], 0))

    def set_processor(self, processor) -> None:
        self.processor = processor

    def forward(self, hidden_states, encoder_hidden_states=None, attention_mask=None, **cross_attention_kwargs):
        return self.processor(self, hidden_states, encoder_hidden_states=encoder_hidden_states,
                              attention_mask=attention_mask, **cross_attention_kwargs)

    def head_to_batch_dim(self, tensor: torch.Tensor, out_dim: int = 3) -> torch.Tensor:
        b, l, dim = tensor.shape
        h = self.heads
        t = tensor.reshape(b, l, h, dim // h).permute(0, 2, 1, 3)
        return t.reshape(b * h, l, dim // h) if out_dim == 3 else t

    def batch_to_head_dim(self, tensor: torch.Tensor) -> torch.Tensor:
        bh, l, d = tensor.shape
        h = self.heads
        return tensor.reshape(bh // h, h, l, d).permute(0, 2, 1, 3).reshape(bh // h, l, d * h)

    def get_attention_scores(self, query, key, attention_mask=None):
        scores = torch.baddbmm(torch.empty(query.shape[0], query.shape[1], key.shape[1], dtype=query.dtype,
                                           device=query.device), query, key.transpose(-1, -2), beta=0,
                               alpha=self.scale)
        if attention_mask is not None:
            scores = scores + attention_mask
        return scores.softmax(dim=-1).to(query.dtype)


class FeedForward(nn.Module):

    def __init__(self, dim: int, mult: int = 4):
        super().__init__()
        inner = dim * mult
        self.net = nn.ModuleList([nn.Module(), nn.Dropout(0.0), HLinear(inner, dim)])
        self.net[0].proj = HLinear(dim, 2 * inner)

    @torch.no_grad()
    def load_geglu(self, w, b):
        wi, bi = ops.geglu_interleave(w.float(), b.float())
        self.net[0].proj.load(wi, bi)


class BasicTransformerBlock(nn.Module):
    def __init__(self, dim: int, heads: int, cross_dim: int):
        super().__init__()
        self.norm1 = HLayerNorm(dim)
        self.attn1 = Attention(dim, None, heads)
        self.norm2 = HLayerNorm(dim)
        self.attn2 = Attention(dim, cross_dim, heads)
        self.norm3 = HLayerNorm(dim)
        self.ff = FeedForward(dim)
        self.lnf = dim in (320, 640)
        self.lnf_folded = False
        for name in ("qkv", "q", "ff"):
            self.register_buffer(f"lnf_{name}_w", None, persistent=False)
            self.register_buffer(f"lnf_{name}_b", None, persistent=False)

    @torch.no_grad()
    def finalize(self) -> None:
        if not (self.lnf and FOLD_LN):
            return
        c = self.norm1.c
        wq = torch.cat([self.attn1.to_q.weight, self.attn1.to_k.weight, self.attn1.to_v.weight], 0)
        for name, w, b, norm in (("qkv", wq, None, self.norm1), ("q", self.attn2.to_q.weight, None, self.norm2),
                                 ("ff", self.ff.net[0].proj.weight, self.ff.net[0].proj.bias, self.norm3)):
            wf, bf = ops.fold_layernorm(w, b, norm.weight, norm.bias, c)
            setattr(self, f"lnf_{name}_w", wf.contiguous())
            setattr(self, f"lnf_{name}_b", bf.contiguous())
        self.lnf_folded = True

    def _lnf_on(self, m: int, cout: int, geglu: bool) -> bool:
        c = self.norm1.c
        if not (self.lnf_folded and ops.panel_gemm(m, c, cout, geglu, lnfold=True)):
            return False
        if ops.panel_gemm(m, c, cout, geglu) or (c == 320 and m >= 8192):
            return True
        if c == 640 and m >= 8192 and FOLD_LN640:
            panels = (m + 127) // 128
            ns = min(max((256 + panels - 1) // panels, 1), ((cout >> 5) + 7) // 8)
            return panels * ns <= 256
        return False

    def _attend(self, attn: Attention, x, h, ehs, mask, kwargs):
        if getattr(attn.processor, "fuses_residual", False):
            return attn(x, encoder_hidden_states=ehs, attention_mask=mask, _residual=h, **kwargs)
        out = attn(x, encoder_hidden_states=ehs, attention_mask=mask, **kwargs)
        return ops.add(out.to(h.dtype).contiguous(), h)

    def forward(self, h: torch.Tensor, ehs: torch.Tensor, cross_attention_kwargs: dict,
                encoder_attention_mask: torch.Tensor | None = None,
                cfg_dup: torch.Tensor | None = None) -> torch.Tensor:
        h = self.forward_attn(h, ehs, cross_attention_kwargs, encoder_attention_mask, cfg_dup)
        b, l, c = h.shape
        h2 = h.view(b * l, c)
        self.ff.net[2](self.ff_inner(h2), resid=h2, out=h2)
        return h

    def ff_inner(self, h2: torch.Tensor) -> torch.Tensor:
        proj = self.ff.net[0].proj
        if self._lnf_on(h2.shape[0], proj.out_features, True):
            return ops.conv(h2, self.lnf_ff_w, proj.kpad, proj.out_features, ksize=1, bias=self.lnf_ff_b,
                            act="geglu", ln_fold=self.norm3.eps)
        return proj(self.norm3(h2), act="geglu")

    def forward_attn(self, h: torch.Tensor, ehs: torch.Tensor, cross_attention_kwargs: dict,
                     encoder_attention_mask: torch.Tensor | None = None,
                     cfg_dup: torch.Tensor | None = None) -> torch.Tensor:
        kw = cross_attention_kwargs or {}
        b, l, c = h.shape
        inner = self.attn1.heads * self.attn1.dim_head
        if type(self.attn1.processor) is AttnProcessor and self._lnf_on(b * l, 3 * inner, False):
            qkv = ops.conv(h.view(b * l, c), self.lnf_qkv_w, self.attn1.kpad_q, 3 * inner, ksize=1,
                           bias=self.lnf_qkv_b, ln_fold=self.norm1.eps)
            h = self._attend(self.attn1, h, h, None, None, dict(kw, _qkv=qkv))
        else:
            h = self._attend(self.attn1, self.norm1(h), h, None, None, kw)
        if cfg_dup is not None:
            n = h.shape[0]
            if h.data_ptr() != cfg_dup.data_ptr():
                cfg_dup[:n].copy_(h)
            cfg_dup[n:].copy_(cfg_dup[:n])
            h = cfg_dup
        b, l, c = h.shape
        if type(self.attn2.processor) in (AttnProcessor, AudioAttnProcessor) and self._lnf_on(b * l, inner, False):
            q = ops.conv(h.view(b * l, c), self.lnf_q_w, self.attn2.kpad_q, inner, ksize=1, bias=self.lnf_q_b,
                         ln_fold=self.norm2.eps)
            return self._attend(self.attn2, h, h, ehs, encoder_attention_mask, dict(kw, _q=q))
        return self._attend(self.attn2, self.norm2(h), h, ehs, encoder_attention_mask, kw)


class Transformer2DModel(nn.Module):
    def __init__(self, c: int, heads: int, cross_dim: int, groups: int = 32):
        super().__init__()
        self.norm = HGroupNorm(groups, c, 1e-6)
        self.proj_in = HConv2d(c, c, 1)
        self.transformer_blocks = nn.ModuleList([BasicTransformerBlock(c, heads, cross_dim)])
        self.proj_out = HConv2d(c, c, 1)
        self.fold_kpad = ops.kpad_of(5 * c)
        self.fold_ok = c % 64 == 0
        self.register_buffer("w_out_fold", torch.zeros(c, self.fold_kpad, dtype=torch.float16), persistent=False)
        self.register_buffer("b_out_fold", torch.zeros(c, dtype=torch.float32), persistent=False)

    @torch.no_grad()
    def finalize(self) -> None:
        for blk in self.transformer_blocks:
            blk.finalize()
        if not self.fold_ok:
            return
        c = self.proj_out.cout
        wp = self.proj_out.weight[:, :c].float()
        ff2 = self.transformer_blocks[0].ff.net[2]
        w2 = ff2.weight[:, :4 * c].float()
        self.w_out_fold.copy_(torch.cat([wp, wp @ w2], 1).to(torch.float16))
        self.b_out_fold.copy_(wp @ ff2.bias.float() + self.proj_out.bias.float())

    def _block_out(self, t: torch.Tensor, x4: torch.Tensor, resid: torch.Tensor, gm: int = 0):
        blk = self.transformer_blocks[0]
        b, l, c = t.shape
        hh, ww = x4.shape[1], x4.shape[2]
        t2 = t.view(b * l, c)
        ff1 = blk.ff_inner(t2)
        r = ops.conv(t2.view(b, hh, ww, c), self.w_out_fold, self.fold_kpad, c, ksize=1, bias=self.b_out_fold,
                     x2=ff1.view(b, hh, ww, ff1.shape[-1]), resid=resid.reshape(b, hh, ww, c),
                     gn_moments=gm)
        return r

    def forward(self, x, ehs, cross_attention_kwargs, encoder_attention_mask=None,
                cfg_dup: torch.Tensor | None = None, x_mom=None, want_mom: bool = False):
        gm = GN_GROUPS if want_mom and GN_MOMENTS else 0
        r = self._forward(x, ehs, cross_attention_kwargs, encoder_attention_mask, cfg_dup, x_mom, gm)
        if want_mom and not gm:
            return r, None
        return r

    def _forward(self, x, ehs, cross_attention_kwargs, encoder_attention_mask, cfg_dup, x_mom, gm):
        n, hh, ww, c = x.shape
        blk = self.transformer_blocks[0]
        fold = FOLD_FF_OUT and self.fold_ok
        if cfg_dup is None:
            h = self.proj_in(self.norm.apply(x, mom=x_mom))
            if fold:
                t = blk.forward_attn(h.view(n, hh * ww, c), ehs, cross_attention_kwargs, encoder_attention_mask)
                return self._block_out(t, x, x, gm)
            t = blk(h.view(n, hh * ww, c), ehs, cross_attention_kwargs, encoder_attention_mask)
            return self.proj_out(t.view(n, hh, ww, c), resid=x, gn_moments=gm)
        hb = x.new_empty((2 * n, hh * ww, c))
        h = self.proj_in(self.norm.apply(x, mom=x_mom), out=hb[:n].view(n, hh, ww, c))
        if fold:
            t = blk.forward_attn(h.view(n, hh * ww, c), ehs, cross_attention_kwargs, encoder_attention_mask,
                                 cfg_dup=hb)
            cfg_dup[n:].copy_(cfg_dup[:n])
            return self._block_out(t, cfg_dup, cfg_dup, gm)
        t = blk(h.view(n, hh * ww, c), ehs, cross_attention_kwargs, encoder_attention_mask, cfg_dup=hb)
        cfg_dup[n:].copy_(cfg_dup[:n])
        return self.proj_out(t.view(2 * n, hh, ww, c), resid=cfg_dup, gn_moments=gm)


class ResnetBlock2D(nn.Module):
    def __init__(self, cin: int, cout: int, temb_ch: int = 1280, groups: int = 32, eps: float = 1e-5):
        super().__init__()
        self.cin, self.cout = cin, cout
        self.norm1 = HGroupNorm(groups, cin, eps)
        self.conv1 = HConv2d(cin, cout, 3)
        self.time_emb_proj = HLinear(temb_ch, cout) if temb_ch else None
        self.norm2 = HGroupNorm(groups, cout, eps)
        self.dropout = nn.Dropout(0.0)
        self.conv2 = HConv2d(cout, cout, 3)
        self.conv_shortcut = HConv2d(cin, cout, 1) if cin != cout else None
        self.temb_off = None

    def forward(self, x, temb_all=None, skip=None, out=None, x_mom=None, want_mom: bool = False):
        temb = None
        if temb_all is not None:
            temb = temb_all[:, self.temb_off:self.temb_off + self.cout]
        n, hh, ww, _ = x.shape
        cin = self.cin
        p1 = ops.rowring_conv(n, hh, ww, cin, self.cout)
        a1 = self.norm1.apply(x, skip, silu=True, pad=p1, mom=x_mom if skip is None else None)
        if GN_MOMENTS:
            h, hm = self.conv1(a1, temb=temb, padded=p1, gn_moments=self.norm2.num_groups)
        else:
            h, hm = self.conv1(a1, temb=temb, padded=p1), None
        res = self.conv_shortcut(x, x2=skip) if self.conv_shortcut is not None else x
        p2 = ops.rowring_conv(n, hh, ww, self.cout, self.cout)
        y = self.conv2(self.norm2.apply(h, silu=True, pad=p2, mom=hm), resid=res, out=out, padded=p2,
                       gn_moments=self.norm2.num_groups if want_mom and GN_MOMENTS else 0)
        return (y, None) if want_mom and not GN_MOMENTS else y


class Downsample2D(nn.Module):
    def __init__(self, c):
        super().__init__()
        self.conv = HConv2d(c, c, 3, stride=2)

    def forward(self, x, want_mom: bool = False):
        if want_mom and GN_MOMENTS:
            return self.conv(x, gn_moments=GN_GROUPS)
        return (self.conv(x), None) if want_mom else self.conv(x)


class Upsample2D(nn.Module):
    def __init__(self, c):
        super().__init__()
        self.conv = HConv2d(c, c, 3)

    def forward(self, x):
        return self.conv(ops.upsample_nearest2x(x))


class _Block(nn.Module):
    def __init__(self):
        super().__init__()
        self.resnets = nn.ModuleList()
        self.attentions = nn.ModuleList()


class TimestepEmbedding(nn.Module):
    def __init__(self, cin: int, dim: int):
        super().__init__()
        self.linear_1 = HLinear(cin, dim)
        self.linear_2 = HLinear(dim, dim)

    def forward(self, t_sin):
        return self.linear_2(self.linear_1(t_sin, act="silu"))


class UNetOutput:
    def __init__(self, sample):
        self.sample = sample

    def __getitem__(self, i):
        return (self.sample,)[i]


class UNet2DConditionModel(nn.Module):
    def __init__(self, cfg: dict = SD15_UNET):
        super().__init__()
        self.cfg = dict(cfg)
        ch = cfg["block_out_channels"]
        heads, ctx, groups = cfg["heads"], cfg["cross_attention_dim"], cfg["norm_groups"]
        temb_ch = ch[0] * 4
        self.in_pad = 8
        self.conv_in = HConv2d(cfg["in_channels"], ch[0], 3, cin_pad=self.in_pad)
        self.time_embedding = TimestepEmbedding(ch[0], temb_ch)
        self.down_blocks = nn.ModuleList()
        out_c = ch[0]
        for i, c in enumerate(ch):
            blk = _Block()
            in_c, out_c = out_c, c
            for j in range(cfg["layers_per_block"]):
                blk.resnets.append(ResnetBlock2D(in_c if j == 0 else out_c, out_c, temb_ch, groups))
                if cfg["attn_blocks"][i]:
                    blk.attentions.append(Transformer2DModel(out_c, heads, ctx, groups))
            if i < len(ch) - 1:
                blk.downsamplers = nn.ModuleList([Downsample2D(out_c)])
            self.down_blocks.append(blk)
        self.mid_block = _Block()
        self.mid_block.resnets.append(ResnetBlock2D(ch[-1], ch[-1], temb_ch, groups))
        self.mid_block.attentions.append(Transformer2DModel(ch[-1], heads, ctx, groups))
        self.mid_block.resnets.append(ResnetBlock2D(ch[-1], ch[-1], temb_ch, groups))
        self.up_blocks = nn.ModuleList()
        rev = list(reversed(ch))
        rev_attn = list(reversed(cfg["attn_blocks"]))
        out_c = rev[0]
        n_up = cfg["layers_per_block"] + 1
        for i in range(len(rev)):
            blk = _Block()
            prev_c, out_c = out_c, rev[i]
            in_c = rev[min(i + 1, len(rev) - 1)]
            for j in range(n_up):
                skip = in_c if j == n_up - 1 else out_c
                r_in = prev_c if j == 0 else out_c
                blk.resnets.append(ResnetBlock2D(r_in + skip, out_c, temb_ch, groups))
                blk.resnets[-1].skip_ch = skip
                if rev_attn[i]:
                    blk.attentions.append(Transformer2DModel(out_c, heads, ctx, groups))
            if i < len(rev) - 1:
                blk.upsamplers = nn.ModuleList([Upsample2D(out_c)])
            self.up_blocks.append(blk)
        self.conv_norm_out = HGroupNorm(groups, ch[0], cfg["norm_eps"])
        self.conv_out = HConv2d(ch[0], cfg["out_channels"], 3)
        resnets = [m for m in self.modules() if isinstance(m, ResnetBlock2D)]
        off = 0
        for r in resnets:
            r.temb_off = off
            off += r.cout
        self.temb_total = off
        kp = ops.kpad_of(temb_ch)
        self.register_buffer("w_temb_all", torch.zeros(off, kp, dtype=torch.float16), persistent=False)
        self.register_buffer("b_temb_all", torch.zeros(off, dtype=torch.float32), persistent=False)
        self.temb_kpad = kp

    @torch.no_grad()
    def load_diffusers_state_dict(self, sd: dict) -> None:
        used = set()
        for name, m in self.named_modules():
            if isinstance(m, FeedForward):
                k = name + ".net.0.proj"
                m.load_geglu(sd[k + ".weight"], sd[k + ".bias"])
                used |= {k + ".weight", k + ".bias"}
        for name, m in self.named_modules():
            if isinstance(m, (HLinear, HConv2d, HGroupNorm, HLayerNorm)):
                if name.endswith("net.0.proj"):
                    continue
                wk, bk = name + ".weight", name + ".bias"
                m.load(sd[wk], sd.get(bk))
                used |= {wk, bk}
        missing = [k for k in sd if k not in used]
        if missing:
            raise KeyError(f"unused checkpoint keys: {missing[:5]} ...")
        self.finalize()

    @torch.no_grad()
    def finalize(self) -> None:
        for m in self.modules():
            if isinstance(m, (Attention, Transformer2DModel)):
                m.finalize()
        rs = [m for m in self.modules() if isinstance(m, ResnetBlock2D)]
        self.w_temb_all.copy_(torch.cat([r.time_emb_proj.weight for r in rs], 0))
        self.b_temb_all.copy_(torch.cat([r.time_emb_proj.bias for r in rs], 0))

    @property
    def attn_processors(self) -> dict:
        return {f"{n}.processor": m.processor for n, m in self.named_modules() if isinstance(m, Attention)}

    def set_attn_processor(self, processor) -> None:
        for n, m in self.named_modules():
            if isinstance(m, Attention):
                m.set_processor(processor[f"{n}.processor"] if isinstance(processor, dict) else processor)

    def time_conditioning(self, t_sin: torch.Tensor) -> torch.Tensor:
        temb = self.time_embedding(t_sin)
        return ops.conv(temb, self.w_temb_all, self.temb_kpad, self.temb_total, ksize=1, bias=self.b_temb_all,
                        silu_in=True)

    def cfg_shared_prefix_ok(self) -> bool:
        blk = self.down_blocks[0]
        if not len(blk.attentions):
            return False
        return type(blk.attentions[0].transformer_blocks[0].attn1.processor) is AttnProcessor

    def forward_nhwc(self, x: torch.Tensor, t_sin: torch.Tensor | None, ehs: torch.Tensor,
                     cross_attention_kwargs: dict | None = None,
                     encoder_attention_mask: torch.Tensor | None = None,
                     temb_all: torch.Tensor | None = None, cfg_pair: bool = False) -> torch.Tensor:
        kw = cross_attention_kwargs or {}
        em = encoder_attention_mask
        if temb_all is None:
            temb_all = self.time_conditioning(t_sin)
        shared = cfg_pair and x.shape[0] >= CFG_PREFIX_MIN and self.cfg_shared_prefix_ok()
        if cfg_pair and not shared:
            x = torch.cat([x, x], 0)
        if shared:
            n0 = x.shape[0]
            skip0 = x.new_empty((2 * n0, x.shape[1], x.shape[2], self.conv_in.cout))
            h = self.conv_in(x, out=skip0[:n0])
            skip0[n0:].copy_(skip0[:n0])
            skips = [skip0]
        else:
# ... 54 lines not shown
```

Measured before the change: 9.303 images/sec.

## Fold nearest-2x upsample into four-phase 2x2 convolutions in upsample blocks

Replaces upsample-nearest-then-3x3-conv in the UNet Upsample2D blocks with four sub-pixel phase convolutions. Each phase uses a 2x2 kernel whose weights are precomputed sums of the original 3x3 taps, and reads the low-resolution input directly. This drops the materialised upsampled tensor and cuts the MACs per output from 9*cin to 4*cin. The cost is extra kernel template instantiations (KS=2), scattered output-row addressing, a folded split-k reduce path, and tile-planner restrictions for the folded case.

```diff
diff --git a/clap2diffusion_amd/csrc/common.h b/clap2diffusion_amd/csrc/common.h
--- a/clap2diffusion_amd/csrc/common.h
+++ b/clap2diffusion_amd/csrc/common.h
@@ -53,6 +53,9 @@
 #endif
 #ifndef C2D_TUNE_TAIL_SPLIT
 #define C2D_TUNE_TAIL_SPLIT 1
+#endif
+#ifndef C2D_TUNE_UPFOLD
+#define C2D_TUNE_UPFOLD 1
 #endif
 #ifndef C2D_TUNE_PANEL_REGB
 #define C2D_TUNE_PANEL_REGB 0
diff --git a/clap2diffusion_amd/csrc/epilogue.h b/clap2diffusion_amd/csrc/epilogue.h
--- a/clap2diffusion_amd/csrc/epilogue.h
+++ b/clap2diffusion_amd/csrc/epilogue.h
@@ -51,7 +51,8 @@
         }
     }
 
-    __device__ __forceinline__ static void body(const IgemmParams& p, const float* img, int pitchf, int row, int sc,
+    template <class P>
+    __device__ __forceinline__ static void body(const P& p, const float* img, int pitchf, int row, int sc,
                                                 int m, int j, bool ok, const hv& rr, const hv& tt) {
         const float* src = img + row * pitchf + sc;
         float v[W];
@@ -90,7 +91,7 @@
         hv o;
 #pragma unroll
         for (int q = 0; q < W; ++q) o[q] = (f16)v[q];
-        if (ok) *reinterpret_cast<hv*>(p.out + (size_t)m * p.out_ld + j) = o;
+        if (ok) *reinterpret_cast<hv*>(p.out + out_row(p, m) * p.out_ld + j) = o;
         if constexpr (WB) {
             float* dst = const_cast<float*>(src);
 #pragma unroll
@@ -99,7 +100,8 @@
         }
     }
 
-    __device__ __forceinline__ void finish(const IgemmParams& p, const float* img, int pitchf, int m0, int jp0,
+    template <class P>
+    __device__ __forceinline__ void finish(const P& p, const float* img, int pitchf, int m0, int jp0,
                                            int lane) const {
 #pragma unroll
         for (int it = 0; it < NIT; ++it) {
@@ -110,7 +112,8 @@
         }
     }
 
-    __device__ __forceinline__ static void compact(const IgemmParams& p, const float* img, int pitchf, int m0,
+    template <class P>
+    __device__ __forceinline__ static void compact(const P& p, const float* img, int pitchf, int m0,
                                                    int jp0, int lane) {
         const int hw = p.oh * p.ow;
         const int n_all = (RG == 0 && (hw % ROWS) == 0) ? m0 / hw : -1;
@@ -128,8 +131,8 @@
     }
 };
 
-template <bool COMPACT, int NT, int RG, int W, bool GG, int ROWS, int COLS, int RES, int TEMB, class WriteImg>
-__device__ __forceinline__ void epi_pass_t(const IgemmParams& p, const float* img, int pitchf, int m0, int jp0,
+template <bool COMPACT, int NT, int RG, int W, bool GG, int ROWS, int COLS, int RES, int TEMB, class P, class WriteImg>
+__device__ __forceinline__ void epi_pass_t(const P& p, const float* img, int pitchf, int m0, int jp0,
                                            int lane, WriteImg&& write_img) {
     typedef EpiPass<W, GG, ROWS, COLS, RES, TEMB, NT, RG> EP;
     auto sync = [&]() __attribute__((always_inline)) {
@@ -215,8 +218,8 @@
     }
 }
 
-template <int ROWS, int COLS, bool COMPACT, int NT = 64, int RG = 0, class WriteImg>
-__device__ __forceinline__ void epi_pass(const IgemmParams& p, const float* img, int pitchf, int m0, int jp0,
+template <int ROWS, int COLS, bool COMPACT, int NT = 64, int RG = 0, class P, class WriteImg>
+__device__ __forceinline__ void epi_pass(const P& p, const float* img, int pitchf, int m0, int jp0,
                                          int lane, WriteImg&& w) {
     const bool gg = p.act == C2D_ACT_GEGLU;
     const int out_cols = gg ? (p.cout >> 1) : p.cout;
@@ -257,8 +260,8 @@
     return *reinterpret_cast<const f32x4*>(p.bias + j);
 }
 
-template <int W, bool GG, int ROWS, int COLS>
-__device__ __forceinline__ void epi_rows_plain_t(const IgemmParams& p, const float* img, int pitchf, int m0, int jp0,
+template <int W, bool GG, int ROWS, int COLS, class P>
+__device__ __forceinline__ void epi_rows_plain_t(const P& p, const float* img, int pitchf, int m0, int jp0,
                                            int lane) {
     typedef _Float16 hv __attribute__((ext_vector_type(W)));
     constexpr int CPR = GG ? COLS / (2 * W) : COLS / W;
@@ -336,12 +339,12 @@
         hv o;
 #pragma unroll
         for (int r = 0; r < W; ++r) o[r] = (f16)v[r];
-        *reinterpret_cast<hv*>(p.out + (size_t)m * p.out_ld + j) = o;
-    }
-}
-
-template <int ROWS, int COLS>
-__device__ __forceinline__ void epi_rows_plain(const IgemmParams& p, const float* img, int pitchf, int m0, int jp0,
+        *reinterpret_cast<hv*>(p.out + out_row(p, m) * p.out_ld + j) = o;
+    }
+}
+
+template <int ROWS, int COLS, class P>
+__device__ __forceinline__ void epi_rows_plain(const P& p, const float* img, int pitchf, int m0, int jp0,
                                          int lane) {
     const bool gg = p.act == C2D_ACT_GEGLU;
     const int out_cols = gg ? (p.cout >> 1) : p.cout;
diff --git a/clap2diffusion_amd/csrc/igemm.hip b/clap2diffusion_amd/csrc/igemm.hip
--- a/clap2diffusion_amd/csrc/igemm.hip
+++ b/clap2diffusion_amd/csrc/igemm.hip
@@ -40,8 +40,46 @@
     int gn_cpg;
 };
 
-__device__ __forceinline__ void store_partial(const IgemmParams& p, int slice, int m, int j, const f32x4& v) {
-    const size_t off = ((size_t)slice * p.M + m) * p.cout + j;
+struct IgemmParamsFold : IgemmParams {
+    int ph;
+    float rcp_w;
+};
+
+__device__ __forceinline__ size_t out_row(const IgemmParams&, int m) { return (size_t)m; }
+__device__ __forceinline__ size_t out_row_ph(const IgemmParams& p, int m, int ph, float rcp_w) {
+    int q = (int)((float)m * rcp_w);
+    int r = m - q * p.w;
+    if (r < 0) { --q; r += p.w; }
+    if (r >= p.w) { ++q; r -= p.w; }
+    return (size_t)((2 * q + (ph >> 1)) * 2 * p.w + 2 * r + (ph & 1));
+}
+__device__ __forceinline__ size_t out_row(const IgemmParamsFold& p, int m) { return out_row_ph(p, m, p.ph, p.rcp_w); }
+
+template <bool FOLD>
+struct KernelParams {
+    const IgemmParams& p;
+    __device__ __forceinline__ explicit KernelParams(const IgemmParams& k) : p(k) {}
+};
+template <>
+struct KernelParams<true> {
+    IgemmParamsFold p;
+    __device__ __forceinline__ explicit KernelParams(const IgemmParams& k) {
+        static_cast<IgemmParams&>(p) = k;
+        p.ph = 0;
+        p.rcp_w = 1.0f / (float)k.w;
+    }
+    __device__ __forceinline__ int set_phase(int mt) {
+        p.ph = mt & 3;
+        p.wt += (size_t)p.ph * p.cout * p.kpad;
+        return mt >> 2;
+    }
+};
+
+template <class P>
+__device__ __forceinline__ void store_partial(const P& p, int slice, int m, int j, const f32x4& v) {
+    size_t row = (size_t)slice * p.M + m;
+    if constexpr (std::is_same<P, IgemmParamsFold>::value) row = ((size_t)slice * 4 + p.ph) * p.M + m;
+    const size_t off = row * p.cout + j;
     if (p.slab16) {
         const f16x4 h = {(f16)v[0], (f16)v[1], (f16)v[2], (f16)v[3]};
         *reinterpret_cast<f16x4*>(reinterpret_cast<f16*>(p.ws) + off) = h;
@@ -184,7 +222,7 @@
                 f16x4 o;
 #pragma unroll
                 for (int r = 0; r < 4; ++r) o[r] = (f16)v[r];
-                if (mok[b] && cok[a]) *reinterpret_cast<f16x4*>(p.out + (size_t)mrow[b] * p.out_ld + col[a]) = o;
+                if (mok[b] && cok[a]) *reinterpret_cast<f16x4*>(p.out + out_row(p, mrow[b]) * p.out_ld + col[a]) = o;
             }
         }
     } else {
@@ -223,7 +261,7 @@
                     if (p.resid) v += (float)rv[b][q][r];
                     o[r] = (f16)v;
                 }
-                if (mok[b] && cok[q]) *reinterpret_cast<f16x4*>(p.out + (size_t)mrow[b] * p.out_ld + jo[q]) = o;
+                if (mok[b] && cok[q]) *reinterpret_cast<f16x4*>(p.out + out_row(p, mrow[b]) * p.out_ld + jo[q]) = o;
             }
         }
     }
@@ -392,7 +430,10 @@
 }
 
 template <int WM, int WN, int TM, int TN, int STAGES, int KS, int KG = 1>
-__global__ void __launch_bounds__(64 * WM * WN * KG) igemm_dma_kernel(IgemmParams p) {
+__global__ void __launch_bounds__(64 * WM * WN * KG) igemm_dma_kernel(IgemmParams pk) {
+    KernelParams<KS == 2> kp(pk);
+    auto& p = kp.p;
+    constexpr int NT = KS * KS;
     constexpr int NW = WM * WN;
     constexpr int BM = WM * TM * 16, BN = WN * TN * 16;
     constexpr int AI = BM / (8 * NW), BI = BN / (8 * NW);
@@ -408,12 +449,14 @@
     const int wm = wave / WN, wn = wave - (wave / WN) * WN;
     const int bid = xcd_remap(blockIdx.x, p.gx * p.gy * p.ksplit);
     const int tile = bid / p.ksplit, slice = bid - tile * p.ksplit;
-    const int mt = tile / p.gx, nt = tile - mt * p.gx;
+    int mt = tile / p.gx;
+    const int nt = tile - mt * p.gx;
+    if constexpr (KS == 2) mt = kp.set_phase(mt);
     const int m0 = mt * BM, n0 = nt * BN;
     const int lrow = lane >> 3, slot = lane & 7;
     const int hw = p.oh * p.ow;
     const bool two = p.c1 > 0;
-    const int pshift = KS == 3 ? p.w + 1 : 0;
+    const int pshift = KS >= 2 ? p.w + 1 : 0;
 
     unsigned a_off0[AI], a_off1[AI], a_mask[AI];
     int a_ch[AI];
@@ -424,7 +467,8 @@
         const int mm = m < p.M ? m : 0;
         const int nn = mm / hw, r = mm - nn * hw;
         const int oy = r / p.ow, ox = r - oy * p.ow;
-        const int iy0 = oy * p.stride - p.pad, ix0 = ox * p.stride - p.pad;
+        int iy0 = oy * p.stride - p.pad, ix0 = ox * p.stride - p.pad;
+        if constexpr (KS == 2) { iy0 = oy + (p.ph >> 1) - 1; ix0 = ox + (p.ph & 1) - 1; }
         unsigned mask = 0;
         if (m < p.M) {
 #pragma unroll
@@ -459,17 +503,17 @@
     const char* u_src1 = uniform_ptr(p.src1);
     const char* u_wt = uniform_ptr(p.wt);
     int tap = 0, cbase = kb * 64;
-    if (KS == 3) {
-        if (p.cmajor) { tap = kb % 9; cbase = (kb / 9) * 64; }
+    if (KS >= 2) {
+        if (p.cmajor) { tap = kb % NT; cbase = (kb / NT) * 64; }
         else { tap = cbase / p.cin; cbase -= tap * p.cin; }
     }
     auto issue = [&](int kt, int buf) {
         (void)kt;
         const int k0 = tap * p.cin + cbase;
-        const int ky = tap / 3, kx = tap - (tap / 3) * 3;
+        const int ky = tap / (KS == 2 ? 2 : 3), kx = tap - ky * (KS == 2 ? 2 : 3);
         const bool use1 = two && cbase >= p.c0;
         const int cs = use1 ? p.c1 : p.c0;
-        const unsigned sterm = 2u * (unsigned)((KS == 3 ? (ky * p.w + kx) * cs : 0) + (use1 ? cbase - p.c0 : cbase));
+        const unsigned sterm = 2u * (unsigned)((KS >= 2 ? (ky * p.w + kx) * cs : 0) + (use1 ? cbase - p.c0 : cbase));
         const char* sb = use1 ? u_src1 : u_src0;
         const unsigned bias = 2u * (unsigned)(pshift * cs);
         const unsigned sbytes = use1 ? bytes1 : bytes0;
@@ -487,11 +531,11 @@
 #pragma unroll
         for (int i = 0; i < BI; ++i)
             dma_piece(rb, base + A_BYTES + (wave * BI + i) * 1024, b_off[i]);
-        if (KS == 3 && p.cmajor) {
-            if (++tap == 9) { tap = 0; cbase += 64; }
+        if (KS >= 2 && p.cmajor) {
+            if (++tap == NT) { tap = 0; cbase += 64; }
         } else {
             cbase += 64;
-            if (KS == 3 && cbase >= p.cin) { cbase = 0; ++tap; }
+            if (KS >= 2 && cbase >= p.cin) { cbase = 0; ++tap; }
         }
     };
 
@@ -616,7 +660,7 @@
     }
 }
 
-template <int KS, bool S16>
+template <int KS, bool S16, bool FOLD = false>
 __global__ void __launch_bounds__(256) splitk_reduce_kernel(IgemmParams p) {
     const int cq = p.cout >> 2;
     const size_t i = (size_t)blockIdx.x * blockDim.x + threadIdx.x;
@@ -663,7 +707,12 @@
         if (p.resid) v[r] += (float)rv[r];
         o[r] = (f16)v[r];
     }
-    *reinterpret_cast<f16x4*>(p.out + (size_t)m * p.out_ld + j) = o;
+    size_t orow = (size_t)m;
+    if constexpr (FOLD) {
+        const int mq = p.M >> 2, ph = m / mq;
+        orow = out_row_ph(p, m - ph * mq, ph, 1.0f / (float)p.w);
+    }
+    *reinterpret_cast<f16x4*>(p.out + orow * p.out_ld + j) = o;
 }
 
 constexpr int kGnRb = 16;
@@ -764,6 +813,24 @@
 #undef C2D_SKG
         return;
     }
+#if C2D_TUNE_UPFOLD
+    if (p.up == 2) {
+        IgemmParams q = p;
+        q.M = 4 * p.M;
+        const size_t total = (size_t)q.M * (q.cout >> 2);
+        const dim3 grid((unsigned)((total + 255) / 256)), blk(256);
+#define C2D_SKF(KS)                                                                               \
+    if (q.slab16) hipLaunchKernelGGL((splitk_reduce_kernel<KS, true, true>), grid, blk, 0, s, q); \
+    else hipLaunchKernelGGL((splitk_reduce_kernel<KS, false, true>), grid, blk, 0, s, q)
+        switch (q.ksplit) {
+            case 2: C2D_SKF(2); break;
+            case 4: C2D_SKF(4); break;
+            default: C2D_SKF(0); break;
+        }
+#undef C2D_SKF
+        return;
+    }
+#endif
     const size_t total = (size_t)p.M * (p.cout >> 2);
     const dim3 grid((unsigned)((total + 255) / 256)), blk(256);
 #define C2D_SKR(KS)                                                                   \
@@ -825,8 +892,11 @@
 static void run_dma(IgemmParams& p, int ksize, int cout, hipStream_t s) {
     constexpr int BM = WM * TM * 16, BN = WN * TN * 16;
     p.gx = (cout + BN - 1) / BN;
-    p.gy = (p.M + BM - 1) / BM;
+    p.gy = (p.M + BM - 1) / BM * (ksize == 2 ? 4 : 1);
     if (ksize == 1) launch_dma<WM, WN, TM, TN, ST, 1, KG>(p, s);
+#if C2D_TUNE_UPFOLD
+    else if (ksize == 2) launch_dma<WM, WN, TM, TN, ST, 2, KG>(p, s);
+#endif
     else launch_dma<WM, WN, TM, TN, ST, 3, KG>(p, s);
 }
 
@@ -1027,11 +1097,18 @@
     return {id, (ncb + cbs - 1) / cbs, 9 * cbs};
 }
 
+static int plan_ksize(const c2d_conv_desc* d) { return d->up == 2 ? 2 : d->ksize; }
+static bool fold_tile_ok(int id) {
+    return id == 40 || id == 41 || id == 7 || id == 1 || id == 2 || id == 3 || id == 8 || id == 9 || id == 80 || id == 81;
+}
+
 static DmaPlan plan_for(long M, int cout, int kpad, int act, bool pps_ok, int ksize, int rr_id = 0,
                         bool panel_ok = false) {
     const bool geglu = act == C2D_ACT_GEGLU;
+    const bool fold = ksize == 2;
     const int nk = kpad / 64;
     int id = gemm_tile();
+    if (fold && !fold_tile_ok(id)) id = 0;
     if (id == 70) {
         if (panel_ok && gemm_split() <= 1) return {70, 1, nk};
         id = 0;
@@ -1065,14 +1142,14 @@
         DmaPlan pl = plan_dma(M, cout, nk, geglu, id, gemm_split());
         if (pl.id) return pl;
     }
-    if (cout <= 64 && !geglu) {
+    if (cout <= 64 && !geglu && !fold) {
         DmaPlan pl = plan_dma(M, cout, nk, geglu, 29, 0);
         if (pl.id == 29) return pl;
     }
     if (!geglu && cout % 320 != 0) {
         const long mt = (M + 255) / 256;
         if (C2D_PP16_DEFAULT && cout % 256 == 0 && mt * (cout / 256) >= 192) return {41, 1, nk};
-        if (cout % 256 != 0 && cout % 128 == 0 && mt * (cout / 128) >= 192) return {29, 1, nk};
+        if (!fold && cout % 256 != 0 && cout % 128 == 0 && mt * (cout / 128) >= 192) return {29, 1, nk};
     }
     const int t256x320 = (geglu || !C2D_PP16_DEFAULT) ? 25 : 40;
     const long t24 = ((M + 255) / 256) * ((cout + 319) / 320);
@@ -1084,7 +1161,7 @@
         }
         return {t256x320, 1, nk};
     }
-    if (nk >= 90 && t24 >= 64) {
+    if (nk >= (fold ? 40 : 90) && t24 >= 64) {
         DmaPlan pl = plan_dma(M, cout, nk, geglu, 25, 0);
         if (pl.id == 25) pl.id = t256x320;
         return pl;
@@ -1124,7 +1201,7 @@
     const int amode = (d->ksize == 1) ? AM_1X1 : ((cin % 64) == 0 ? AM_3X3_FAST : AM_3X3_GEN);
     const int pd = d->src_pad ? 2 : 0;
     const size_t src_bytes = (size_t)d->n * (d->h + pd) * (d->w + pd) * (size_t)(d->c0 > d->c1 ? d->c0 : d->c1) * 2;
-    return (d->pro == C2D_PRO_NONE || d->pro == C2D_PRO_LNFOLD) && amode != AM_3X3_GEN && !d->up && gemm_mode() != 2 &&
+    return (d->pro == C2D_PRO_NONE || d->pro == C2D_PRO_LNFOLD) && amode != AM_3X3_GEN && d->up != 1 && gemm_mode() != 2 &&
            (d->c1 == 0 || (d->c0 & 63) == 0) && src_bytes < (1u << 31) &&
            (size_t)d->cout * d->kpad * 2 < (1u << 31);
 }
@@ -1142,7 +1219,7 @@
 }
 
 static int tail_images(const c2d_conv_desc* d, const DmaPlan& pl) {
-    if (pl.split != 1 || d->n < 2 || d->pro != C2D_PRO_NONE || d->kpad / 64 < 16) return 0;
+    if (pl.split != 1 || d->n < 2 || d->pro != C2D_PRO_NONE || d->kpad / 64 < 16 || d->up == 2) return 0;
     if (plan_override_tile() || plan_override_split() || !tuning().tail_split) return 0;
     const DmaTile* t = nullptr;
     for (const DmaTile& x : kDmaTiles)
@@ -1174,16 +1251,29 @@
 static size_t tail_ws_bytes(const c2d_conv_desc* d, int n1) {
     const c2d_conv_desc t = tail_desc(d, n1);
     const long Mt = (long)t.n * t.oh * t.ow;
-    const DmaPlan tp = plan_for(Mt, t.cout, t.kpad, t.act, pps_eligible(&t), t.ksize, rr_eligible(&t), panel_eligible(&t));
+    const DmaPlan tp = plan_for(Mt, t.cout, t.kpad, t.act, pps_eligible(&t), plan_ksize(&t), rr_eligible(&t), panel_eligible(&t));
     return tp.split > 1 ? (size_t)tp.split * Mt * t.cout * sizeof(float) : 0;
+}
+
+static int fold_check(const c2d_conv_desc* d) {
+    if (!C2D_TUNE_UPFOLD) return C2D_E_SHAPE;
+    if (d->ksize != 3 || d->stride != 1 || d->c1 != 0 || d->src1) return C2D_E_SHAPE;
+    if (d->n <= 0 || d->h <= 0 || d->w <= 0 || d->oh != 2 * d->h || d->ow != 2 * d->w) return C2D_E_SHAPE;
+    if (d->c0 <= 0 || (d->c0 & 63) || d->kpad != 4 * d->c0 || d->cout <= 0 || (d->cout & 3)) return C2D_E_SHAPE;
+    if ((long)d->n * d->h * d->w >= (1L << 24)) return C2D_E_SHAPE;
+    if (d->src_pad || d->pro != C2D_PRO_NONE || d->act != C2D_ACT_NONE || d->temb || d->resid) return C2D_E_ARG;
+    if (d->gn_mom) return C2D_E_SHAPE;
+    if (!dma_eligible(d)) return C2D_E_SHAPE;
+    return C2D_OK;
 }
 
 extern "C" size_t c2d_conv2d_igemm_workspace_size(const c2d_conv_desc* d) {
     if (!d || d->ksize < 1 || d->oh <= 0 || d->ow <= 0 || d->n <= 0 || d->cout <= 0 || d->kpad < 64) return 0;
+    if (d->up == 2 && fold_check(d) != C2D_OK) return 0;
     if (!dma_eligible(d)) return 0;
     if (d->pro == C2D_PRO_LNFOLD) return 0;
     const long M = (long)d->n * d->oh * d->ow;
-    const DmaPlan pl = plan_for(M, d->cout, d->kpad, d->act, pps_eligible(d), d->ksize, rr_eligible(d), panel_eligible(d));
+    const DmaPlan pl = plan_for(M, d->cout, d->kpad, d->act, pps_eligible(d), plan_ksize(d), rr_eligible(d), panel_eligible(d));
     if (const int n1 = tail_images(d, pl)) return tail_ws_bytes(d, n1);
     return pl.split > 1 ? (size_t)pl.split * M * d->cout * sizeof(float) : 0;
 }
@@ -1193,14 +1283,14 @@
 }
 
 static int gn_rows_for(const c2d_conv_desc* d) {
-    if (!d || d->gn_groups <= 0 || d->cout % d->gn_groups) return 0;
+    if (!d || d->gn_groups <= 0 || d->cout % d->gn_groups || d->up == 2) return 0;
     const int cpg = d->cout / d->gn_groups;
     if (320 % cpg || d->cout % 320 || d->act != C2D_ACT_NONE) return 0;
     if ((d->out_ld & 7) || (d->resid && (d->resid_ld & 7)) || (d->temb && (d->temb_ld & 7)) || d->out_ld < d->cout) return 0;
     if (((uintptr_t)d->out | (uintptr_t)d->resid | (uintptr_t)d->temb) & 15) return 0;
     if (d->ksize < 1 || d->oh <= 0 || d->ow <= 0 || d->n <= 0 || d->kpad < 64 || !dma_eligible(d)) return 0;
     const long M = (long)d->n * d->oh * d->ow;
-    DmaPlan pl = plan_for(M, d->cout, d->kpad, d->act, pps_eligible(d), d->ksize, rr_eligible(d), panel_eligible(d));
+    DmaPlan pl = plan_for(M, d->cout, d->kpad, d->act, pps_eligible(d), plan_ksize(d), rr_eligible(d), panel_eligible(d));
     if (pl.id == 50 || pl.id == 70) return 0;
     bool split = false;
     if (pl.split > 1) {
@@ -1226,6 +1316,10 @@
 extern "C" int c2d_conv2d_igemm_plan(const c2d_conv_desc* d, int* tile_id, int* ksplit) {
     if (!d || !tile_id || !ksplit) return C2D_E_ARG;
     if (d->ksize < 1 || d->oh <= 0 || d->ow <= 0 || d->n <= 0 || d->cout <= 0 || d->kpad < 64) return C2D_E_SHAPE;
+    if (d->up == 2) {
+        const int rc = fold_check(d);
+        if (rc != C2D_OK) return rc;
+    }
     if (d->pro == C2D_PRO_LNFOLD) {
         if (!panel_eligible(d)) return C2D_E_SHAPE;
         *tile_id = 70;
@@ -1238,7 +1332,7 @@
         return C2D_OK;
     }
     const long M = (long)d->n * d->oh * d->ow;
-    DmaPlan pl = plan_for(M, d->cout, d->kpad, d->act, pps_eligible(d), d->ksize, rr_eligible(d), panel_eligible(d));
+    DmaPlan pl = plan_for(M, d->cout, d->kpad, d->act, pps_eligible(d), plan_ksize(d), rr_eligible(d), panel_eligible(d));
     if (pl.split > 1) {
         const size_t need = (size_t)pl.split * M * d->cout * sizeof(float);
         if (!(d->ws && d->ws_bytes >= need && aligned16(d->ws))) pl.split = 1;
@@ -1253,11 +1347,16 @@
 extern "C" int c2d_conv2d_igemm(const c2d_conv_desc* d, void* stream) {
     if (!d || !d->src0 || !d->weight || !d->out) return C2D_E_ARG;
     hipStream_t s = (hipStream_t)stream;
+    if (d->up < 0 || d->up > 2) return C2D_E_ARG;
+    if (d->up == 2) {
+        const int rc = fold_check(d);
+        if (rc != C2D_OK) return rc;
+    }
     if (d->gn_mom && gn_rows_for(d) == 0) return C2D_E_SHAPE;
     if (d->gn_mom && ((uintptr_t)d->gn_mom & 7)) return C2D_E_ALIGN;
     if (d->n >= 2 && d->ksize >= 1 && d->oh > 0 && d->ow > 0 && d->cout > 0 && d->kpad >= 64 && dma_eligible(d)) {
         const long M = (long)d->n * d->oh * d->ow;
-        const DmaPlan pl = plan_for(M, d->cout, d->kpad, d->act, pps_eligible(d), d->ksize, rr_eligible(d), panel_eligible(d));
+        const DmaPlan pl = plan_for(M, d->cout, d->kpad, d->act, pps_eligible(d), plan_ksize(d), rr_eligible(d), panel_eligible(d));
         if (const int n1 = tail_images(d, pl)) {
             c2d_conv_desc head = *d;
             head.n = n1;
@@ -1277,7 +1376,8 @@
     const int cin = d->c0 + d->c1;
     if ((d->c0 & 7) || (d->c1 & 7) || cin <= 0) return C2D_E_SHAPE;
     if (d->kpad & 63) return C2D_E_SHAPE;
-    const int ktot = d->ksize * d->ksize * cin;
+    const bool fold = d->up == 2;
+    const int ktot = (fold ? 4 : d->ksize * d->ksize) * cin;
     if (d->kpad < ktot) return C2D_E_SHAPE;
     if ((d->cout & 3) || d->cout <= 0) return C2D_E_SHAPE;
     if (d->act == C2D_ACT_GEGLU && (d->cout & 31)) return C2D_E_SHAPE;
@@ -1321,6 +1421,11 @@
     p.resid = (const f16*)d->resid; p.resid_ld = d->resid_ld;
     p.out = (f16*)d->out; p.out_ld = d->out_ld;
     p.M = d->n * d->oh * d->ow;
+    if (fold) {
+        p.oh = d->h; p.ow = d->w;
+        p.M = d->n * d->h * d->w;
+    }
+    const long M_all = (long)d->n * d->oh * d->ow;
     p.gn_mom = (float*)d->gn_mom;
     p.gn_cpg = d->gn_mom ? d->cout / d->gn_groups : 0;
     if (p.M <= 0) return C2D_OK;
@@ -1336,10 +1441,10 @@
     p.cmajor = gemm_korder();
     const long t128 = (long)((p.M + 127) / 128) * ((d->cout + 127) / 128);
     if (dma) {
-        DmaPlan pl = fixed ? *fixed : plan_for(p.M, d->cout, d->kpad, d->act, pps_eligible(d), d->ksize, rr_eligible(d), panel_eligible(d));
+        DmaPlan pl = fixed ? *fixed : plan_for(M_all, d->cout, d->kpad, d->act, pps_eligible(d), plan_ksize(d), rr_eligible(d), panel_eligible(d));
         if (d->pro == C2D_PRO_LNFOLD) pl = {70, 1, d->kpad / 64};
         if (pl.split > 1) {
-            const size_t need = (size_t)pl.split * p.M * d->cout * sizeof(float);
+            const size_t need = (size_t)pl.split * M_all * d->cout * sizeof(float);
             if (d->ws && d->ws_bytes >= need && aligned16(d->ws)) {
                 p.ws = (float*)d->ws;
             } else {
@@ -1347,7 +1452,9 @@
                 pl.nkt = d->kpad / 64;
             }
         }
-        dispatch_dma(p, pl, d->ksize, d->cout, s);
+        dispatch_dma(p, pl, plan_ksize(d), d->cout, s);
+    } else if (fold) {
+        return C2D_E_SHAPE;
     } else if (t128 < 512) {
         p.gx = (d->cout + 63) / 64; p.gy = (p.M + 63) / 64;
         if (amode == AM_1X1) launch<64, 64, AM_1X1>(p, s);
diff --git a/clap2diffusion_amd/csrc/igemm_m32.h b/clap2diffusion_amd/csrc/igemm_m32.h
--- a/clap2diffusion_amd/csrc/igemm_m32.h
+++ b/clap2diffusion_amd/csrc/igemm_m32.h
@@ -15,6 +15,7 @@
 
 template <int BM, int BN, int BK, int NW, int KS, int SW = 0, bool PRE = false>
 struct M32Loader {
+    static constexpr int NT = KS * KS;
     static constexpr int RB = 2 * BK, RPP = 1024 / RB, CPR = BK / 8;
     static constexpr int NA = BM / RPP, NB = BN / RPP;
     static constexpr int SA = NA / NW;
@@ -36,19 +37,20 @@
     __device__ __forceinline__ int row_of(int wave, int i) const { return (wave + i * NW) * RPP + lrow; }
     __device__ __forceinline__ int chunk_of(int row) const { return (lchunk ^ sw_of<BK, SW>(row)) * 8; }
 
-    __device__ __forceinline__ void init(const IgemmParams& p, int m0, int n0, int wave, int lane, int kb) {
+    __device__ __forceinline__ void init(const IgemmParams& p, int m0, int n0, int wave, int lane, int kb, int ph = 0) {
         lrow = lane / CPR;
         lchunk = lane % CPR;
         const int hw = p.oh * p.ow;
         two = p.c1 > 0;
-        pshift = KS == 3 ? p.w + 1 : 0;
+        pshift = KS >= 2 ? p.w + 1 : 0;
 #pragma unroll
         for (int i = 0; i < SA; ++i) {
             const int m = m0 + row_of(wave, i);
             const int mm = m < p.M ? m : 0;
             const int nn = mm / hw, r = mm - nn * hw;
             const int oy = r / p.ow, ox = r - oy * p.ow;
-            const int iy0 = oy * p.stride - p.pad, ix0 = ox * p.stride - p.pad;
+            int iy0 = oy * p.stride - p.pad, ix0 = ox * p.stride - p.pad;
+            if constexpr (KS == 2) { iy0 = oy + (ph >> 1) - 1; ix0 = ox + (ph & 1) - 1; }
             unsigned mask = 0;
             if (m < p.M) {
 #pragma unroll
@@ -86,8 +88,8 @@
         u_wt = uniform_ptr(p.wt);
         cbase = kb * BK;
         tap = 0;
-        if (KS == 3) {
-            if (p.cmajor) { tap = kb % 9; cbase = (kb / 9) * BK; }
+        if (KS >= 2) {
+            if (p.cmajor) { tap = kb % NT; cbase = (kb / NT) * BK; }
             else { tap = cbase / p.cin; cbase -= tap * p.cin; }
         }
     }
@@ -101,10 +103,10 @@
     __device__ __forceinline__ Stage prep_at(const IgemmParams& p, int tap, int cbase) const {
         Stage st;
         const int k0 = tap * p.cin + cbase;
-        const int ky = tap / 3, kx = tap - (tap / 3) * 3;
+        const int ky = tap / (KS == 2 ? 2 : 3), kx = tap - ky * (KS == 2 ? 2 : 3);
         const bool use1 = two && cbase >= p.c0;
         st.cs = use1 ? p.c1 : p.c0;
-        const unsigned sterm = 2u * (unsigned)((KS == 3 ? (ky * p.w + kx) * st.cs : 0) + (use1 ? cbase - p.c0 : cbase));
+        const unsigned sterm = 2u * (unsigned)((KS >= 2 ? (ky * p.w + kx) * st.cs : 0) + (use1 ? cbase - p.c0 : cbase));
         const char* sb = use1 ? u_src1 : u_src0;
         const unsigned bias = 2u * (unsigned)(pshift * st.cs);
         const unsigned sbytes = use1 ? bytes1 : bytes0;
@@ -131,11 +133,11 @@
         }
     }
     __device__ __forceinline__ void advance() {
-        if (KS == 3 && cbase_major) {
-            if (++tap == 9) { tap = 0; cbase += BK; }
+        if (KS >= 2 && cbase_major) {
+            if (++tap == NT) { tap = 0; cbase += BK; }
         } else {
             cbase += BK;
-            if (KS == 3 && cbase >= cin_) { cbase = 0; ++tap; }
+            if (KS >= 2 && cbase >= cin_) { cbase = 0; ++tap; }
         }
     }
 
diff --git a/clap2diffusion_amd/csrc/igemm_pp16.h b/clap2diffusion_amd/csrc/igemm_pp16.h
--- a/clap2diffusion_amd/csrc/igemm_pp16.h
+++ b/clap2diffusion_amd/csrc/igemm_pp16.h
@@ -10,7 +10,9 @@
 namespace c2d {
 
 template <int TN, int KS, int PH>
-__global__ void __launch_bounds__(512) igemm_pp16_kernel(IgemmParams p) {
+__global__ void __launch_bounds__(512) igemm_pp16_kernel(IgemmParams pk) {
+    KernelParams<KS == 2> kp(pk);
+    auto& p = kp.p;
     constexpr int BK = 64, NW = 8, TMW = 8;
     constexpr int BM = 2 * TMW * 16, BN = 4 * TN * 16;
     constexpr int RB = 2 * BK, STAGE = (BM + BN) * RB;
@@ -27,13 +29,16 @@
     const int wr = wave >> 2, wc = wave & 3;
     const int bid = xcd_remap(blockIdx.x, p.gx * p.gy * p.ksplit);
     const int tile = bid / p.ksplit, slice = bid - tile * p.ksplit;
-    const int mt = tile / p.gx, nt = tile - mt * p.gx;
+    int mt = tile / p.gx;
+    const int nt = tile - mt * p.gx;
+    int ph = 0;
+    if constexpr (KS == 2) { mt = kp.set_phase(mt); ph = p.ph; }
     const int m0 = mt * BM, n0 = nt * BN;
     const int nk_all = p.kpad / BK;
     const int kb = slice * p.nkt, ke = min(nk_all, kb + p.nkt);
 
     Loader ld;
-    ld.init(p, m0, n0, wave, lane, kb);
+    ld.init(p, m0, n0, wave, lane, kb, ph);
     const int fo0 = lds_sw<BK>(lane & 15, lane >> 4), fo1 = lds_sw<BK>(lane & 15, 4 + (lane >> 4));
     const int a_base = wr * TMW * 16 * RB, b_base = BM * RB + wc * TN * 16 * RB;
 
@@ -189,8 +194,11 @@
 static void run_pp16(IgemmParams& p, int ksize, int cout, hipStream_t s) {
     constexpr int BM = 256, BN = 4 * TN * 16;
     p.gx = (cout + BN - 1) / BN;
-    p.gy = (p.M + BM - 1) / BM;
+    p.gy = (p.M + BM - 1) / BM * (ksize == 2 ? 4 : 1);
     if (ksize == 1) launch_pp16<TN, 1>(p, s);
+#if C2D_TUNE_UPFOLD
+    else if (ksize == 2) launch_pp16<TN, 2>(p, s);
+#endif
     else launch_pp16<TN, 3>(p, s);
 }
 
diff --git a/clap2diffusion_amd/layers.py b/clap2diffusion_amd/layers.py
--- a/clap2diffusion_amd/layers.py
+++ b/clap2diffusion_amd/layers.py
@@ -51,6 +51,24 @@
 
     def forward(self, x: torch.Tensor, **kw) -> torch.Tensor:
         return ops.conv(x, self.weight, self.kpad, self.cout, ksize=self.ksize, stride=self.stride, bias=self.bias, **kw)
+
+
+class HUpConv2d(HConv2d):
+
+    def __init__(self, cin: int, cout: int):
+        super().__init__(cin, cout, 3)
+        self.kpad_fold = 4 * cin
+        self.register_buffer("weight_fold", torch.zeros(4, cout, self.kpad_fold, dtype=torch.float16), persistent=False)
+
+    @torch.no_grad()
+    def load(self, w: torch.Tensor, b: torch.Tensor | None) -> None:
+        super().load(w, b)
+        wf, kp = ops.fold_upsample_weight(w.float())
+        assert kp == self.kpad_fold
+        self.weight_fold.copy_(wf)
+
+    def forward_folded(self, x: torch.Tensor) -> torch.Tensor:
+        return ops.conv(x, self.weight_fold, self.kpad_fold, self.cout, ksize=3, bias=self.bias, up_fold=True)
 
 
 class HGroupNorm(nn.Module):
diff --git a/clap2diffusion_amd/ops.py b/clap2diffusion_amd/ops.py
--- a/clap2diffusion_amd/ops.py
+++ b/clap2diffusion_amd/ops.py
@@ -55,6 +55,36 @@
     return wp.to(F16).contiguous(), kp
 
 
+_UPFOLD_TAPS = (((0,), (1, 2)), ((0, 1), (2,)))
+
+
+@torch.no_grad()
+def fold_upsample_weight(w: torch.Tensor, dtype: torch.dtype = F16) -> tuple[torch.Tensor, int]:
+    cout, cin, kh, kw = w.shape
+    assert kh == 3 and kw == 3
+    out = w.new_zeros(4, cout, 2, 2, cin)
+    for a in range(2):
+        for b in range(2):
+            for ty in range(2):
+                for tx in range(2):
+                    acc = out[2 * a + b, :, ty, tx, :]
+                    for ky in _UPFOLD_TAPS[a][ty]:
+                        for kx in _UPFOLD_TAPS[b][tx]:
+                            acc += w[:, :, ky, kx]
+    return out.reshape(4, cout, 4 * cin).to(dtype).contiguous(), 4 * cin
+
+
+@functools.lru_cache(maxsize=None)
+def upfold_ok(n: int, h: int, w: int, cin: int, cout: int) -> bool:
+    import ctypes
+    from ._lib import ConvDesc, lib
+    d = ConvDesc()
+    d.c0, d.n, d.h, d.w, d.oh, d.ow, d.ksize, d.stride, d.up = cin, n, h, w, 2 * h, 2 * w, 3, 1, 2
+    d.cout, d.kpad, d.out_ld = cout, 4 * cin, cout
+    tid, ks = ctypes.c_int(), ctypes.c_int()
+    return lib().c2d_conv2d_igemm_plan(ctypes.byref(d), ctypes.byref(tid), ctypes.byref(ks)) == 0
+
+
 def geglu_interleave(w: torch.Tensor, b: torch.Tensor | None):
     two_i = w.shape[0]
     inner = two_i // 2
@@ -69,7 +99,7 @@
          up: bool = False, x2: torch.Tensor | None = None, gn=None, gn_silu: bool = False, ln=None,
          silu_in: bool = False, act: str | None = None, temb: torch.Tensor | None = None,
          resid: torch.Tensor | None = None, out: torch.Tensor | None = None, padded: bool = False,
-         ln_fold=None, gn_moments: int = 0):
+         ln_fold=None, gn_moments: int = 0, up_fold: bool = False):
     _require(x, "x")
     if x.dim() == 2:
         h, w = 1, x.shape[0]
@@ -82,8 +112,12 @@
     assert x.is_contiguous() and x.dtype == F16
     if x2 is not None:
         assert x2.is_contiguous() and x2.dtype == F16 and x2.shape[:-1] == x.shape[:-1]
+    if up_fold:
+        assert ksize == 3 and stride == 1 and not up and not padded and x2 is None and x.dim() == 4
+        assert gn is None and ln is None and not silu_in and act is None and temb is None and resid is None
+        assert not gn_moments and not ln_fold
     if ksize == 3:
-        vh, vw = (2 * h, 2 * w) if up else (h, w)
+        vh, vw = (2 * h, 2 * w) if up or up_fold else (h, w)
         oh, ow = (vh + 2 - 3) // stride + 1, (vw + 2 - 3) // stride + 1
     else:
         oh, ow = h, w
@@ -103,7 +137,8 @@
         if rows:
             mom = torch.empty((out.shape[0], oh * ow // rows, gn_moments, 2), device=x.device, dtype=torch.float32)
     C2D.conv2d_igemm(x, weight, kpad, cout, ksize, stride, up, x2, gs, gh, gn_silu, ls, lg, lb, silu_in, bias,
-                     C2D_ACT[act], temb, resid, out, bool(padded), float(ln_fold or 0.0), mom, int(gn_moments))
+                     C2D_ACT[act], temb, resid, out, bool(padded), float(ln_fold or 0.0), mom, int(gn_moments),
+                     bool(up_fold))
     if gn_moments:
         return out, (GnMoments(out, mom, rows, gn_moments) if mom is not None else None)
     return out
diff --git a/clap2diffusion_amd/torch_ops.py b/clap2diffusion_amd/torch_ops.py
--- a/clap2diffusion_amd/torch_ops.py
+++ b/clap2diffusion_amd/torch_ops.py
@@ -12,7 +12,7 @@
 
 def _conv_desc(x, weight, kpad, cout, ksize, stride, up, x2, gn_scale, gn_shift, gn_silu, ln_stats, ln_gamma,
                ln_beta, silu_in, bias, act, temb, resid, out, src_pad=False, lnf_eps=0.0, gn_mom=None,
-               gn_groups=0) -> ConvDesc:
+               gn_groups=0, up_fold=False) -> ConvDesc:
     if x.dim() == 2:
         n, h, w = 1, 1, x.shape[0]
         c0 = x.shape[1]
@@ -22,14 +22,14 @@
             h, w = h - 2, w - 2
     c1 = x2.shape[-1] if x2 is not None else 0
     if ksize == 3:
-        vh, vw = (2 * h, 2 * w) if up else (h, w)
+        vh, vw = (2 * h, 2 * w) if up or up_fold else (h, w)
         oh, ow = (vh + 2 - 3) // stride + 1, (vw + 2 - 3) // stride + 1
     else:
         oh, ow = h, w
     d = ConvDesc()
     d.src0 = ptr(x); d.src1 = ptr(x2); d.c0 = c0; d.c1 = c1
     d.n, d.h, d.w, d.oh, d.ow = n, h, w, oh, ow
-    d.ksize, d.stride, d.up = ksize, stride, int(up)
+    d.ksize, d.stride, d.up = ksize, stride, (2 if up_fold else int(up))
     d.weight = ptr(weight); d.cout = cout; d.kpad = kpad
     if lnf_eps > 0.0:
         d.pro = C2D_PRO_LNFOLD; d.pro_eps = lnf_eps
@@ -64,9 +64,9 @@
                  ln_stats: Optional[Tensor], ln_gamma: Optional[Tensor], ln_beta: Optional[Tensor], silu_in: bool,
                  bias: Optional[Tensor], act: int, temb: Optional[Tensor], resid: Optional[Tensor],
                  out: Tensor, src_pad: bool = False, lnf_eps: float = 0.0, gn_mom: Optional[Tensor] = None,
-                 gn_groups: int = 0) -> None:
+                 gn_groups: int = 0, up_fold: bool = False) -> None:
     d = _conv_desc(x, weight, kpad, cout, ksize, stride, up, x2, gn_scale, gn_shift, gn_silu, ln_stats, ln_gamma,
-                   ln_beta, silu_in, bias, act, temb, resid, out, src_pad, lnf_eps, gn_mom, gn_groups)
+                   ln_beta, silu_in, bias, act, temb, resid, out, src_pad, lnf_eps, gn_mom, gn_groups, up_fold)
     wsb = lib().c2d_conv2d_igemm_workspace_size(ctypes.byref(d))
     if wsb:
         ws = torch.empty(wsb // 4, device=x.device, dtype=torch.float32)
@@ -80,7 +80,7 @@
 
 @conv2d_igemm.register_fake
 def _(x, weight, kpad, cout, ksize, stride, up, x2, gn_scale, gn_shift, gn_silu, ln_stats, ln_gamma, ln_beta,
-      silu_in, bias, act, temb, resid, out, src_pad=False, lnf_eps=0.0, gn_mom=None, gn_groups=0):
+      silu_in, bias, act, temb, resid, out, src_pad=False, lnf_eps=0.0, gn_mom=None, gn_groups=0, up_fold=False):
     return None
 
 
diff --git a/clap2diffusion_amd/unet.py b/clap2diffusion_amd/unet.py
--- a/clap2diffusion_amd/unet.py
+++ b/clap2diffusion_amd/unet.py
@@ -6,7 +6,7 @@
 import torch.nn as nn
 
 from . import ops
-from .layers import HConv2d, HGroupNorm, HLayerNorm, HLinear
+from .layers import HConv2d, HGroupNorm, HLayerNorm, HLinear, HUpConv2d
 from .processor import AttnProcessor, AudioAttnProcessor
 from .weights import SD15_UNET
 
@@ -292,11 +292,15 @@
 
 
 class Upsample2D(nn.Module):
+
     def __init__(self, c):
         super().__init__()
-        self.conv = HConv2d(c, c, 3)
+        self.conv = HUpConv2d(c, c)
 
     def forward(self, x):
+        n, h, w, c = x.shape
+        if ops.upfold_ok(n, h, w, c, self.conv.cout):
+            return self.conv.forward_folded(x)
         return self.conv(ops.upsample_nearest2x(x))
 
 
```

Measured after the change: 9.609 images/sec, median of 6. 3.3% higher.
